# grunwaldlab/krisp

Hardware: AMD Instinct MI355X
Metric: k-mers/s sorted+intersected at k=28 (higher is better)
Workload: dtype u64

## Files before the change

### include/krisp_hip.h

```cpp
#ifndef KRISP_HIP_H
#define KRISP_HIP_H

#include <stddef.h>
#include <stdint.h>

#ifdef __cplusplus
extern "C" {
#endif

typedef struct kr_ctx kr_ctx;

typedef struct { uint64_t prefix, in_mask, out_mask; } kr_cand;

typedef struct { uint64_t key; uint32_t genome; uint32_t count; } kr_record;

enum {
    KR_OK = 0,
    KR_ERR_HIP = -1,
    KR_ERR_PARAM = -2,
    KR_ERR_CAPACITY = -3,
    KR_ERR_STATE = -4,
    KR_ERR_KEY = -5,
    KR_ERR_HOST = -6
};
// ... 122 lines not shown
int64_t kr_design_fetch(kr_ctx*, kr_design_record* out, size_t cap);
typedef struct {
    int32_t loop_ds[64];
} kr_hairpin_params;
int kr_design_hairpins(kr_ctx*, const kr_hairpin_params* params);
int64_t kr_design_fetch_hairpins(kr_ctx*, int32_t* out, size_t cap);

typedef struct {
    int32_t guide_size, pam5_len, pam3_len;
    uint8_t pam5[8], pam3[8];
    int32_t gc_lo, gc_hi, min_mismatches;
} kr_guide_params;
int kr_guides_table(kr_ctx*, const kr_guide_params* params);
typedef struct {
    uint32_t found, strand, start, min_mismatches, sum_mismatches, gc, candidates, pad;
} kr_guide_record;
int64_t kr_guides_run(kr_ctx*, const uint8_t* rows, const uint64_t* row_off, const uint32_t* bounds, uint64_t nregions, int K,
                      int L, int D);
int64_t kr_guides_fetch(kr_ctx*, kr_guide_record* out, size_t cap);
int64_t kr_guides_run_top(kr_ctx*, const uint8_t* rows, const uint64_t* row_off, const uint32_t* bounds, uint64_t nregions, int K,
                          int L, int D, int top);
int64_t kr_guides_fetch_top(kr_ctx*, kr_guide_record* out, size_t cap);

int64_t kr_guide_hits_table(kr_ctx*, const uint8_t* texts, uint64_t nguides, int mismatches, const char* pam5, const char* pam3,
                            int need_pam);
typedef struct { uint32_t guide; uint8_t strand, mismatches, pam, pad; uint64_t pos; uint64_t columns; } kr_guide_hit;
int64_t kr_guide_hits_scan(kr_ctx*, int id);
int64_t kr_guide_hits_fetch(kr_ctx*, kr_guide_hit* out, size_t cap);
int64_t kr_guide_hits_windows(kr_ctx*, uint8_t* rows, size_t cap_bytes);
int64_t kr_guide_hits_tally(kr_ctx*, uint32_t* out, size_t cap);

int64_t kr_guide_bulges_table(kr_ctx*, const uint8_t* texts, uint64_t nguides, int mismatches, int bulges, const char* pam5,
                              const char* pam3, int need_pam);
typedef struct { uint32_t guide; uint8_t strand, mismatches, pam; int8_t bulge; uint64_t pos; uint64_t columns;
                 uint32_t bulge_column, length; } kr_guide_bulge_hit;
int64_t kr_guide_bulges_scan(kr_ctx*, int id);
int64_t kr_guide_bulges_fetch(kr_ctx*, kr_guide_bulge_hit* out, size_t cap);
int64_t kr_guide_bulges_windows(kr_ctx*, uint8_t* rows, size_t cap_bytes);

int64_t kr_assay_table(kr_ctx*, const uint32_t* links, uint64_t n);
typedef struct { uint64_t pos; uint32_t length, pair; uint8_t strand, left_mm, right_mm, left_end_mm, right_end_mm, hit_strand,
                 hit_mismatches, hit_pam; uint64_t hit_pos; uint64_t columns; uint32_t guide, hit; } kr_assay_hit;
int64_t kr_assay_join(kr_ctx*, int id);
int64_t kr_assay_fetch(kr_ctx*, kr_assay_hit* out, size_t cap);

int64_t kr_fasta_to_bases(const uint8_t* text, size_t n, int universal_newlines, int one_shot, uint8_t* out,
                          size_t cap, int64_t* stats);

int64_t kr_ingest_file(const char* path, uint8_t** bases, int64_t* stats);
int64_t kr_read_file(const char* path, uint8_t** text, int64_t* stats);
int64_t kr_genome_upload_bgzf(kr_ctx*, int id, const uint8_t* file, size_t n, int one_shot, int64_t* stats);
int64_t kr_genome_upload_gzip(kr_ctx*, int id, const uint8_t* file, size_t n, size_t chunk, int one_shot, int64_t* stats);
int kr_reserve(kr_ctx*, const int* ids, int n, size_t n_bases, int with_text);
int kr_mem_info(kr_ctx*, int64_t* out4);
int64_t kr_genome_upload_text(kr_ctx*, int id, const uint8_t* text, size_t n, int universal_newlines, int one_shot,
                              int64_t* stats);
int64_t kr_genome_fetch_bases(kr_ctx*, int id, uint8_t* out, size_t cap);
void    kr_host_free(void* p);

int64_t kr_scan_special(const uint8_t* bases, size_t n, int k, int omit_soft, uint64_t* starts, size_t cap,
                        int* bad_char);

int64_t kr_render_records(const kr_record* recs, size_t n, int L, int D, int R, const uint32_t* label_of,
                          size_t n_genomes, const char* const* label_text, size_t n_labels, const uint8_t* label_in,
                          int dot, char** csv, size_t* csv_len, char** align, size_t* align_len);
int64_t kr_render_windows(const uint8_t* rows, size_t n, int L, int D, int R, const uint32_t* cand, const uint32_t* genome,
                          const uint32_t* label_of, size_t n_genomes, const char* const* label_text, size_t n_labels,
                          const uint8_t* label_in, int dot, int rna, char** csv, size_t* csv_len, char** align,
                          size_t* align_len);
void    kr_text_free(void* p);

enum { KR_OPT_SLICE_BASES = 1,
       KR_OPT_GENERIC_INTERSECT = 2,
       KR_OPT_ISECT_FORMAT = 3,
       KR_OPT_ABLATE = 4,
       KR_OPT_WIDE_SLOTS = 5,
       KR_OPT_PLACE_TRIES = 7,
       KR_OPT_ISECT_KERNEL = 8,
       KR_OPT_LANES = 9,
       KR_OPT_LAZY_ORDER = 10,
       KR_OPT_COARSE_REST = 11,
       KR_OPT_COARSE_POOL = 12,
       KR_OPT_JOIN2 = 13,
       KR_OPT_WIDE_ORDERED = 6 };
int     kr_set_option(kr_ctx*, int option, int64_t value);

int     kr_sync(kr_ctx*);
int     kr_timer_begin(kr_ctx*);
double  kr_timer_end_ms(kr_ctx*);
int     kr_stage_enable(kr_ctx*, int on);
int     kr_stage_select(kr_ctx*, unsigned stage_mask);
int     kr_stage_reset(kr_ctx*);
double  kr_stage_ms(kr_ctx*, int stage);
int64_t kr_stage_launches(kr_ctx*, int stage);

int64_t kr_debug_fetch(kr_ctx*, int genome_id, int what, void* out, size_t cap_bytes);
int64_t kr_debug_inversions(kr_ctx*, int genome_id);
double  kr_debug_localsort(kr_ctx*, int genome_id, int reps, int mode);
double  kr_debug_intersect(kr_ctx*, const int* genome_ids, int n, const uint8_t* is_ingroup, int reps, int mode);
double  kr_debug_copy_gbps(kr_ctx*, size_t bytes, int reps);
const char* kr_debug_copy_which(kr_ctx*);
int     kr_build_experiments(void);
int     kr_debug_lazy(kr_ctx*, int64_t* out8);
int     kr_debug_isect(kr_ctx*, int64_t* out8);
int     kr_debug_scan(kr_ctx*, int64_t* out8);
int     kr_debug_place(kr_ctx*, double* out8);
int     kr_debug_coarse_pool(kr_ctx*, double* out8);
int     kr_debug_comm(kr_ctx*, int64_t* out8);
int     kr_debug_comm_probe(kr_ctx*, size_t bytes, int reps, double* out3);
int64_t kr_debug_cands_selfexchange(kr_ctx*, int apply_filter);
int     kr_debug_comm_hang(kr_ctx*);
int64_t kr_debug_budget_left(kr_ctx*);
int     kr_debug_budget_set(kr_ctx*, int64_t left);
int     kr_debug_info(kr_ctx*, int64_t* out8);

#ifdef __cplusplus
}
#endif
#endif
```

### krisp_amd/_native.py

```python
import ctypes
import os

import numpy as np

HERE = os.path.dirname(os.path.abspath(__file__))
LIB_PATH = os.environ.get("KRISP_HIP_LIB") or os.path.join(HERE, "libkrisp_hip.so")

CAND = np.dtype([("prefix", "<u8"), ("in_mask", "<u8"), ("out_mask", "<u8")])
RECORD = np.dtype([("key", "<u8"), ("genome", "<u4"), ("count", "<u4")])
WIDE_HIT = np.dtype([("cand", "<u4"), ("genome", "<u4"), ("pos", "<u4"), ("strand", "<u4")])
LOC_HIT = np.dtype([("group", "<u4"), ("strand", "<u4"), ("pos", "<u8")])
NEAR_HIT = np.dtype([("target", "<u4"), ("strand", "u1"), ("mismatches", "u1"), ("flank_mismatches", "u1"), ("pad", "u1"),
                     ("pos", "<u8")])
PRODUCT_SITE = np.dtype([("pos", "<u8"), ("entry", "<u4"), ("mismatches", "u1"), ("end_mismatches", "u1"),
                         ("pad", "<u2")])
PRODUCT_HIT = np.dtype([("pos", "<u8"), ("length", "<u4"), ("pair", "<u4"), ("strand", "u1"), ("left_mm", "u1"),
                        ("right_mm", "u1"), ("left_end_mm", "u1"), ("right_end_mm", "u1"), ("pad", "u1", (3,))])
DESIGN_RECORD = np.dtype([("found", "<u4"), ("product_size", "<u4"), ("pair_penalty", "<u4"), ("left_start", "<u2"),
                          ("left_len", "<u2"), ("right_start", "<u2"), ("right_len", "<u2"), ("left_tm", "<i4"), ("right_tm", "<i4"),
                          ("left_gc", "<u2"), ("right_gc", "<u2"), ("left_penalty", "<u4"), ("right_penalty", "<u4"),
                          ("left_self_any", "<i4"), ("left_self_end", "<i4"), ("right_self_any", "<i4"),
                          ("right_self_end", "<i4"), ("pair_any", "<i4"), ("pair_end", "<i4")])
DESIGN_RECORD_HP = np.dtype(DESIGN_RECORD.descr + [("left_hairpin", "<i4"), ("right_hairpin", "<i4")])
GUIDE_RECORD = np.dtype([("found", "<u4"), ("strand", "<u4"), ("start", "<u4"), ("min_mismatches", "<u4"),
                         ("sum_mismatches", "<u4"), ("gc", "<u4"), ("candidates", "<u4"), ("pad", "<u4")])
GUIDE_HIT_RAW = np.dtype([("guide", "<u4"), ("strand", "u1"), ("mismatches", "u1"), ("pam", "u1"), ("pad", "u1"), ("pos", "<u8"),
                          ("columns", "<u8")])
ASSAY_HIT_RAW = np.dtype([("pos", "<u8"), ("length", "<u4"), ("pair", "<u4"), ("strand", "u1"), ("left_mm", "u1"), ("right_mm", "u1"),
                          ("left_end_mm", "u1"), ("right_end_mm", "u1"), ("hit_strand", "u1"), ("hit_mismatches", "u1"),
                          ("hit_pam", "u1"), ("hit_pos", "<u8"), ("columns", "<u8"), ("guide", "<u4"), ("hit", "<u4")])
GUIDE_BULGE_HIT_RAW = np.dtype([("guide", "<u4"), ("strand", "u1"), ("mismatches", "u1"), ("pam", "u1"), ("bulge", "i1"),
                                ("pos", "<u8"), ("columns", "<u8"), ("bulge_column", "<u4"), ("length", "<u4")])
WIDE_DICT_LEFT, WIDE_DICT_RIGHT, WIDE_GROUPS, WIDE_HITS, WIDE_COUNTS, WIDE_SLOT_BITS, WIDE_NGROUPS, WIDE_BATCH_USED, WIDE_LOCATED, WIDE_KEYS_LISTED = 0, 1, 2, 3, 4, 5, 6, 7, 8, 9
WIDE_MAX_K = 1024
WIDE_MAX_FLANK = 256
COMM_ID_BYTES = 128

SOFT_MAP, SOFT_OMIT = 0, 1
OPT_SLICE_BASES, OPT_GENERIC_INTERSECT, OPT_ISECT_FORMAT, OPT_ABLATE, OPT_WIDE_SLOTS, OPT_WIDE_ORDERED, OPT_PLACE_TRIES = 1, 2, 3, 4, 5, 6, 7
OPT_ISECT_KERNEL = 8
OPT_LANES = 9
OPT_LAZY_ORDER = 10
OPT_COARSE_REST = 11
OPT_COARSE_POOL = 12
OPT_JOIN2 = 13
ERR_KEY, ERR_HOST = -5, -6
STRANDS_BOTH, STRANDS_FORWARD, STRANDS_CANONICAL = 0, 1, 2
STAGES = ["pack", "hist8", "reduce8", "scatter1", "hist2", "scan2", "scatter2", "chunks", "localsort",
          "fallback", "intersect", "compact", "collect", "merge", "locate"]
STAGE_KERNELS = {"pack": "k_pack", "hist8": "k_hist8 (wide path: k_hist8w, slices: k_hist8k)", "reduce8": "k_reduce8a+k_reduce8b",
                 "scatter1": "k_scatter1p (wide path: k_scatter1w, slices: k_scatter1kp)",
                 "hist2": "k_hist16 (or k_hist2)", "scan2": "k_hist16_off (or k_scan2)", "scatter2": "k_scatter2",
                 "chunks": "k_chunk_table", "localsort": "k_localsort2",
                 "fallback": "k_seg_merge", "intersect": "k_intersect3 (+ k_intersect for oversized items)",
                 "compact": "k_scan+k_publish_reset+k_gather_items",
                 "collect": "k_collect_count+k_tile_sums+k_scan+k_tile_apply+k_publish+k_collect_emit",
                 "merge": "k_cands_flag+k_scan+k_cands_compact", "locate": "k_wide_locate"}

_c = ctypes
_P = _c.c_void_p
SYMBOLS = [
    ("kr_create", _P, [_c.c_int, _c.c_size_t]),
    ("kr_destroy", None, [_P]),
    ("kr_last_error", _c.c_char_p, [_P]),
    ("kr_set_params", _c.c_int, [_P, _c.c_int, _c.c_int, _c.c_int, _c.c_int, _c.c_size_t]),
    ("kr_set_strands", _c.c_int, [_P, _c.c_int]),
    ("kr_genome_upload", _c.c_int, [_P, _c.c_int, _P, _c.c_size_t]),
    ("kr_genome_sort", _c.c_int, [_P, _c.c_int]),
    ("kr_genome_partition", _c.c_int, [_P, _c.c_int]),
    ("kr_genome_add", _c.c_int64, [_P, _c.c_int, _P, _c.c_size_t]),
    ("kr_genome_count", _c.c_int64, [_P, _c.c_int]),
    ("kr_genome_load_sorted", _c.c_int64, [_P, _c.c_int, _P, _c.c_size_t]),
    ("kr_genome_fetch_keys", _c.c_int64, [_P, _c.c_int, _P, _c.c_size_t]),
    ("kr_genome_keys_in_order", _c.c_int64, [_P, _c.c_int, _P, _c.c_size_t]),
    ("kr_set_allow", _c.c_int, [_P, _c.c_uint]),
    ("kr_set_field_order", _c.c_int, [_P, _P, _P]),
    ("kr_set_field_pieces", _c.c_int, [_P, _c.c_int, _P, _P]),
    ("kr_genome_free", _c.c_int, [_P, _c.c_int]),
    ("kr_intersect", _c.c_int64, [_P, _P, _c.c_int, _P, _c.c_int]),
    ("kr_cands_count", _c.c_int64, [_P]),
    ("kr_cands_fetch", _c.c_int64, [_P, _P, _c.c_size_t]),
    ("kr_cands_load", _c.c_int64, [_P, _P, _c.c_size_t]),
    ("kr_cands_merge", _c.c_int64, [_P, _P, _c.c_size_t, _c.c_int, _c.c_int]),
    ("kr_cands_probe", _c.c_int64, [_P, _P, _c.c_int, _P, _c.c_int]),
    ("kr_comm_unique_id", _c.c_int, [_P]),
    ("kr_comm_init", _c.c_int, [_P, _c.c_int, _c.c_int, _P]),
    ("kr_comm_init_dir", _c.c_int, [_P, _c.c_int, _c.c_int, _c.c_char_p]),
    ("kr_comm_destroy", _c.c_int, [_P]),
    ("kr_comm_rank", _c.c_int, [_P]),
    ("kr_comm_world", _c.c_int, [_P]),
    ("kr_comm_rccl_ranks", _c.c_int, [_P]),
    ("kr_comm_barrier", _c.c_int, [_P]),
    ("kr_comm_allreduce", _c.c_int, [_P, _P, _c.c_int, _c.c_int]),
    ("kr_comm_allgather", _c.c_int, [_P, _P, _c.c_size_t, _P]),
    ("kr_cands_reduce", _c.c_int64, [_P, _c.c_int]),
    ("kr_cands_bcast", _c.c_int64, [_P]),
    ("kr_records_gather", _c.c_int64, [_P]),
    ("kr_collect", _c.c_int64, [_P, _P, _c.c_int]),
    ("kr_fetch", _c.c_int64, [_P, _P, _c.c_size_t]),
    ("kr_set_params_wide", _c.c_int, [_P, _c.c_int, _c.c_int, _c.c_int, _c.c_int, _c.c_size_t]),
    ("kr_wide_run", _c.c_int64, [_P, _P, _c.c_int, _P, _c.c_int]),
    ("kr_wide_fetch", _c.c_int64, [_P, _c.c_int, _P, _c.c_size_t]),
    ("kr_wide_fetch_windows", _c.c_int64, [_P, _P, _c.c_size_t]),
    ("kr_set_params_locate", _c.c_int, [_P, _c.c_int, _c.c_int, _c.c_int, _c.c_int, _c.c_size_t]),
    ("kr_locate_table", _c.c_int64, [_P, _P, _c.c_uint64]),
    ("kr_locate_scan", _c.c_int64, [_P, _c.c_int]),
    ("kr_locate_fetch", _c.c_int64, [_P, _P, _c.c_size_t]),
    ("kr_locate_windows", _c.c_int64, [_P, _P, _c.c_size_t]),
    ("kr_locate_seps", _c.c_int64, [_P, _c.c_int, _P, _c.c_size_t]),
    ("kr_near_table", _c.c_int64, [_P, _P, _c.c_uint64, _c.c_int]),
    ("kr_near_scan", _c.c_int64, [_P, _c.c_int]),
    ("kr_near_fetch", _c.c_int64, [_P, _P, _c.c_size_t]),
    ("kr_near_windows", _c.c_int64, [_P, _P, _c.c_size_t]),
    ("kr_products_table", _c.c_int64, [_P, _P, _c.c_uint64, _P, _c.c_uint64, _P, _c.c_uint64, _c.c_int, _c.c_uint32]),
    ("kr_products_scan", _c.c_int64, [_P, _c.c_int]),
    ("kr_products_fetch", _c.c_int64, [_P, _P, _c.c_size_t]),
    ("kr_products_sites", _c.c_int64, [_P, _P, _c.c_size_t]),
    ("kr_primers_table", _c.c_int64, [_P, _P, _P, _c.c_uint64, _c.c_uint64, _P, _c.c_uint64, _c.c_int, _c.c_uint32]),
    ("kr_primers_scan", _c.c_int64, [_P, _c.c_int]),
    ("kr_primers_fetch", _c.c_int64, [_P, _P, _c.c_size_t]),
    ("kr_primers_sites", _c.c_int64, [_P, _P, _c.c_size_t]),
    ("kr_design_table", _c.c_int, [_P, _P]),
    ("kr_design_run", _c.c_int64, [_P, _P, _c.c_uint64, _c.c_int, _c.c_int, _c.c_int]),
    ("kr_design_fetch", _c.c_int64, [_P, _P, _c.c_size_t]),
    ("kr_design_hairpins", _c.c_int, [_P, _P]),
    ("kr_design_fetch_hairpins", _c.c_int64, [_P, _P, _c.c_size_t]),
    ("kr_guides_table", _c.c_int, [_P, _P]),
    ("kr_guides_run", _c.c_int64, [_P, _P, _P, _P, _c.c_uint64, _c.c_int, _c.c_int, _c.c_int]),
    ("kr_guides_fetch", _c.c_int64, [_P, _P, _c.c_size_t]),
    ("kr_guides_run_top", _c.c_int64, [_P, _P, _P, _P, _c.c_uint64, _c.c_int, _c.c_int, _c.c_int, _c.c_int]),
    ("kr_guides_fetch_top", _c.c_int64, [_P, _P, _c.c_size_t]),
    ("kr_guide_hits_table", _c.c_int64, [_P, _P, _c.c_uint64, _c.c_int, _c.c_char_p, _c.c_char_p, _c.c_int]),
    ("kr_guide_hits_scan", _c.c_int64, [_P, _c.c_int]),
    ("kr_guide_hits_fetch", _c.c_int64, [_P, _P, _c.c_size_t]),
    ("kr_guide_hits_windows", _c.c_int64, [_P, _P, _c.c_size_t]),
    ("kr_guide_hits_tally", _c.c_int64, [_P, _P, _c.c_size_t]),
    ("kr_guide_bulges_table", _c.c_int64, [_P, _P, _c.c_uint64, _c.c_int, _c.c_int, _c.c_char_p, _c.c_char_p, _c.c_int]),
    ("kr_guide_bulges_scan", _c.c_int64, [_P, _c.c_int]),
    ("kr_guide_bulges_fetch", _c.c_int64, [_P, _P, _c.c_size_t]),
    ("kr_guide_bulges_windows", _c.c_int64, [_P, _P, _c.c_size_t]),
    ("kr_assay_table", _c.c_int64, [_P, _P, _c.c_uint64]),
    ("kr_assay_join", _c.c_int64, [_P, _c.c_int]),
    ("kr_assay_fetch", _c.c_int64, [_P, _P, _c.c_size_t]),
    ("kr_render_windows", _c.c_int64, [_P, _c.c_size_t, _c.c_int, _c.c_int, _c.c_int, _P, _P, _P, _c.c_size_t, _P, _c.c_size_t, _P,
                                       _c.c_int, _c.c_int, _P, _P, _P, _P]),
    ("kr_fasta_to_bases", _c.c_int64, [_P, _c.c_size_t, _c.c_int, _c.c_int, _P, _c.c_size_t, _P]),
    ("kr_ingest_file", _c.c_int64, [_c.c_char_p, _P, _P]),
    ("kr_read_file", _c.c_int64, [_c.c_char_p, _P, _P]),
    ("kr_genome_upload_text", _c.c_int64, [_P, _c.c_int, _P, _c.c_size_t, _c.c_int, _c.c_int, _P]),
    ("kr_genome_upload_bgzf", _c.c_int64, [_P, _c.c_int, _P, _c.c_size_t, _c.c_int, _P]),
    ("kr_genome_upload_gzip", _c.c_int64, [_P, _c.c_int, _P, _c.c_size_t, _c.c_size_t, _c.c_int, _P]),
    ("kr_reserve", _c.c_int, [_P, _P, _c.c_int, _c.c_size_t, _c.c_int]),
    ("kr_genome_fetch_bases", _c.c_int64, [_P, _c.c_int, _P, _c.c_size_t]),
    ("kr_host_free", None, [_P]),
    ("kr_scan_special", _c.c_int64, [_P, _c.c_size_t, _c.c_int, _c.c_int, _P, _c.c_size_t, _P]),
    ("kr_set_option", _c.c_int, [_P, _c.c_int, _c.c_int64]),
    ("kr_sync", _c.c_int, [_P]),
    ("kr_timer_begin", _c.c_int, [_P]),
    ("kr_timer_end_ms", _c.c_double, [_P]),
    ("kr_stage_enable", _c.c_int, [_P, _c.c_int]),
    ("kr_stage_select", _c.c_int, [_P, _c.c_uint]),
    ("kr_stage_reset", _c.c_int, [_P]),
    ("kr_stage_ms", _c.c_double, [_P, _c.c_int]),
    ("kr_stage_launches", _c.c_int64, [_P, _c.c_int]),
    ("kr_debug_fetch", _c.c_int64, [_P, _c.c_int, _c.c_int, _P, _c.c_size_t]),
    ("kr_debug_inversions", _c.c_int64, [_P, _c.c_int]),
    ("kr_debug_localsort", _c.c_double, [_P, _c.c_int, _c.c_int, _c.c_int]),
    ("kr_debug_intersect", _c.c_double, [_P, _P, _c.c_int, _P, _c.c_int, _c.c_int]),
    ("kr_debug_copy_gbps", _c.c_double, [_P, _c.c_size_t, _c.c_int]),
    ("kr_debug_copy_which", _c.c_char_p, [_P]),
    ("kr_mem_info", _c.c_int, [_P, _P]),
    ("kr_debug_comm", _c.c_int, [_P, _P]),
    ("kr_debug_place", _c.c_int, [_P, _P]),
    ("kr_debug_coarse_pool", _c.c_int, [_P, _P]),
    ("kr_debug_comm_probe", _c.c_int, [_P, _c.c_size_t, _c.c_int, _P]),
    ("kr_debug_cands_selfexchange", _c.c_int64, [_P, _c.c_int]),
    ("kr_debug_info", _c.c_int, [_P, _P]),
    ("kr_render_records", _c.c_int64, [_P, _c.c_size_t, _c.c_int, _c.c_int, _c.c_int, _P, _c.c_size_t, _P, _c.c_size_t, _P,
                                       _c.c_int, _P, _P, _P, _P]),
    ("kr_text_free", None, [_P]),
    ("kr_debug_isect", _c.c_int, [_P, _P]),
    ("kr_debug_lazy", _c.c_int, [_P, _P]),
    ("kr_debug_scan", _c.c_int, [_P, _P]),
    ("kr_set_mixed_alphabets", _c.c_int, [_P, _c.c_int]),
    ("kr_build_experiments", _c.c_int, []),
    ("kr_comm_set_timeout", _c.c_int, [_P, _c.c_int]),
    ("kr_debug_comm_hang", _c.c_int, [_P]),
    ("kr_debug_budget_left", _c.c_int64, [_P]),
    ("kr_debug_budget_set", _c.c_int, [_P, _c.c_int64]),
]


class GuideParams(ctypes.Structure):
    _fields_ = [("guide_size", _c.c_int32), ("pam5_len", _c.c_int32), ("pam3_len", _c.c_int32), ("pam5", _c.c_uint8 * 8),
                ("pam3", _c.c_uint8 * 8), ("gc_lo", _c.c_int32), ("gc_hi", _c.c_int32), ("min_mismatches", _c.c_int32)]


class KrispHipError(RuntimeError):
    code = None


ERR_CAPACITY = -3


_lib = None


def load():
    global _lib
    if _lib is not None:
        return _lib
    if not os.path.exists(LIB_PATH):
        raise KrispHipError(
            f"{LIB_PATH} is missing: build it with `python -m krisp_amd.build` "
            "(hipcc --offload-arch=gfx950); there is no CPU fallback")
    lib = ctypes.CDLL(LIB_PATH)
    for name, res, args in SYMBOLS:
        fn = getattr(lib, name)
        fn.restype = res
        fn.argtypes = args
    _lib = lib
    return lib


def _ptr(a):
    return a.ctypes.data_as(ctypes.c_void_p)


def _motif_bytes(m):
    return m if isinstance(m, bytes) else str(m).encode("ascii", "replace")


def fasta_to_bases(data, universal_newlines, one_shot=True):
    lib = load()
    src = np.frombuffer(data, dtype=np.uint8)
    out = np.empty(len(src) + 1, dtype=np.uint8)
    stats = np.zeros(4, dtype=np.int64)
    n = lib.kr_fasta_to_bases(_ptr(src) if len(src) else None, len(src), 1 if universal_newlines else 0,
                              1 if one_shot else 0, _ptr(out), len(out), _ptr(stats))
    if n < 0:
        raise KrispHipError(f"kr_fasta_to_bases: [{n}]")
    return out[:n], int(stats[0]), int(stats[1]), stats[2] == 1, bool(stats[3])


class _HostBlock:

    def __init__(self, lib, ptr):
        self.lib, self.ptr = lib, ptr

    def __del__(self):
        try:
            if self.ptr:
                self.lib.kr_host_free(self.ptr)
                self.ptr = None
        except Exception:
            pass

# ... 555 lines not shown

    def guides_top(self, rows, row_off, bounds, L, D, top):
        rows, off, bnd, n = self._guide_regions(rows, row_off, bounds, "guides_top")
        self._check(self.lib.kr_guides_run_top(self.ctx, _ptr(rows) if rows.size else None, _ptr(off), _ptr(bnd) if n else None, n,
                                               rows.shape[1], L, D, top), "kr_guides_run_top")
        out = np.empty((max(n, 1), top), dtype=GUIDE_RECORD)
        self._check(self.lib.kr_guides_fetch_top(self.ctx, _ptr(out), n * top), "kr_guides_fetch_top")
        return out[:n]

    def sync(self):
        self._check(self.lib.kr_sync(self.ctx), "kr_sync")

    def timer_begin(self):
        self._check(self.lib.kr_timer_begin(self.ctx), "kr_timer_begin")

    def timer_end_ms(self):
        ms = self.lib.kr_timer_end_ms(self.ctx)
        if ms < 0:
            raise KrispHipError("kr_timer_end_ms failed")
        return ms

    def stage_enable(self, on=True):
        self.lib.kr_stage_enable(self.ctx, 1 if on else 0)

    def stage_select(self, names):
        mask = 0
        for n in names:
            mask |= 1 << STAGES.index(n)
        self.lib.kr_stage_select(self.ctx, mask)

    def stage_reset(self):
        self.lib.kr_stage_reset(self.ctx)

    def stage_times(self):
        return {name: (self.lib.kr_stage_ms(self.ctx, i), self.lib.kr_stage_launches(self.ctx, i))
                for i, name in enumerate(STAGES)}

    def debug_info(self):
        o = np.zeros(8, dtype=np.int64)
        self.lib.kr_debug_info(self.ctx, _ptr(o))
        return dict(b=int(o[0]), nbuckets=int(o[1]), T=int(o[2]), CAP=int(o[3]), nwg=int(o[4]),
                    overflow_segments=int(o[5]), fallback_launches=int(o[6]), nslices=int(o[7]))

    def debug_isect(self):
        o = np.zeros(8, dtype=np.int64)
        self.lib.kr_debug_isect(self.ctx, _ptr(o))
        return dict(chunk_kernel_items=int(o[0]), slices_redone=int(o[1]), threads=int(o[2]), buckets_per_item_log2=int(o[3]),
                    heads32=int(o[4]), sort_lanes=int(o[5]), join2_launches=int(o[6]), join2_handed_on=int(o[7]))

    def debug_lazy(self):
        o = np.zeros(8, dtype=np.int64)
        self.lib.kr_debug_lazy(self.ctx, _ptr(o))
        return dict(skipped=int(o[0]), ordered_later=int(o[1]), touch_collects=int(o[2]), on=int(o[3]),
                    anchor_in_bucket_order=int(o[4]), fuse_anchor=int(o[5]), coarse=int(o[6]), coarse_promoted=int(o[7]))

    def debug_scan(self):
        o = np.zeros(8, dtype=np.int64)
        self.lib.kr_debug_scan(self.ctx, _ptr(o))
        return dict(tiles=int(o[0]), grid=int(o[1]), cap=int(o[2]), blocks=int(o[3]))

    def copy_gbps(self, nbytes=1 << 30, reps=10):
        v = self.lib.kr_debug_copy_gbps(self.ctx, nbytes, reps)
        if v < 0:
            raise KrispHipError("kr_debug_copy_gbps failed")
        return v

    def mem_info(self):
        o = np.zeros(4, dtype=np.int64)
        self._check(self.lib.kr_mem_info(self.ctx, _ptr(o)), "kr_mem_info")
        return dict(avail=int(o[0]), total=int(o[1]), used=int(o[2]), budget=int(o[3]))

    def debug_comm(self):
        o = np.zeros(8, dtype=np.int64)
        self._check(self.lib.kr_debug_comm(self.ctx, _ptr(o)), "kr_debug_comm")
        return dict(syncs=int(o[0]), p2p=int(o[1]), collectives=int(o[2]), exchange_us=int(o[3]), reduces=int(o[4]),
                    message_entries=int(o[5]))

    def debug_place(self):
        o = np.zeros(8, dtype=np.float64)
        self._check(self.lib.kr_debug_place(self.ctx, _ptr(o)), "kr_debug_place")
        return dict(candidates=int(o[0]), taken=int(o[1]), fastest_ms=[round(float(x), 4) for x in o[2:6]],
                    median_ms=round(float(o[6]), 4), slowest_ms=round(float(o[7]), 4))

    def debug_coarse_pool(self):
        o = np.zeros(8, dtype=np.float64)
        self._check(self.lib.kr_debug_coarse_pool(self.ctx, _ptr(o)), "kr_debug_coarse_pool")
        return dict(total=int(o[0]), free=int(o[1]), held=int(o[2]), partitions=int(o[3]), searches=int(o[4]),
                    held_ms=[round(float(o[5]), 4), round(float(o[6]), 4)], on=int(o[7]))

    def comm_set_timeout(self, seconds):
        self._check(self.lib.kr_comm_set_timeout(self.ctx, int(seconds)), "kr_comm_set_timeout")

    def debug_comm_hang(self):
        return self._check(self.lib.kr_debug_comm_hang(self.ctx), "kr_debug_comm_hang")

    def cands_selfexchange(self, apply_filter=False):
        return self._check(self.lib.kr_debug_cands_selfexchange(self.ctx, 1 if apply_filter else 0), "kr_debug_cands_selfexchange")

    def comm_probe(self, nbytes=64 << 10, reps=50):
        o = np.zeros(3, dtype=np.float64)
        self._check(self.lib.kr_debug_comm_probe(self.ctx, nbytes, reps, _ptr(o)), "kr_debug_comm_probe")
        return dict(allreduce_sync_us=round(float(o[0]), 2), sendrecv_self_sync_us=round(float(o[1]), 2),
                    bcast_sync_us=round(float(o[2]), 2), message_bytes=int(nbytes))

    def copy_which(self):
        return (self.lib.kr_debug_copy_which(self.ctx) or b"").decode()

    def inversions(self, gid):
        return self._check(self.lib.kr_debug_inversions(self.ctx, gid), "kr_debug_inversions")

    def debug_fetch(self, gid, what, n_max):
        dt = {0: np.uint64, 1: np.uint32, 2: np.uint32, 3: np.uint32, 4: np.uint64, 5: np.uint64}[what]
        out = np.empty(max(n_max, 1), dtype=dt)
        n = self._check(self.lib.kr_debug_fetch(self.ctx, gid, what, _ptr(out), out.nbytes), "kr_debug_fetch")
        return out[:n]
```

### krisp_amd/csrc/h_core.inc

```
static thread_local std::string g_last_error;

struct DevBuf {
    void* p = nullptr;
    size_t bytes = 0;
};

struct Slice {
    DevBuf keys, off, chunkstart, chunkdesc, ovf;
    u64 nmax = 0;
    u32 nchunks = 0;
    int64_t count = -1;
    int res = -1;
};

struct Genome {
    int id = -1;
    size_t n_bases = 0;
    u64 nwords = 0;
    u64 nmax = 0;
    DevBuf bases, wkeys;
    DevBuf wlcnt;
    bool wlist = false;
    u32 wlcap = 0;
    std::vector<Slice> sl;
    bool uploaded = false, sorted = false, finalized = false;
    bool ordered = false;
    bool coarse = false;
    DevBuf ckeys;
    double ckeys_ms = 0;
    hipStream_t ckeys_busy = nullptr;
    hipEvent_t ckeys_ev = nullptr;
    bool ckeys_wait = false;
    int64_t partitions = 0;
    DevBuf hits;
    u32 hitcap = 0;
    bool hits_valid = false;
    bool was_anchor = false;
    int64_t count = -1;
    hipEvent_t up_done = nullptr;
};

struct Lane {
    hipStream_t stream = nullptr;
    hipEvent_t done = nullptr;
    bool pending = false;
    DevBuf codes, bad, partial8, base1, tmpkeys, tp, tiledesc, tilehist, wkeys;
    DevBuf partial16, cursor, h16exc;
    DevBuf pass0, base64;
    DevBuf slt, offa, cura;
    void bufs(std::vector<DevBuf*>& v) {
        v.insert(v.end(), {&codes, &bad, &partial8, &base1, &tmpkeys, &tp, &tiledesc, &tilehist, &wkeys, &pass0, &base64,
                           &partial16, &cursor, &h16exc, &slt, &offa, &cura});
    }
};
#define MAX_LANES 8

struct kr_comm;

struct kr_ctx {
    int device = 0;
    kr_comm* comm = nullptr;
    hipStream_t stream = nullptr;
    hipStream_t copy_stream = nullptr;
    Lane lanes[MAX_LANES];
    int nlanes = 0, next_lane = 0;
    int lanes_ready = 0;
    int64_t sorts_done = 0;
    int place_n = 0, place_taken = 0;
    double place_ms[6] = {0, 0, 0, 0, 0, 0};
    size_t place_bytes = 0;
    u64 ex_cap = 0;
    char copy_which[160] = {0};
    u64 lane_maxcount = 0;
    int last_lane = 0;
    int sb = 0, nslices = 1;
    size_t budget = 0, used = 0;
    bool have_params = false;
    Geom g{};
    size_t max_bases = 0;
    std::map<int, Genome> genomes;
    int ls_grid = 768;
    int place_tries = 8;
    bool place_tries_set = false;
    bool shared_gpu = false;
    DevBuf candP;
    DevBuf candA, candB, chunkcnt, chunkpos, flags, blockcnt, blockpos, other, records, nrec, fbdesc, fbsegs;
    DevBuf coltab, collo, colcnt, colpos, coltsum, coltpos, colfirst, colfm;
    int64_t ncand = -1;
    int64_t nrecords = 0;
    std::string err;
    hipEvent_t t0 = nullptr, t1 = nullptr;
    bool stage_on = false;
    unsigned stage_mask = ~0u;
    struct Pair { hipEvent_t a, b; int stage; };
    std::vector<Pair> pending;
    std::vector<hipEvent_t> pool;
    double stage_ms[KR_ST_COUNT] = {0};
    int64_t stage_n[KR_ST_COUNT] = {0};
    int64_t fallback_launches = 0, overflow_segments = 0;
    int dbg = 0;
    int isect_kernel = 0;
    int ncu = 256;
    DevBuf bgz_in, bgz_tab, bgz_stat;
    DevBuf tx_scan;
    DevBuf tx_text, tx_tile, tx_tilepos, tx_lines, tx_ls, tx_ll, tx_op, tx_outpos, tx_state, tx_tsum, tx_tpos;
    u32* mbox = nullptr;
    std::vector<uint64_t> coltab_host;
    std::vector<int> mb_free;
    int mb_next = 0;
    int i3_occ[3][4][9] = {{{0}}};
    DevBuf isovf;
    int join2 = 1;
    u32 j2_grid = 0;
    int j2_occ[9] = {0};
    int64_t j2_launches = 0, j2_full = 0;
    bool j2_full_counted = false;
    int64_t isect_ovf_items = 0, isect_refall = 0;
    int i3_last_T = 0, i3_last_mlog = 0, i3_last_tags = 0, i3_last_ua = 0;
    int64_t isect_ua = 0;
    int fuse_anchor = 1;
    u32 i3_ovf_cap = I3_OVF_CAP;
    int isect_fmt = 0;
    int opt_slice_bases = -1;
    hipEvent_t slice_ready[2] = {nullptr, nullptr};
    bool custom_layout = false;
    bool mixed_alphabets = false;
    int lazy_order = 1;
    bool order_wanted = false;
    int64_t lazy_skipped = 0, lazy_ordered = 0, lazy_touch = 0;
    DevBuf touchdesc, touchovf;
    int coarse_rest = 1;
    int64_t coarse_done = 0, coarse_promoted = 0;
    int coarse_pool = 1;
    struct PoolBuf { DevBuf buf; double ms; hipEvent_t ev; bool wait; };
    std::vector<PoolBuf> cpool_free;
    int cpool_total = 0;
    int64_t cpool_partitions = 0;
    int64_t cpool_searches = 0;
    size_t place_min_bytes = (size_t)256 << 20;
    DevBuf co_state, co_tab;
    u32 co_tcap = CO_TCAP;
    u32 co_hitcap = 0;
    int co_occ = 0;
    u32 co_grid = 0;
    u32 scan_cap = 0;
    int64_t scan_dbg[3] = {0, 0, 0};
    int slice_route = 1;
    typedef std::vector<DevBuf*> Bufs;
    struct Wide {
        bool on = false;
        int L = 0, D = 0, R = 0, k = 0, omit = 0, W = 0, strands = 0;
        struct DictBufs {
            DevBuf keys, idx, slots;
            DevBuf mzT, mzB;
            int ib = 1, sb = 0, mzlen = 0;
            u32 n = 0, mznb = 0;
            bool canon = false;
            u32 nfull = 0;
            void bufs(Bufs& v) { v.insert(v.end(), {&keys, &idx, &slots, &mzT, &mzB}); }
            Dict view() const {
                Dict d{};
                d.keys = (const u64*)keys.p;
                d.idx = (const u32*)idx.p;
                d.slots = sb && slots.p ? (const uint4*)slots.p : nullptr;
                d.ib = ib;
                d.sb = sb;
                d.mzT = mzlen && mzT.p ? (const u64*)mzT.p : nullptr;
                d.mzB = (const u32*)mzB.p;
                d.mznb = mznb;
                d.mzlen = mzlen;
                d.canon = canon ? 1 : 0;
                return d;
            }
        };
        DictBufs fd[2][2 * FR_MAXP - 1], fin;
        static int fd_pieces(int len) { return (len + 31) / 32; }
        static int fd_plen(int len, int j) { const int np = fd_pieces(len); return len / np + (j < len % np ? 1 : 0); }
        static int fd_poff(int len, int j) { int o = 0; for (int q = 0; q < j; q++) o += fd_plen(len, q); return o; }
        static int fd_last(int len) { return fd_pieces(len) > 1 ? 2 * (fd_pieces(len) - 1) : 0; }
        FlankRank fr[2];
        DevBuf flbuf;
        FlankRank flhost[8][2];
        int flslot = 0;
        std::vector<int> run_ids;
        DevBuf rows, rowtab;
        DevBuf masks, keep, cnt, hitoff, cursor, hits, cibuf, tsum, tpos;
        DevBuf loc, loccur;
        u64 located = 0;
        bool use_slots = true;
        bool ordered = false;
        bool use_share = true;
        int lanes = 0;
        bool packed_spectrum = true;
        DevBuf wcount;
        bool share = false;
        bool genome_cache = false;
        bool key_list = false;
        bool key_list_failed = false;
        double key_list_frac = 0;
        u64 keys_listed = 0;
        int batch = 0;
        std::vector<u64> nkeys;
        u32 nfin = 0;
        u64 ngroups = 0;
        int64_t nhits = -1;
        void locate_bufs(Bufs& v) { v.insert(v.end(), {&masks, &keep, &cnt, &hitoff, &cursor, &hits, &cibuf, &loc}); }
        void bufs(Bufs& v) {
            fin.bufs(v);
            locate_bufs(v);
            v.insert(v.end(), {&loccur, &tsum, &tpos, &wcount, &flbuf, &rows, &rowtab});
            for (auto& flank : fd)
                for (DictBufs& d : flank) d.bufs(v);
        }
    } wide;
    struct SeedTable {
// ... 173 lines not shown

#define MB_WORDS 65536
#define MB_SLICE0 64
#define PUB_CAP 4096
static int mbox_slot(kr_ctx* c) {
    if (!c->mb_free.empty()) { const int s = c->mb_free.back(); c->mb_free.pop_back(); return s; }
    if (MB_SLICE0 + 2 * (c->mb_next + 1) > MB_WORDS) return -1;
    return c->mb_next++;
}

static void coarse_pool_handover(kr_ctx* c, Genome& G) {
    if (!G.ckeys.p || !G.ckeys_busy) return;
    if (!G.ckeys_ev && hipEventCreateWithFlags(&G.ckeys_ev, hipEventDisableTiming) != hipSuccess) G.ckeys_ev = nullptr;
    if (G.ckeys_ev && hipEventRecord(G.ckeys_ev, G.ckeys_busy) == hipSuccess) G.ckeys_wait = true;
    else (void)hipStreamSynchronize(G.ckeys_busy);
    G.ckeys_busy = nullptr;
    (void)c;
}
static void coarse_pool_return(kr_ctx* c, Genome& G) {
    if (!G.ckeys.p) return;
    coarse_pool_handover(c, G);
    kr_ctx::PoolBuf pb{G.ckeys, G.ckeys_ms, G.ckeys_ev, G.ckeys_wait};
    auto at = c->cpool_free.begin();
    while (at != c->cpool_free.end() && at->ms <= pb.ms) ++at;
    c->cpool_free.insert(at, pb);
    G.ckeys = DevBuf();
    G.ckeys_ms = 0;
    G.ckeys_ev = nullptr;
    G.ckeys_wait = false;
}
static void coarse_pool_purge(kr_ctx* c, size_t bytes) {
    for (size_t i = c->cpool_free.size(); i-- > 0;) {
        kr_ctx::PoolBuf& pb = c->cpool_free[i];
        if (pb.buf.bytes >= bytes) continue;
        if (pb.ev) { if (pb.wait) (void)hipEventSynchronize(pb.ev); (void)hipEventDestroy(pb.ev); }
        release(c, pb.buf);
        c->cpool_free.erase(c->cpool_free.begin() + (long)i);
        c->cpool_total--;
    }
}
static bool coarse_pool_take(kr_ctx* c, Genome& G, size_t bytes) {
    for (auto at = c->cpool_free.begin(); at != c->cpool_free.end(); ++at)
        if (at->buf.bytes >= bytes) {
            G.ckeys = at->buf;
            G.ckeys_ms = at->ms;
            G.ckeys_ev = at->ev;
            G.ckeys_wait = at->wait;
            G.ckeys_busy = nullptr;
            c->cpool_free.erase(at);
            return true;
        }
    return false;
}
static void coarse_pool_release(kr_ctx* c) {
    if (c->cpool_free.empty()) return;
    (void)hipDeviceSynchronize();
    for (auto& pb : c->cpool_free) {
        release(c, pb.buf);
        if (pb.ev) (void)hipEventDestroy(pb.ev);
    }
    c->cpool_total -= (int)c->cpool_free.size();
    c->cpool_free.clear();
}

static void release_slice(kr_ctx* c, Slice& S) {
    release(c, S.keys);
    release(c, S.off);
    release(c, S.chunkstart);
    release(c, S.chunkdesc);
    release(c, S.ovf);
    if (S.res >= 0) c->mb_free.push_back(S.res);
}
static void genome_drop_sorted(kr_ctx* c, Genome& G) {
    for (Slice& S : G.sl) release_slice(c, S);
    G.sl.clear();
    G.sorted = G.finalized = G.ordered = false;
}
static void reset_slices(kr_ctx* c, Genome& G) {
    if ((int)G.sl.size() == c->nslices) return;
    for (Slice& S : G.sl) release_slice(c, S);
    G.sl.assign(c->nslices, Slice());
}
static void genome_unsorted(Genome& G) {
    G.sorted = G.finalized = G.ordered = G.coarse = G.hits_valid = false;
    G.count = -1;
}

static void release_genome(kr_ctx* c, Genome& G) {
    coarse_pool_return(c, G);
    if (G.up_done) { (void)hipEventDestroy(G.up_done); G.up_done = nullptr; }
    release(c, G.bases);
    release(c, G.wkeys);
    release(c, G.wlcnt);
    release(c, G.hits);
    for (Slice& S : G.sl) release_slice(c, S);
    G.sl.clear();
}

struct StageScope {
    kr_ctx* c;
    int stage;
    hipEvent_t a = nullptr, b = nullptr;
    hipStream_t stream;
    StageScope(kr_ctx* c_, int st, hipStream_t s_ = nullptr) : c(c_), stage(st), stream(s_ ? s_ : c_->stream) {
        c->stage_n[st]++;
        if (!c->stage_on || !((c->stage_mask >> st) & 1u)) return;
        auto get = [&]() {
            hipEvent_t e;
            if (!c->pool.empty()) { e = c->pool.back(); c->pool.pop_back(); }
            else (void)hipEventCreate(&e);
            return e;
        };
        a = get();
        b = get();
        (void)hipEventRecord(a, stream);
    }
    ~StageScope() {
        if (!a) return;
        (void)hipEventRecord(b, stream);
        c->pending.push_back({a, b, stage});
    }
};

static void resolve_stages(kr_ctx* c) {
    for (auto& p : c->pending) {
        float ms = 0;
        (void)hipEventSynchronize(p.b);
        if (hipEventElapsedTime(&ms, p.a, p.b) == hipSuccess) c->stage_ms[p.stage] += ms;
        c->pool.push_back(p.a);
        c->pool.push_back(p.b);
    }
    c->pending.clear();
}

#define LANES_AUTO 3
#define LANES_AFTER 16
static inline int lanes_used(const kr_ctx* c) {
    if (c->wide.on) return c->wide.lanes > 0 ? c->wide.lanes : (c->nlanes > 1 ? 2 : 1);
    if (c->g.wmode) return 1;
    if (c->nslices > 1) return c->nlanes == 1 || (c->nlanes == 0 && c->sorts_done < 2) ? 1 : 2;
    return c->nlanes > 0 ? c->nlanes : (c->sorts_done >= LANES_AFTER ? LANES_AUTO : 1);
}

static int join_lanes(kr_ctx* c) {
    for (int i = 1; i < MAX_LANES; i++) {
        Lane& ln = c->lanes[i];
        if (!ln.pending) continue;
        HIPCHK(c, hipEventRecord(ln.done, ln.stream));
        HIPCHK(c, hipStreamWaitEvent(c->stream, ln.done, 0));
        ln.pending = false;
    }
    return KR_OK;
}

static int lane_open(kr_ctx* c, Lane& ln) {
    if (ln.stream) return KR_OK;
    HIPCHK(c, hipStreamCreate(&ln.stream));
    HIPCHK(c, hipEventCreateWithFlags(&ln.done, hipEventDisableTiming));
    return KR_OK;
}
static void release_lanes(kr_ctx* c, int first) {
    std::vector<DevBuf*> lb;
    for (int i = first; i < MAX_LANES; i++) c->lanes[i].bufs(lb);
    for (DevBuf* b : lb) release(c, *b);
}
static int ensure_h16exc(kr_ctx* c, Lane& ln, hipStream_t st) {
    if (ln.h16exc.p) return KR_OK;
    int rc;
    if ((rc = ensure(c, ln.h16exc, (1 + 3 * (size_t)H16_EXC_CAP) * 4))) return rc;
    HIPCHK(c, hipMemsetAsync(ln.h16exc.p, 0, 16, st));
    return KR_OK;
}

static void launch_excl_scan(hipStream_t st, const u32* in, u32 n, u32* tsum, u32* tpos, u32* out) {
    const u32 ntiles = (n + 2047) / 2048;
    hipLaunchKernelGGL(k_tile_sums, dim3(ntiles), dim3(256), 0, st, in, n, tsum);
    hipLaunchKernelGGL(k_scan, dim3(1), dim3(1024), 0, st, (const u32*)tsum, tpos, ntiles);
    hipLaunchKernelGGL(k_tile_apply, dim3(ntiles), dim3(256), 0, st, in, n, (const u32*)tpos, ntiles, out);
}

extern "C" {

const char* kr_last_error(kr_ctx* c) { return c ? c->err.c_str() : g_last_error.c_str(); }

kr_ctx* kr_create(int device, size_t hbm_budget_bytes) {
    int ndev = 0;
    if (hipGetDeviceCount(&ndev) != hipSuccess || ndev <= 0) {
        g_last_error = "no HIP device visible";
        return nullptr;
    }
    if (device < 0 || device >= ndev) {
        g_last_error = "device index out of range";
        return nullptr;
    }
    if (hipSetDevice(device) != hipSuccess) {
        g_last_error = "hipSetDevice failed";
        return nullptr;
    }
    kr_ctx* c = new kr_ctx();
    c->device = device;
    c->budget = hbm_budget_bytes;
    {
        const char* e = getenv("KR_DBG");
        c->dbg = e ? (atoi(e) & 32) : 0;
        const char* e2 = getenv("KR_ISECT_FMT");
        c->isect_fmt = e2 ? (atoi(e2) == 1 ? 1 : (atoi(e2) == 2 ? 2 : 0)) : 0;
        const char* e3 = getenv("KR_SLICE_BASES");
        c->opt_slice_bases = e3 ? std::max(0, std::min(4, atoi(e3))) : -1;
        const char* e16 = getenv("KR_FUSE_ANCHOR");
        c->fuse_anchor = e16 ? atoi(e16) != 0 : 1;
        const char* e15 = getenv("KR_LAZY_ORDER");
        c->lazy_order = e15 ? atoi(e15) != 0 : 1;
        const char* e17 = getenv("KR_COARSE_REST");
        c->coarse_rest = e17 ? atoi(e17) != 0 : 1;
        const char* e21 = getenv("KR_COARSE_POOL");
        c->coarse_pool = e21 ? atoi(e21) != 0 : 1;
        const char* e22 = getenv("KR_PLACE_MIN_BYTES");
        if (e22) c->place_min_bytes = (size_t)std::max(0ll, atoll(e22));
        const char* e18 = getenv("KR_COARSE_TCAP");
        if (e18) c->co_tcap = (u32)std::max(1, std::min((int)CO_TCAP, atoi(e18)));
        const char* e19 = getenv("KR_COARSE_HITCAP");
        if (e19) c->co_hitcap = (u32)std::max(1, atoi(e19));
        const char* e20 = getenv("KR_COARSE_GRID");
        if (e20) c->co_grid = (u32)std::max(0, std::min(65536, atoi(e20)));
        const char* e24 = getenv("KR_JOIN2");
        c->join2 = e24 ? atoi(e24) != 0 : 1;
        const char* e25 = getenv("KR_JOIN2_GRID");
        if (e25) c->j2_grid = (u32)std::max(0, std::min(65536, atoi(e25)));
        const char* e23 = getenv("KR_SCAN_GRID");
        if (e23) c->scan_cap = (u32)std::max(0, std::min(65536, atoi(e23)));
        const char* e13 = getenv("KR_SLICE_ROUTE");
        c->slice_route = e13 ? atoi(e13) != 0 : 1;
        const char* e8 = getenv("KR_PLACE_TRIES");
        c->place_tries = e8 ? std::max(1, std::min(16, atoi(e8))) : 8;
        c->place_tries_set = e8 != nullptr;
        const char* e4 = getenv("KR_WIDE_SLOTS");
        c->wide.use_slots = e4 ? atoi(e4) != 0 : true;
        const char* e7 = getenv("KR_WIDE_SHARE");
        c->wide.use_share = e7 ? atoi(e7) != 0 : true;
        const char* e11 = getenv("KR_WIDE_SPECTRUM");
        c->wide.packed_spectrum = e11 ? atoi(e11) != 0 : true;
        const char* e5 = getenv("KR_WIDE_ORDERED");
        c->wide.ordered = e5 ? atoi(e5) != 0 : false;
        int ncu = 256, per = 3;
        (void)hipDeviceGetAttribute(&ncu, hipDeviceAttributeMultiprocessorCount, device);
        if (hipOccupancyMaxActiveBlocksPerMultiprocessor(&per, k_localsort2, LS_THREADS, 0) != hipSuccess || per < 1)
            per = 2;
        c->ls_grid = ncu * per;
        c->ncu = ncu;
        const char* e9 = getenv("KR_ISECT_KERNEL");
        c->isect_kernel = e9 ? (atoi(e9) == 1 ? 1 : (atoi(e9) == 2 ? 2 : 0)) : 0;
        const char* e10 = getenv("KR_ISECT_OVF_CAP");
        if (e10) c->i3_ovf_cap = (u32)std::max(0, std::min((int)I3_OVF_CAP, atoi(e10)));
    }
    {
        const char* e = getenv("KR_LANES");
        int nl = e ? atoi(e) : 0;
        c->nlanes = nl < 0 ? 0 : (nl > MAX_LANES ? MAX_LANES : nl);
    }
    bool ok = hipHostMalloc((void**)&c->mbox, MB_WORDS * 4 + PUB_CAP * sizeof(PubEnt), hipHostMallocMapped) == hipSuccess &&
              hipEventCreate(&c->t0) == hipSuccess && hipEventCreate(&c->t1) == hipSuccess &&
              hipStreamCreateWithFlags(&c->copy_stream, hipStreamNonBlocking) == hipSuccess;
    ok = ok && lane_open(c, c->lanes[0]) == KR_OK;
    if (!ok) {
        g_last_error = "stream / event creation failed";
        delete c;
        return nullptr;
    }
    c->stream = c->lanes[0].stream;
    return c;
}

int kr_comm_destroy(kr_ctx* c);

void kr_destroy(kr_ctx* c) {
    if (!c) return;
    (void)kr_comm_destroy(c);
    (void)hipSetDevice(c->device);
    (void)hipDeviceSynchronize();
    resolve_stages(c);
    release_lanes(c, 0);
    for (auto& kv : c->genomes) release_genome(c, kv.second);
    coarse_pool_release(c);
    DevBuf* all[] = {&c->candA, &c->candB, &c->chunkcnt,
                     &c->chunkpos, &c->flags, &c->blockcnt, &c->blockpos, &c->other, &c->records, &c->nrec, &c->fbdesc, &c->fbsegs,
                     &c->coltab, &c->collo, &c->colcnt, &c->colpos, &c->coltsum, &c->coltpos, &c->colfirst, &c->colfm, &c->isovf,
                     &c->bgz_in, &c->bgz_tab, &c->bgz_stat, &c->tx_scan, &c->tx_text, &c->tx_tile, &c->tx_tilepos, &c->tx_lines, &c->tx_ls, &c->tx_ll, &c->tx_op, &c->tx_outpos, &c->tx_state,
                     &c->tx_tsum, &c->tx_tpos, &c->candP, &c->touchdesc, &c->touchovf, &c->co_state, &c->co_tab};
    for (DevBuf* b : all) release(c, *b);
    {
        kr_ctx::Bufs sb;
        c->wide.bufs(sb);
        c->loc.bufs(sb); c->near.bufs(sb); c->ghit.bufs(sb); c->gbulge.bufs(sb); c->prod.bufs(sb); c->prim.bufs(sb); c->assay.bufs(sb);
        for (DevBuf* b : sb) release(c, *b);
        auto& ds = c->design;
        DevBuf* db[] = {&ds.par, &ds.tmpl, &ds.rec, &ds.hprec};
        for (DevBuf* b : db) release(c, *b);
        auto& gu = c->guides;
        DevBuf* gb[] = {&gu.rows, &gu.off, &gu.bnd, &gu.rec};
        for (DevBuf* b : gb) release(c, *b);
    }
    if (c->mbox) (void)hipHostFree(c->mbox);
    for (auto e : c->pool) (void)hipEventDestroy(e);
    if (c->copy_stream) (void)hipStreamDestroy(c->copy_stream);
    for (hipEvent_t e : c->slice_ready) if (e) (void)hipEventDestroy(e);
    (void)hipEventDestroy(c->t0);
    (void)hipEventDestroy(c->t1);
    for (int i = 0; i < MAX_LANES; i++) {
        if (c->lanes[i].done) (void)hipEventDestroy(c->lanes[i].done);
        if (c->lanes[i].stream) (void)hipStreamDestroy(c->lanes[i].stream);
    }
    delete c;
}

static u64 topbits(int nbits) { return nbits <= 0 ? 0ull : (nbits >= 64 ? ~0ull : (~0ull << (64 - nbits))); }

static Geom slice_geom(const kr_ctx* c, u32 slice) {
    Geom g = c->g;
    g.slice = slice;
    return g;
}

#define KR_RETRY_DENSE (-1000)
static Geom make_geom(int L, int D, int R, int omit, int sb, int b) {
    Geom g{};
    const int k = L + D + R;
    g.k = k; g.L = L; g.D = D; g.R = R;
    g.sR = 2 * D;
    g.sD = 2 * R;
    g.topmask = topbits(2 * k);
    g.mL = topbits(2 * L);
    g.mR = topbits(2 * (L + R)) & ~g.mL;
    g.mD = topbits(2 * k) & ~topbits(2 * (L + R));
    g.omit = omit;
    g.allow = 15;
    g.sbits = 2 * sb;
    g.slice = 0;
    g.LRrel = L - sb + R;
    g.pmask = topbits(2 * g.LRrel);
    g.b = b;
    g.rb = 64 - b;
    return g;
}

static int plan_sort(kr_ctx* c, size_t max_bases, int Lmin, int& sb, int& b) {
    const u64 nmax = 2 * (u64)max_bases;
    sb = 0;
    while (sb < 4 && (nmax >> (2 * sb)) > (BUCKET_AVG << 18)) sb++;
    if (sb > 0)
        while (sb < 4 && sb < Lmin && (nmax >> (2 * sb)) > (BUCKET_AVG << 16)) sb++;
    const bool forced = c->opt_slice_bases >= 0;
    if (forced) sb = c->opt_slice_bases;
    if (sb > Lmin) {
        if (forced) sb = Lmin;
        else return fail(c, KR_ERR_PARAM, "a genome of %zu bases needs %d slice bases but conserved-left is %d", max_bases, sb, Lmin);
    }
    if ((nmax >> (2 * sb)) > (BUCKET_AVG << 18) * 4)
        return fail(c, KR_ERR_PARAM, "genome of %zu bases is too large for %d slice bases", max_bases, sb);
    if (sb == 0 && nmax >= KR_MAX_SLICE_KEYS)
        return fail(c, KR_ERR_CAPACITY, "a genome of %zu bases gives up to %llu keys in one sort unit (the limit is %llu, "
                    "the 4 GiB a buffer descriptor spans): use key-space slices (KR_OPT_SLICE_BASES >= 1)", max_bases,
                    (unsigned long long)nmax, (unsigned long long)KR_MAX_SLICE_KEYS);
    const u64 per_slice = nmax >> (2 * sb);
    b = 8;
    while (b < 18 && (per_slice >> b) > BUCKET_AVG) b++;
    return KR_OK;
}

int kr_set_params(kr_ctx* c, int L, int D, int R, int softmask_mode, size_t max_bases) {
    if (!c) return KR_ERR_PARAM;
    const int k = L + D + R;
    if (L < 0 || D < 0 || R < 0 || k < 1 || k > 32)
        return fail(c, KR_ERR_PARAM, "need 1 <= L+D+R <= 32 on the packed path (got %d/%d/%d)", L, D, R);
    if (D > 16) return fail(c, KR_ERR_PARAM, "diagnostic length %d > 16 unsupported by the mask format", D);
    if (softmask_mode != KR_SOFT_MAP && softmask_mode != KR_SOFT_OMIT)
        return fail(c, KR_ERR_PARAM, "unknown softmask mode %d", softmask_mode);
    if (!c->genomes.empty()) return fail(c, KR_ERR_STATE, "kr_set_params after genomes were uploaded");
    coarse_pool_release(c);
    if (max_bases >= KR_MAX_BASES) return fail(c, KR_ERR_PARAM, "genomes of >= 2^33 bases are not supported");
    int sb, b, rc;
    if ((rc = plan_sort(c, max_bases, L, sb, b))) return rc;
    c->sb = sb;
    c->nslices = 1 << (2 * sb);
    c->g = make_geom(L, D, R, softmask_mode == KR_SOFT_OMIT, sb, b);
    c->max_bases = max_bases;
    c->have_params = true;
    c->wide.on = false;
    c->custom_layout = false;
    return KR_OK;
}

static int ensure_lanes(kr_ctx* c, u64 maxcount);

int kr_set_option(kr_ctx* c, int option, int64_t value) {
    if (!c) return KR_ERR_PARAM;
    switch (option) {
    case KR_OPT_SLICE_BASES:
        if (value < -1 || value > 4) return fail(c, KR_ERR_PARAM, "KR_OPT_SLICE_BASES: -1 .. 4");
        if (!c->genomes.empty()) return fail(c, KR_ERR_STATE, "KR_OPT_SLICE_BASES after genomes were uploaded");
        c->opt_slice_bases = (int)value;
        return KR_OK;
    case KR_OPT_GENERIC_INTERSECT:
        c->dbg = (c->dbg & ~32) | (value ? 32 : 0);
        return KR_OK;
    case KR_OPT_ISECT_FORMAT:
        if (value < 0 || value > 2) return fail(c, KR_ERR_PARAM, "KR_OPT_ISECT_FORMAT: 0, 1 or 2");
        c->isect_fmt = (int)value;
        return KR_OK;
    case KR_OPT_ISECT_KERNEL:
        if (value < 0 || value > 2) return fail(c, KR_ERR_PARAM, "KR_OPT_ISECT_KERNEL: 0, 1 or 2");
        c->isect_kernel = (int)value;
        return KR_OK;
    case KR_OPT_WIDE_SLOTS:
        if (value != 0 && value != 1) return fail(c, KR_ERR_PARAM, "KR_OPT_WIDE_SLOTS: 0 or 1");
        c->wide.use_slots = value != 0;
        return KR_OK;
    case KR_OPT_LANES:
        if (value < 0 || value > MAX_LANES) return fail(c, KR_ERR_PARAM, "KR_OPT_LANES: 0 (automatic), 1 .. %d", MAX_LANES);
        HIPCHK(c, hipSetDevice(c->device));
        { int rcj = join_lanes(c); if (rcj) return rcj; }
        HIPCHK(c, hipDeviceSynchronize());
        c->nlanes = (int)value;
        c->next_lane = 0;
        return (c->have_params && c->lane_maxcount) ? ensure_lanes(c, c->lane_maxcount) : KR_OK;
    case KR_OPT_PLACE_TRIES:
        if (value < 1 || value > 16) return fail(c, KR_ERR_PARAM, "KR_OPT_PLACE_TRIES: 1 .. 16");
        c->place_tries = (int)value;
        c->place_tries_set = true;
        return KR_OK;
    case KR_OPT_WIDE_ORDERED:
        if (value != 0 && value != 1) return fail(c, KR_ERR_PARAM, "KR_OPT_WIDE_ORDERED: 0 or 1");
        c->wide.ordered = value != 0;
        return KR_OK;
    case KR_OPT_LAZY_ORDER:
        if (value != 0 && value != 1) return fail(c, KR_ERR_PARAM, "KR_OPT_LAZY_ORDER: 0 or 1");
        c->lazy_order = (int)value;
        return KR_OK;
    case KR_OPT_COARSE_REST:
        if (value != 0 && value != 1) return fail(c, KR_ERR_PARAM, "KR_OPT_COARSE_REST: 0 or 1");
        c->coarse_rest = (int)value;
        return KR_OK;
    case KR_OPT_COARSE_POOL:
        if (value != 0 && value != 1) return fail(c, KR_ERR_PARAM, "KR_OPT_COARSE_POOL: 0 or 1");
        c->coarse_pool = (int)value;
        return KR_OK;
    case KR_OPT_JOIN2:
        if (value != 0 && value != 1) return fail(c, KR_ERR_PARAM, "KR_OPT_JOIN2: 0 or 1");
        c->join2 = (int)value;
        return KR_OK;
    case KR_OPT_ABLATE:
#ifdef KR_ABLATE
        c->dbg = (c->dbg & 32) | ((int)value & ~32);
        return KR_OK;
#else
        return fail(c, KR_ERR_PARAM, "KR_OPT_ABLATE needs a -DKR_ABLATE build");
#endif
    default:
        return fail(c, KR_ERR_PARAM, "unknown option %d", option);
    }
}

int kr_set_strands(kr_ctx* c, int mode) {
    if (!c || !c->have_params) return fail(c, KR_ERR_STATE, "kr_set_params first");
    if (mode < KR_STRANDS_BOTH || mode > KR_STRANDS_CANONICAL) return fail(c, KR_ERR_PARAM, "unknown strand mode %d", mode);
    if (c->wide.on && mode == KR_STRANDS_CANONICAL) return fail(c, KR_ERR_PARAM, "the wide path emits both strands or the forward one");
    if (!c->genomes.empty()) return fail(c, KR_ERR_STATE, "kr_set_strands after genomes were uploaded");
    c->g.strands = mode;
    c->wide.strands = mode;
    return KR_OK;
}

int kr_set_allow(kr_ctx* c, unsigned base_mask) {
    if (!c || !c->have_params) return fail(c, KR_ERR_STATE, "kr_set_params first");
    if (base_mask > 15) return fail(c, KR_ERR_PARAM, "kr_set_allow: a mask of the four bases A C G T (bits 0..3)");
    if (!c->genomes.empty()) return fail(c, KR_ERR_STATE, "kr_set_allow after genomes were uploaded");
    c->g.allow = base_mask;
    return KR_OK;
}

int kr_set_field_order(kr_ctx* c, const int* widths, const int* order) {
    if (!c || !c->have_params || c->wide.on) return fail(c, KR_ERR_STATE, "kr_set_params first");
    if (!widths || !order) return KR_ERR_PARAM;
    if (!c->genomes.empty()) return fail(c, KR_ERR_STATE, "kr_set_field_order after genomes were uploaded");
    const int k = c->g.k;
    if (c->g.D != 0 || c->g.R != 0 || c->g.L != k)
        return fail(c, KR_ERR_STATE, "kr_set_field_order: after kr_set_params(k, 0, 0, ...)");
    int seen = 0, sum = 0;
    for (int i = 0; i < 3; i++) {
        if (widths[i] < 0 || order[i] < 0 || order[i] > 2) return fail(c, KR_ERR_PARAM, "kr_set_field_order: widths >= 0, order a permutation of 0 1 2");
        seen |= 1 << order[i];
        sum += widths[i];
    }
    if (seen != 7 || sum != k) return fail(c, KR_ERR_PARAM, "kr_set_field_order: order must be a permutation of 0 1 2 and the widths add up to k = %d", k);
    int src0[3], dst[3];
    src0[0] = 0; src0[1] = widths[0]; src0[2] = widths[0] + widths[1];
    for (int i = 0, at = 0; i < 3; i++) { dst[order[i]] = at; at += widths[order[i]]; }
    u64 mS = 0, mLf = 0, mRt = 0;
    int sLf = 0, sRt = 0, rot = -1;
    for (int r : {0, src0[1], src0[2]}) {
        if (r >= k) continue;
        mS = mLf = mRt = 0;
        sLf = sRt = 0;
        bool ok = true;
        for (int f = 0; f < 3 && ok; f++) {
            if (!widths[f]) continue;
            const int src = (src0[f] - r + k) % k;
            if (src + widths[f] > k) { ok = false; break; }
            const u64 m = topbits(2 * (dst[f] + widths[f])) & ~topbits(2 * dst[f]);
            const int mv = dst[f] - src;
            if (mv == 0) mS |= m;
            else if (mv < 0) {
                if (sLf && sLf != -2 * mv) ok = false;
                sLf = -2 * mv; mLf |= m;
            } else {
                if (sRt && sRt != 2 * mv) ok = false;
                sRt = 2 * mv; mRt |= m;
            }
        }
        if (ok) { rot = 2 * r; break; }
    }
    if (rot < 0) return fail(c, KR_ERR_PARAM, "kr_set_field_order: this order needs two different shifts of one direction");
    c->g.rot = rot;
    c->g.mL = mS;
    c->g.sR = sLf; c->g.mR = mLf;
    c->g.sD = sRt; c->g.mD = mRt;
    const bool moved = (mS & topbits(2)) == 0 || mLf || mRt || rot;
    if (moved) { c->g.L = 0; c->g.LRrel = 0; c->g.pmask = 0; }
    c->custom_layout = moved;
// ... 150 lines not shown
        if (bufs[i]->bytes < bytes) todo.push_back(bufs[i]);
    if (todo.empty()) return KR_OK;
    int rc;
    for (DevBuf* b : todo)
        if ((rc = ensure(c, *b, bytes))) return rc;
    const int tries = place_tries_for(c, bytes);
    if (tries <= 1) return KR_OK;
    PlaceStats ps;
    place_search(c, todo, bytes, tries, ps);
    c->place_n = ps.n;
    c->place_taken = ps.taken;
    for (int i = 0; i < 6; i++) c->place_ms[i] = ps.ms[i];
    c->place_bytes = ps.bytes;
    return KR_OK;
}

static void coarse_pool_grow(kr_ctx* c, int want) {
    const size_t bytes = ((size_t)c->lane_maxcount + 2) * 8;
    if (want <= 0 || !c->coarse_pool || !c->lane_maxcount) return;
    coarse_pool_purge(c, bytes);
    want -= (int)c->cpool_free.size();
    if (want <= 0) return;
    const int tries = place_tries_for(c, bytes);
    if (tries <= 1) return;
    std::vector<DevBuf> fresh((size_t)want);
    std::vector<DevBuf*> todo;
    for (DevBuf& b : fresh) {
        if (ensure(c, b, bytes)) break;
        todo.push_back(&b);
    }
    c->err.clear();
    if (todo.empty()) return;
    PlaceStats ps;
    std::vector<double> ms;
    place_search(c, todo, bytes, tries, ps, &ms);
    c->err.clear();
    c->cpool_searches++;
    for (size_t i = 0; i < todo.size(); i++) {
        if (!todo[i]->p) continue;
        c->cpool_free.push_back({*todo[i], ms[i] > 0 ? ms[i] : 1e30, nullptr, false});
        c->cpool_total++;
    }
    std::stable_sort(c->cpool_free.begin(), c->cpool_free.end(),
                     [](const kr_ctx::PoolBuf& a, const kr_ctx::PoolBuf& b2) { return a.ms < b2.ms; });
}

static int ensure_lanes(kr_ctx* c, u64 maxcount) {
    const u32 nb = 1u << c->g.b;
    const u64 mw = (c->max_bases + 31) / 32 + PAD_WORDS + 2;
    const u64 ntmax = maxcount / P2_TILE + 260;
    int rc;
    c->lane_maxcount = std::max(c->lane_maxcount, maxcount);
    maxcount = c->lane_maxcount;
    c->lanes_ready = lanes_used(c);
    for (int i = 0; i < lanes_used(c); i++) {
        Lane& ln = c->lanes[i];
        if ((rc = lane_open(c, ln))) return rc;
        if ((rc = ensure(c, ln.codes, mw * 8))) return rc;
        if ((rc = ensure(c, ln.bad, mw * 4))) return rc;
        if ((rc = ensure(c, ln.partial8, (size_t)NWG * 256 * 4))) return rc;
        if ((rc = ensure(c, ln.base1, (260 + 256) * 4))) return rc;
        if ((rc = ensure(c, ln.tp, 260 * 4))) return rc;
        if ((rc = ensure(c, ln.base64, 260 * 8))) return rc;
        if ((rc = ensure(c, ln.tiledesc, ntmax * 8))) return rc;
        if ((rc = ensure(c, ln.tilehist, ntmax * (nb >> 8) * 4))) return rc;
        if (USE_HIST16 && nb > 256) {
            if ((rc = ensure(c, ln.partial16, (size_t)H16_RANGES * nb * 2 + 64))) return rc;
            if ((rc = ensure_h16exc(c, ln, ln.stream))) return rc;
            if ((rc = ensure(c, ln.cursor, ((size_t)nb + 4) * 4))) return rc;
        }
    }
    DevBuf* tk[MAX_LANES];
    for (int i = 0; i < lanes_used(c); i++) tk[i] = &c->lanes[i].tmpkeys;
    return ensure_placed(c, tk, lanes_used(c), (maxcount + 2) * 8);
}

static void launch_pack(kr_ctx* c, Genome& G, Lane& ln, hipStream_t st) {
    const u64 nwp = G.nwords + PAD_WORDS;
    u32 grid = (u32)std::min<u64>((nwp + 255) / 256, 4096);
    hipLaunchKernelGGL(k_pack, dim3(grid), dim3(256), 0, st, (const uint8_t*)G.bases.p, (u64)G.n_bases,
                       (u64*)ln.codes.p, (u32*)ln.bad.p, nwp, c->g.omit, c->g.allow);
}

static void launch_scatter1(const Geom& g, hipStream_t st, const u64* codes, const u32* bad, u64 nwords,
                            const u32* base1, const u64* base64, const u32* rowoff, u64* dst, u64 dst_keys) {
    const bool big = base64 != nullptr;
    static const bool fast_on = [] { const char* e = getenv("KR_P1_FAST"); return e ? atoi(e) != 0 : true; }();
    const bool fast = fast_on && g.wmode == 0 && g.strands == 0 && g.rot == 0 && g.npc == 0 && (u32)((g.mR | g.mD) >> 32) == 0u;
    if (g.wmode && g.wmode != 1 && g.wcmode == 4) {
        hipLaunchKernelGGL(k_scatter1l, dim3(NWG), dim3(P1_T), 0, st, base1, base64, rowoff, dst, g);
    } else if (g.wmode) {
        const auto kw = g.wmode == 1 ? k_scatter1w<1> : g.wcmode == 2 ? k_scatter1w<3> : k_scatter1w<2>;
        hipLaunchKernelGGL(kw, dim3(NWG), dim3(P1_T), 0, st, codes, bad, nwords, base1, base64, rowoff, dst, g);
    } else {
        const auto kp = fast ? (big ? k_scatter1p<0, 1, 1> : k_scatter1p<0, 0, 1>)
                             : g.strands ? (big ? k_scatter1p<2, 1> : k_scatter1p<2, 0>) : (big ? k_scatter1p<0, 1> : k_scatter1p<0, 0>);
        hipLaunchKernelGGL(kp, dim3(NWG), dim3(P1_T), 0, st, codes, bad, nwords, base1, base64, rowoff, dst, dst_keys, g);
    }
}

static void launch_scatter2(hipStream_t st, const u64* src, u64* dst, const uint2* tiledesc, u32 ntmax,
                            const u32* tilehist, u32* cursor, int b, int shl = 0, u32 region_n = 0) {
    hipLaunchKernelGGL(k_scatter2<2 * P2_T>, dim3(ntmax), dim3(2 * P2_T), 0, st, src, dst, tiledesc, tilehist, cursor, b, shl, region_n);
}

static void launch_hist8(kr_ctx* c, Genome& G, Lane& ln, hipStream_t st, const Geom& g) {
    const auto kh = g.wmode == 1 ? k_hist8w<1> : g.wmode ? (g.wcmode == 2 ? k_hist8w<3> : k_hist8w<2>) : g.strands ? k_hist8<2> : k_hist8<0>;
    hipLaunchKernelGGL(kh, dim3(NWG), dim3(P1_T), 0, st, (const u64*)ln.codes.p, (const u32*)ln.bad.p, G.nwords,
                       (u32*)ln.partial8.p, g);
}

static constexpr u32 P2_KEYS = 2 * P2_TILE;
static u32 p2_tiles(u64 nmax) { return (u32)(nmax / P2_KEYS) + 257; }

static Lane& peek_lane(kr_ctx* c) {
    if (c->next_lane >= lanes_used(c)) c->next_lane = 0;
    return c->lanes[c->next_lane];
}

static Geom pass0_geom(const kr_ctx* c, bool counting = false) {
    Geom g0 = c->g;
    g0.sbits = 0;
    g0.slice = 0;
    if (counting && g0.wmode == 2 && g0.wcache) g0.wcmode = g0.wlcnt ? 3 : 1;
    return g0;
}

static int count_slices(kr_ctx* c, Genome& G) {
    int rc;
    if ((rc = ensure_lanes(c, 16))) return rc;
    Lane& ln = peek_lane(c);
    hipStream_t st = ln.stream;
    ln.pending = true;
    if (G.up_done && st != c->stream) HIPCHK(c, hipStreamWaitEvent(st, G.up_done, 0));
    launch_pack(c, G, ln, st);
    reset_slices(c, G);
    std::vector<u32> tot(256);
    u64 maxcount = 0;
    G.nmax = 0;
    genome_unsorted(G);
    coarse_pool_return(c, G);
    const Geom g0 = pass0_geom(c, true);
    {
        StageScope sc(c, KR_ST_HIST8, st);
        launch_hist8(c, G, ln, st, g0);
    }
    hipLaunchKernelGGL(k_reduce8a, dim3(256), dim3(256), 0, st, (u32*)ln.partial8.p, (u32*)ln.base1.p + 260);
    HIPCHK(c, hipMemcpyAsync(tot.data(), (u32*)ln.base1.p + 260, 256 * 4, hipMemcpyDeviceToHost, st));
    std::vector<u32> seglen;
    if (g0.wcmode == 3) {
        seglen.resize(NWG);
        HIPCHK(c, hipMemcpyAsync(seglen.data(), g0.wlcnt, NWG * 4, hipMemcpyDeviceToHost, st));
    }
    HIPCHK(c, hipStreamSynchronize(st));
    if (g0.wcmode == 3) {
        u64 listed = 0;
        for (u32 v : seglen) {
            if (v > g0.wlcap) return KR_RETRY_DENSE;
            listed += v;
        }
        c->wide.keys_listed += listed;
    }
    const int per = 256 >> c->g.sbits;
    for (int s = 0; s < c->nslices; s++) {
        u64 cnt = 0;
        for (int d = s * per; d < (s + 1) * per; d++) cnt += tot[d];
        if (cnt >= KR_MAX_SLICE_KEYS)
            return fail(c, KR_ERR_CAPACITY, "slice %d of genome %d holds %llu keys (the limit is %llu, the 4 GiB a buffer "
                        "descriptor spans): raise KR_SLICE_BASES", s, G.id, (unsigned long long)cnt,
                        (unsigned long long)KR_MAX_SLICE_KEYS);
        if ((rc = alloc_slice(c, G.sl[s], cnt))) return rc;
        G.nmax += cnt;
        maxcount = std::max(maxcount, cnt);
    }
    if (c->nslices > 1 && (rc = ensure(c, ln.pass0, (G.nmax + 2) * 8))) return rc;
    HIPCHK(c, hipGetLastError());
    return ensure_lanes(c, maxcount);
}

static bool host_is_pinned(const void* p, int device);

static int upload_finish(kr_ctx* c, Genome& G, int id, size_t n);

int kr_genome_upload(kr_ctx* c, int id, const uint8_t* bases, size_t n) {
    if (!c || !c->have_params) return fail(c, KR_ERR_STATE, "kr_set_params first");
    if (n > c->max_bases) return fail(c, KR_ERR_PARAM, "genome of %zu bases exceeds max_bases %zu", n, c->max_bases);
    HIPCHK(c, hipSetDevice(c->device));
    const auto seen = c->genomes.find(id);
    const bool known = seen != c->genomes.end() && (seen->second.uploaded || seen->second.n_bases);
    if (known) HIPCHK(c, hipDeviceSynchronize());
// ... 16 lines not shown
static int upload_finish(kr_ctx* c, Genome& G, int id, size_t n) {
    int rc;
    if (c->wide.on || c->loc.on) {
        G.uploaded = true;
        return KR_OK;
    }
    if (c->nslices == 1) {
        reset_slices(c, G);
        const u64 bound = 2 * (u64)n;
        if (bound >= KR_MAX_SLICE_KEYS)
            return fail(c, KR_ERR_CAPACITY, "genome %d: %llu keys in one sort unit (the limit is %llu)", id,
                        (unsigned long long)bound, (unsigned long long)KR_MAX_SLICE_KEYS);
        if ((rc = alloc_slice(c, G.sl[0], bound))) return rc;
        G.nmax = bound;
        if ((rc = ensure_lanes(c, bound))) return rc;
    } else if ((rc = count_slices(c, G))) {
        return rc;
    }
    G.uploaded = true;
    return KR_OK;
}

#define SLICE_HELPER 2
#define SLICE_HELPERS 2
static inline int slice_lanes(const kr_ctx* c) { return c->nlanes == 1 ? 1 : 1 + SLICE_HELPERS; }

static int ensure_slice_lanes(kr_ctx* c, int helper) {
    const u32 nb = 1u << c->g.b;
    const u64 maxcount = c->lane_maxcount;
    const u64 ntmax = maxcount / P2_TILE + 260;
    int rc;
    Lane& ln = c->lanes[helper];
    if ((rc = lane_open(c, ln))) return rc;
    if ((rc = ensure(c, ln.base1, (260 + 256) * 4))) return rc;
    if ((rc = ensure(c, ln.tp, 260 * 4))) return rc;
    if ((rc = ensure(c, ln.slt, 1024 * 4))) return rc;
    if ((rc = ensure(c, ln.tiledesc, ntmax * 8))) return rc;
    if ((rc = ensure(c, ln.tilehist, ntmax * (nb >> 8) * 4))) return rc;
    return ensure(c, ln.tmpkeys, (maxcount + 2) * 8);
}

int kr_reserve(kr_ctx* c, const int* ids, int n, size_t n_bases, int with_text) {
    if (!c || !c->have_params) return fail(c, KR_ERR_STATE, "kr_set_params first");
    if (n < 0 || (n && !ids)) return fail(c, KR_ERR_PARAM, "kr_reserve: bad argument");
    if (n_bases > c->max_bases) return fail(c, KR_ERR_PARAM, "kr_reserve: %zu bases exceed max_bases %zu", n_bases, c->max_bases);
    HIPCHK(c, hipSetDevice(c->device));
    int rc;
    const u64 bound = 2 * (u64)n_bases;
    const u64 per_slice = c->nslices > 1 ? bound / (u64)c->nslices + bound / (u64)c->nslices / 50 + 4096 : bound;
    if (with_text && (rc = ensure(c, c->tx_text, n_bases + 64))) return rc;
    for (int i = 0; i < n; i++) {
        Genome& G = c->genomes[ids[i]];
        G.id = ids[i];
        if ((rc = ensure(c, G.bases, n_bases + 64))) return rc;
        if (c->wide.on || c->g.wmode) continue;
        reset_slices(c, G);
        if (per_slice >= KR_MAX_SLICE_KEYS) continue;
        for (Slice& S : G.sl)
            if ((rc = ensure(c, S.keys, (per_slice + 2) * 8))) return rc;
    }
    if (c->wide.on || c->g.wmode || !n || per_slice >= KR_MAX_SLICE_KEYS) return KR_OK;
    if ((rc = ensure_lanes(c, per_slice))) return rc;
    if (c->nslices > 1)
        for (int l = 0; l < std::min(n, lanes_used(c)); l++)
            if ((rc = ensure(c, c->lanes[l].pass0, (bound + 2) * 8))) return rc;
    return KR_OK;
}

static int genome_sort(kr_ctx* c, int id, bool reuse_count, bool coarse = false);
int kr_genome_sort(kr_ctx* c, int id) { return genome_sort(c, id, false); }

static bool coarse_eligible(const kr_ctx* c) {
    return c->coarse_rest && c->have_params && !c->wide.on && c->g.wmode == 0 && c->g.strands == 0 && !c->custom_layout &&
           c->nslices == 1 && c->g.b > 8;
}
int kr_genome_partition(kr_ctx* c, int id) {
    if (!c) return KR_ERR_PARAM;
    return genome_sort(c, id, false, coarse_eligible(c));
}

struct SortPlan {
    bool reuse_count;
    bool coarse;
    bool lazy;
    bool sliced, route2, fine16;
    bool cached_keys;
    int cached_mode;
    int nba;
    u32 h16_ranges;
    int nsl, helper;
};

static SortPlan sort_plan(const kr_ctx* c, const Genome& G, const Lane& ln, bool reuse_count, bool coarse) {
    SortPlan p{};
    p.reuse_count = reuse_count;
    p.coarse = coarse;
    p.cached_keys = reuse_count && c->g.wmode == 2 && c->g.wcache;
    p.cached_mode = c->g.wlcnt ? 4 : 2;
    p.sliced = c->nslices > 1;
    static const bool lazy_wide = [] { const char* e = getenv("KR_LAZY_WIDE"); return e ? atoi(e) != 0 : true; }();
    p.lazy = c->lazy_order && (lazy_wide || (!c->wide.on && c->g.wmode == 0)) && !c->custom_layout && c->g.strands == 0 &&
             !c->order_wanted && !(G.was_anchor && !c->i3_last_ua);
    p.nba = 8 + c->g.sbits;
    p.route2 = p.sliced && USE_HIST16 && c->slice_route && c->g.wmode == 0 && c->g.strands == 0 && 2 * c->g.L >= p.nba && p.nba <= 16;
    p.h16_ranges = H16_RANGES;
    if (p.route2)
        while (p.h16_ranges < NWG && G.nmax / ((u64)p.h16_ranges * 256) > 30000) p.h16_ranges *= 2;
    p.fine16 = USE_HIST16 && c->g.b > 8 && !p.sliced && c->g.wmode == 0 && c->g.strands == 0 && 2 * c->g.L >= c->g.b;
    p.nsl = p.route2 ? slice_lanes(c) : 1;
    p.helper = SLICE_HELPER + SLICE_HELPERS * (int)(&ln - c->lanes);
    return p;
}

static int take_lane(kr_ctx* c, Genome& G, Lane*& taken) {
    if (lanes_used(c) > c->lanes_ready) {
        int rcl = ensure_lanes(c, c->lane_maxcount);
        if (rcl && c->nlanes == 0) {
            release_lanes(c, 1);
            c->nlanes = 1;
            c->lanes_ready = 1;
            c->next_lane = 0;
            c->err.clear();
            rcl = KR_OK;
        }
        if (rcl) return rcl;
    }
    Lane& ln = peek_lane(c);
    c->last_lane = c->next_lane;
    c->next_lane = (c->next_lane + 1) % lanes_used(c);
    ln.pending = true;
    hipStream_t st = ln.stream;
    if (G.up_done && st != c->stream) HIPCHK(c, hipStreamWaitEvent(st, G.up_done, 0));
    taken = &ln;
    return KR_OK;
}

static void coarse_pool_step(kr_ctx* c, Genome& G, bool coarse) {
    const size_t cbytes = ((size_t)c->lane_maxcount + 2) * 8;
    if (G.ckeys.p && (!coarse || !c->coarse_pool || G.ckeys.bytes < cbytes)) coarse_pool_return(c, G);
    if (coarse) {
        G.partitions++;
        if (c->coarse_pool && !G.ckeys.p) (void)coarse_pool_take(c, G, cbytes);
    }
}

static void pass_pack(kr_ctx* c, Genome& G, Lane& ln) {
    StageScope sc(c, KR_ST_PACK, ln.stream);
    launch_pack(c, G, ln, ln.stream);
}

static int pass0(kr_ctx* c, Genome& G, const SortPlan& p, Lane& ln) {
    hipStream_t st = ln.stream;
    int rc;
    for (int h = 0; h < SLICE_HELPERS; h++) {
        Lane& hp = c->lanes[p.helper + h];
        if (hp.stream && hp.pending) {
            HIPCHK(c, hipEventRecord(hp.done, hp.stream));
            HIPCHK(c, hipStreamWaitEvent(st, hp.done, 0));
        }
    }
    if (p.route2) {
        if ((rc = ensure(c, ln.partial16, ((size_t)p.h16_ranges << p.nba) * 2 + 64))) return rc;
        if ((rc = ensure_h16exc(c, ln, st))) return rc;
        if ((rc = ensure(c, ln.slt, 1024 * 4))) return rc;
        if ((rc = ensure(c, ln.offa, (((size_t)1 << p.nba) + 4) * 4))) return rc;
        if ((rc = ensure(c, ln.cura, (((size_t)1 << p.nba) + 4) * 4))) return rc;
    }
    if (!p.reuse_count) pass_pack(c, G, ln);
    if ((rc = ensure(c, ln.pass0, (G.nmax + 2) * 8))) return rc;
    if (!p.reuse_count) {
        StageScope sc(c, KR_ST_HIST8, st);
        launch_hist8(c, G, ln, st, pass0_geom(c, true));
    }
    {
        StageScope sc(c, KR_ST_REDUCE8, st);
        if (!p.reuse_count)
            hipLaunchKernelGGL(k_reduce8a, dim3(256), dim3(256), 0, st, (u32*)ln.partial8.p, (u32*)ln.base1.p + 260);
        hipLaunchKernelGGL(k_bases64, dim3(1), dim3(64), 0, st, (const u32*)ln.base1.p + 260, (u64*)ln.base64.p);
    }
    Geom g0 = pass0_geom(c);
    g0.wcmode = (g0.wmode == 2 && g0.wcache) ? p.cached_mode : 0;
    g0.slice = (u32)c->g.sbits;
    {
        StageScope sc(c, KR_ST_SCATTER1, st);
        launch_scatter1(g0, st, (const u64*)ln.codes.p, (const u32*)ln.bad.p, G.nwords, (const u32*)nullptr,
                        (const u64*)ln.base64.p, (const u32*)ln.partial8.p, (u64*)ln.pass0.p, G.nmax);
    }
    if (!p.route2) return KR_OK;
    {
        StageScope sc(c, KR_ST_HIST2, st);
        hipLaunchKernelGGL(k_hist16, dim3(p.h16_ranges, 1), dim3(H16_T), 0, st, (const u64*)ln.codes.p, (const u32*)ln.bad.p,
                           G.nwords, (const u32*)ln.partial8.p, (const u32*)ln.base1.p + 260,
                           (unsigned short*)ln.partial16.p, (u32*)ln.h16exc.p, c->g.k, p.nba);
    }
    StageScope sc(c, KR_ST_SCAN2, st);
    hipLaunchKernelGGL(k_bases_rel, dim3(1), dim3(256), 0, st, (const u32*)ln.base1.p + 260, 256u >> c->g.sbits,
                       (u32*)ln.slt.p);
    hipLaunchKernelGGL(k_hist16_off, dim3(256), dim3(1024), 0, st, (const unsigned short*)ln.partial16.p, p.h16_ranges,
                       p.nba, (const u32*)ln.h16exc.p, (const u32*)ln.slt.p, (u32*)ln.offa.p, (u32*)ln.cura.p);
    return KR_OK;
}

static int slice_lanes_start(kr_ctx* c, const SortPlan& p, Lane& ln) {
    int rcs;
    hipStream_t st = ln.stream;
    hipEvent_t& ready = c->slice_ready[(int)(&ln - c->lanes)];
    if (!ready) HIPCHK(c, hipEventCreateWithFlags(&ready, hipEventDisableTiming));
    HIPCHK(c, hipEventRecord(ready, st));
    for (int h = p.helper; h < p.helper + SLICE_HELPERS; h++) {
        if ((rcs = ensure_slice_lanes(c, h))) return rcs;
        HIPCHK(c, hipStreamWaitEvent(c->lanes[h].stream, ready, 0));
        c->lanes[h].pending = true;
    }
    return KR_OK;
}

static int pass1_target(kr_ctx* c, Genome& G, const SortPlan& p, Lane& ls, Slice& S, u64*& pass1_dst) {
    hipStream_t ss = ls.stream;
    pass1_dst = (c->g.b > 8 && !p.coarse) ? (u64*)ls.tmpkeys.p : (u64*)S.keys.p;
    if (!p.coarse || !G.ckeys.p) return KR_OK;
    pass1_dst = (u64*)G.ckeys.p;
    if (G.ckeys_busy && G.ckeys_busy != ss) coarse_pool_handover(c, G);
    if (G.ckeys_wait) {
        HIPCHK(c, hipStreamWaitEvent(ss, G.ckeys_ev, 0));
        G.ckeys_wait = false;
    }
    G.ckeys_busy = ss;
    c->cpool_partitions++;
    return KR_OK;
}

static void pass1_route2(kr_ctx* c, const SortPlan& p, Lane& ln, Lane& ls, Slice& S, int s, const u64* src, u64* pass1_dst) {
    hipStream_t ss = ls.stream;
    const int b = c->g.b;
    const u32 ntA = (u32)((S.nmax + P2_KEYS - 1) / P2_KEYS);
    if (ntA) {
        StageScope sc(c, KR_ST_SCATTER1, ss);
        launch_scatter2(ss, src, pass1_dst, (const uint2*)nullptr, ntA, (const u32*)nullptr, (u32*)ln.cura.p, p.nba, c->g.sbits,
                        (u32)S.nmax);
    }
    StageScope sc(c, KR_ST_REDUCE8, ss);
    const u32 ntmax = b > 8 ? p2_tiles(S.nmax) : 0u;
    hipLaunchKernelGGL(k_reduce8b, dim3(std::max(1u, (ntmax + 255) / 256)), dim3(256), 0, ss, (const u32*)nullptr,
                       (u32*)ls.base1.p, (u32*)ls.tp.p, b > 8 ? P2_KEYS : 0u, ntmax, (uint2*)ls.tiledesc.p,
                       (const u32*)ln.offa.p + (size_t)s * 256, (u32)S.nmax);
}

static void pass1_counted(kr_ctx* c, Genome& G, const SortPlan& p, Lane& ln, Lane& ls, Slice& S, int s, const u64* src,
                          u64* pass1_dst) {
    hipStream_t ss = ls.stream;
    Geom g = slice_geom(c, (u32)s);
    if (p.cached_keys) g.wcmode = p.cached_mode;
    if (p.sliced) {
        StageScope sc(c, KR_ST_HIST8, ss);
        hipLaunchKernelGGL(k_hist8k, dim3(NWG), dim3(P1_T), 0, ss, src, (u64)S.nmax, g.sbits, (u32*)ln.partial8.p);
    } else if (!p.reuse_count) {
        StageScope sc(c, KR_ST_HIST8, ss);
        launch_hist8(c, G, ln, ss, g);
    }
    {
        StageScope sc(c, KR_ST_REDUCE8, ss);
        if (p.sliced || !p.reuse_count)
            hipLaunchKernelGGL(k_reduce8a, dim3(256), dim3(256), 0, ss, (u32*)ln.partial8.p, (u32*)ls.base1.p + 260);
        const u32 ntmax = (g.b > 8 && !p.coarse) ? p2_tiles(S.nmax) : 0u;
        hipLaunchKernelGGL(k_reduce8b, dim3(std::max(1u, (ntmax + 255) / 256)), dim3(256), 0, ss,
                           (const u32*)ls.base1.p + 260, (u32*)ls.base1.p, (u32*)ls.tp.p, ntmax ? P2_KEYS : 0u, ntmax,
                           (uint2*)ls.tiledesc.p, (const u32*)nullptr, 0u);
    }
    StageScope sc(c, KR_ST_SCATTER1, ss);
    if (p.sliced)
        hipLaunchKernelGGL(k_scatter1kp, dim3(NWG), dim3(P1_T), 0, ss, src, (u64)S.nmax, g.sbits,
                           (const u32*)ls.base1.p, (const u32*)ln.partial8.p, pass1_dst, (u32)S.nmax);
    else
        launch_scatter1(g, ss, (const u64*)ln.codes.p, (const u32*)ln.bad.p, G.nwords, (const u32*)ls.base1.p,
                        (const u64*)nullptr, (const u32*)ln.partial8.p, pass1_dst, S.nmax);
}

static void coarse_exit(kr_ctx* c, Lane& ls, Slice& S) {
    StageScope sc(c, KR_ST_REDUCE8, ls.stream);
    hipLaunchKernelGGL(k_coarse_keep, dim3(1), dim3(320), 0, ls.stream, (const u32*)ls.base1.p, (u32*)S.off.p, 1u << c->g.b,
                       (u32*)S.ovf.p);
}

static int pass2(kr_ctx* c, Genome& G, const SortPlan& p, Lane& ln, Lane& ls, Slice& S) {
    hipStream_t ss = ls.stream;
    const int b = c->g.b;
    const u32 nb = 1u << b;
    if (b <= 8) {
        HIPCHK(c, hipMemcpyAsync(S.off.p, ls.base1.p, 257 * 4, hipMemcpyDeviceToDevice, ss));
        return KR_OK;
    }
    const u32 ntmax = p2_tiles(S.nmax);
    if (p.fine16) {
        {
            StageScope sc(c, KR_ST_HIST2, ss);
            const u32 parts = nb > H16_BINS ? nb / H16_BINS : 1;
            hipLaunchKernelGGL(k_hist16, dim3(H16_RANGES, parts), dim3(H16_T), 0, ss, (const u64*)ln.codes.p,
                               (const u32*)ln.bad.p, G.nwords, (const u32*)ln.partial8.p, (const u32*)ls.base1.p + 260,
                               (unsigned short*)ln.partial16.p, (u32*)ln.h16exc.p, c->g.k, b);
        }
        {
            StageScope sc(c, KR_ST_SCAN2, ss);
            hipLaunchKernelGGL(k_hist16_off, dim3(256), dim3(1024), 0, ss, (const unsigned short*)ln.partial16.p,
                               (u32)H16_RANGES, b, (const u32*)ln.h16exc.p, (const u32*)ls.base1.p, (u32*)S.off.p,
                               (u32*)ls.cursor.p);
        }
        StageScope sc(c, KR_ST_SCATTER2, ss);
        launch_scatter2(ss, (const u64*)ls.tmpkeys.p, (u64*)S.keys.p, (const uint2*)ls.tiledesc.p, ntmax, (const u32*)nullptr,
                        (u32*)ls.cursor.p, b);
        return KR_OK;
    }
    {
        StageScope sc(c, KR_ST_HIST2, ss);
        hipLaunchKernelGGL(k_hist2<2 * P2_T>, dim3(ntmax), dim3(2 * P2_T), 0, ss, (const u64*)ls.tmpkeys.p,
                           (const uint2*)ls.tiledesc.p, (u32*)ls.tilehist.p, b);
    }
    {
        StageScope sc(c, KR_ST_SCAN2, ss);
        hipLaunchKernelGGL(k_scan2, dim3(256), dim3(1024), 0, ss, (u32*)ls.tilehist.p, (const u32*)ls.base1.p,
                           (const u32*)ls.tp.p, (u32*)S.off.p, b);
    }
    StageScope sc(c, KR_ST_SCATTER2, ss);
    launch_scatter2(ss, (const u64*)ls.tmpkeys.p, (u64*)S.keys.p, (const uint2*)ls.tiledesc.p, ntmax, (const u32*)ls.tilehist.p,
                    (u32*)nullptr, b);
    return KR_OK;
}

static void launch_localsort(kr_ctx* c, Slice& S, const DevBuf& desc, u32 ntiles, hipStream_t st) {
    hipLaunchKernelGGL(k_localsort2, dim3(std::min<u32>(ntiles, (u32)c->ls_grid)), dim3(LS_THREADS), 0, st, (u64*)S.keys.p,
                       (const u32*)S.off.p, (const uint4*)desc.p, ntiles, c->g.b, (u32*)S.ovf.p, (uint4*)((char*)S.ovf.p + 16));
}

static void chunks_and_order(kr_ctx* c, const SortPlan& p, Lane& ln, Lane& ls, Slice& S) {
    hipStream_t ss = ls.stream;
    {
        StageScope sc(c, KR_ST_CHUNKS, ss);
        hipLaunchKernelGGL(k_chunk_table, dim3((S.nchunks + 255) / 256), dim3(256), 0, ss, (const u32*)S.off.p, 1u << c->g.b,
                           S.nchunks, (uint4*)S.chunkdesc.p, (u32*)S.ovf.p, (p.fine16 || p.route2) ? (u32*)ln.h16exc.p : (u32*)nullptr);
    }
    if (p.lazy) {
        c->lazy_skipped++;
        return;
    }
    StageScope sc(c, KR_ST_LOCALSORT, ss);
    launch_localsort(c, S, S.chunkdesc, S.nchunks, ss);
}

static int genome_sort(kr_ctx* c, int id, bool reuse_count, bool coarse) {
    if (!c) return KR_ERR_PARAM;
    auto it = c->genomes.find(id);
    if (it == c->genomes.end() || !it->second.uploaded) return fail(c, KR_ERR_STATE, "genome %d not uploaded", id);
    if (it->second.sl.empty()) return fail(c, KR_ERR_STATE, "genome %d has no slice plan (wide windows: use kr_wide_run)", id);
    HIPCHK(c, hipSetDevice(c->device));
    Genome& G = it->second;
    c->sorts_done++;
    int rc;
    Lane* lane;
    if ((rc = take_lane(c, G, lane))) return rc;
    Lane& ln = *lane;
    genome_unsorted(G);
    coarse_pool_step(c, G, coarse);
    const SortPlan p = sort_plan(c, G, ln, reuse_count, coarse);
    if (p.sliced) {
        if ((rc = pass0(c, G, p, ln))) return rc;
    } else if (!reuse_count) {
        pass_pack(c, G, ln);
    }
    if (p.nsl > 1 && (rc = slice_lanes_start(c, p, ln))) return rc;
    u64 region = 0;
    for (int s = 0; s < c->nslices; s++) {
        Slice& S = G.sl[s];
        Lane& ls = (p.nsl > 1 && s % p.nsl) ? c->lanes[p.helper + s % p.nsl - 1] : ln;
        const u64* src = (const u64*)ln.pass0.p + region;
        region += S.nmax;
        S.count = -1;
        u64* pass1_dst;
        if ((rc = pass1_target(c, G, p, ls, S, pass1_dst))) return rc;
        if (p.route2) pass1_route2(c, p, ln, ls, S, s, src, pass1_dst);
        else pass1_counted(c, G, p, ln, ls, S, s, src, pass1_dst);
        if (coarse) {
            coarse_exit(c, ls, S);
            continue;
        }
        if ((rc = pass2(c, G, p, ln, ls, S))) return rc;
        chunks_and_order(c, p, ln, ls, S);
    }
    G.ordered = !p.lazy && !coarse;
    G.sorted = !coarse;
    G.coarse = coarse;
    return KR_OK;
}

static int ensure_fine(kr_ctx* c, Genome& G) {
    if (!G.coarse) return KR_OK;
    c->coarse_promoted++;
    return genome_sort(c, G.id, false);
}
static int ensure_fine_id(kr_ctx* c, int id) {
    auto it = c->genomes.find(id);
    return (it == c->genomes.end()) ? KR_OK : ensure_fine(c, it->second);
}

static void publish_slices(kr_ctx* c, Slice* const* sl, size_t n, hipStream_t st) {
    PubEnt* tab = (PubEnt*)(c->mbox + MB_WORDS);
    const u32 nb = 1u << c->g.b;
    for (size_t i = 0; i < n; i++) {
        tab[i].ovf = (const u32*)sl[i]->ovf.p;
        tab[i].tot = (const u32*)sl[i]->off.p + nb;
        tab[i].res = (u32)sl[i]->res;
        tab[i].pad = 0;
    }
    if (n) hipLaunchKernelGGL(k_publish_slices, dim3((u32)(n + 63) / 64), dim3(64), 0, st, (const PubEnt*)tab, (u32)n, c->mbox + MB_SLICE0);
}

static int order_genome(kr_ctx* c, Genome& G, hipStream_t st) {
    if (!G.sorted || G.ordered) return KR_OK;
    for (Slice& S : G.sl) {
        HIPCHK(c, hipMemsetAsync(S.ovf.p, 0, 16, st));
        StageScope sc(c, KR_ST_LOCALSORT, st);
        launch_localsort(c, S, S.chunkdesc, S.nchunks, st);
        c->lazy_ordered++;
    }
    G.ordered = true;
    G.finalized = false;
    return KR_OK;
}

static int ensure_ordered(kr_ctx* c, const std::vector<Genome*>& gs) {
    bool any = false;
    for (Genome* G : gs) any = any || (G->sorted && !G->ordered);
    if (!any) return KR_OK;
    int rc = join_lanes(c);
    if (rc) return rc;
    for (Genome* G : gs)
        if ((rc = order_genome(c, *G, c->stream))) return rc;
    return KR_OK;
}

static int repair_slice(kr_ctx* c, Slice& S, u32 novf, u32 total, hipStream_t st) {
    StageScope sc(c, KR_ST_FALLBACK);
    const u32 nb = 1u << c->g.b;
    std::vector<uint4> segs;
    uint4* dsegs = (uint4*)((char*)S.ovf.p + 16);
    if (novf > OVF_MAX) {
        segs.push_back(make_uint4(0, total, 0, nb));
    } else {
        segs.resize(novf);
        HIPCHK(c, hipMemcpy(segs.data(), dsegs, (size_t)novf * 16, hipMemcpyDeviceToHost));
        for (auto& sg : segs) sg.w = sg.z + 1;
    }
    c->overflow_segments += (int64_t)segs.size();
    std::vector<uint4> tiles;
    u32 maxlen = 0;
    for (auto& sg : segs) {
        maxlen = std::max(maxlen, sg.y - sg.x);
        for (u32 t = sg.x; t < sg.y; t += LS_CAP) tiles.push_back(make_uint4(t, std::min(t + LS_CAP, sg.y), sg.z, sg.w));
    }
    int rc;
    if ((rc = ensure(c, c->fbdesc, tiles.size() * 16 + 16))) return rc;
    if ((rc = ensure(c, c->fbsegs, (segs.size() + 1) * 16))) return rc;
    HIPCHK(c, hipMemcpy(c->fbdesc.p, tiles.data(), tiles.size() * 16, hipMemcpyHostToDevice));
    HIPCHK(c, hipMemsetAsync(S.ovf.p, 0, 16, st));
    launch_localsort(c, S, c->fbdesc, (u32)tiles.size(), st);
    c->fallback_launches++;
    Lane& ln = c->lanes[0];
    if ((rc = ensure(c, ln.tmpkeys, ((size_t)total + 2) * 8))) return rc;
    for (u64 run = LS_CAP; run < maxlen; run *= 2) {
        std::vector<uint4> act;
        u32 ntiles = 0;
        for (auto& sg : segs) {
            u32 len = sg.y - sg.x;
            if (len <= run) continue;
// ... 223 lines not shown
```

### krisp_amd/csrc/h_intersect.inc

```
static int64_t intersect_once(kr_ctx* c, const int* ids, int n, const uint8_t* is_in, int apply_filter, bool* redo);

static int64_t cands_merge_device(kr_ctx* c, size_t m, int have_other, int apply_filter);

static inline int fmode(const kr_ctx* c, int apply_filter) { return apply_filter ? (c->mixed_alphabets ? 2 : 1) : 0; }

int kr_set_mixed_alphabets(kr_ctx* c, int on) {
    if (!c) return KR_ERR_PARAM;
    c->mixed_alphabets = on != 0;
    return KR_OK;
}

#define KR_MAX_CANDS 0xFFFFFF00ull
static int cands_fit(kr_ctx* c, uint64_t n, const char* who) {
    if (n < KR_MAX_CANDS) return KR_OK;
    return fail(c, KR_ERR_CAPACITY, "%s: a candidate list of %llu entries exceeds the %llu a list may hold (an intersection that "
                "nothing prunes: give both ingroup and outgroup genomes to one call, or fewer genomes per call)", who,
                (unsigned long long)n, (unsigned long long)KR_MAX_CANDS);
}

static int cands_compact_room(kr_ctx* c, u32 n) {
    const size_t nblk = ((size_t)n + 255) / 256;
    int rc;
    if ((rc = ensure(c, c->flags, (size_t)n * 4))) return rc;
    if ((rc = ensure(c, c->blockcnt, (nblk + 2) * 4))) return rc;
    if ((rc = ensure(c, c->blockpos, (nblk + 2) * 4))) return rc;
    return ensure(c, c->candA, ((size_t)n + 2) * sizeof(kr_cand));
}
static const u32* cands_compact_enqueue(kr_ctx* c, u32 n, hipStream_t st, bool publish) {
    const u32 nblk = (n + 255) / 256;
    const u32* total = (const u32*)c->blockpos.p + nblk;
    hipLaunchKernelGGL(k_scan, dim3(1), dim3(1024), 0, st, (const u32*)c->blockcnt.p, (u32*)c->blockpos.p, nblk);
    hipLaunchKernelGGL(k_cands_compact, dim3(nblk), dim3(256), 0, st, (const kr_cand*)c->candB.p, n,
                       (const u32*)c->flags.p, (const u32*)c->blockpos.p, (kr_cand*)c->candA.p);
    if (publish)
        hipLaunchKernelGGL(k_publish, dim3(1), dim3(64), 0, st, total, (const u32*)nullptr, (const u32*)nullptr, c->mbox + 16);
    return total;
}
static int64_t cands_compact_adopt(kr_ctx* c, u32 total) {
    std::swap(c->candA, c->candB);
    c->ncand = total;
    return total;
}

static int64_t intersect_batch(kr_ctx* c, const int* ids, int n, const uint8_t* is_in, int apply_filter) {
    bool redo = false;
    int64_t r = intersect_once(c, ids, n, is_in, apply_filter, &redo);
    if (r >= 0 && redo) r = intersect_once(c, ids, n, is_in, apply_filter, &redo);
    return r;
}

#define KR_COARSE_PASS (-1001)
static int64_t intersect_coarse(kr_ctx* c, const int* ids, int n, const uint8_t* is_in, int apply_filter) {
    std::vector<Genome*> cg;
    std::vector<int> pid, cpos;
    std::vector<uint8_t> pin;
    bool has_in = false, has_out = false;
    for (int i = 0; i < n; i++) {
        auto it = c->genomes.find(ids[i]);
        if (it == c->genomes.end()) return KR_COARSE_PASS;
        if (it->second.coarse) { cg.push_back(&it->second); cpos.push_back(i); }
        else {
            pid.push_back(ids[i]);
            pin.push_back(is_in[i]);
            (is_in[i] ? has_in : has_out) = true;
        }
    }
    if (cg.empty()) return KR_COARSE_PASS;
    const bool ok = apply_filter && fmode(c, apply_filter) == 1 && c->g.D == 1 && n <= CO_MAXG && has_in && has_out &&
                    c->nslices == 1 && !c->wide.on && !c->custom_layout;
    if (!ok) return KR_COARSE_PASS;
    HIPCHK(c, hipSetDevice(c->device));
    const int64_t nC64 = intersect_batch(c, pid.data(), (int)pid.size(), pin.data(), 1);
    if (nC64 <= 0) {
        if (nC64 == 0) c->coarse_done += (int64_t)cg.size();
        return nC64;
    }
    int rc;
    if ((rc = cands_fit(c, (uint64_t)nC64, "kr_intersect"))) return rc;
    const u32 nC = (u32)nC64, nblk = (nC + 255) / 256;
    const Geom g = slice_geom(c, 0);
    hipStream_t st = c->stream;
    const u32 hitcap = c->co_hitcap ? c->co_hitcap : (u32)std::min<u64>(2ull * nC + 65536, 0x7FFFFFF0ull);
    if ((rc = ensure(c, c->co_state, (size_t)nC * 4))) return rc;
    if ((rc = ensure(c, c->co_tab, (size_t)(2 * 260 + 256 * CO_ROW) * 4))) return rc;
    if ((rc = cands_compact_room(c, nC))) return rc;
    for (Genome* G : cg) {
        if (G->hitcap < hitcap || !G->hits.p) {
            if ((rc = ensure(c, G->hits, (size_t)hitcap * 8 + 16))) return rc;
        }
        G->hitcap = hitcap;
        G->hits_valid = false;
    }
    if (c->co_occ == 0) {
        int per = 0;
        const hipError_t e = hipOccupancyMaxActiveBlocksPerMultiprocessor(&per, k_coarse_probe, CO_T, 0);
        c->co_occ = (e == hipSuccess && per >= 1) ? per : 1;
    }
    const u32 grid = c->co_grid ? c->co_grid : (u32)(c->co_occ * c->ncu);
    if ((rc = join_lanes(c))) return rc;
    HIPCHK(c, hipMemsetAsync(c->co_state.p, 0, (size_t)nC * 4, st));
    u32 *cb = (u32*)c->co_tab.p, *ust = cb + 260, *rows = cb + 520;
    u32 need = 0;
    CoarsePub pub{};
    pub.n = (int)cg.size();
    CoarseArgs ca{};
    ca.n = (u32)cg.size();
    for (size_t j = 0; j < cg.size(); j++) {
        Genome& G = *cg[j];
        ca.keys[j] = (const u64*)(G.ckeys.p ? G.ckeys.p : G.sl[0].keys.p);
        ca.off[j] = (const u32*)G.sl[0].off.p;
        ca.hits[j] = (u32*)G.hits.p;
        ca.hitcap[j] = hitcap;
        ca.bit[j] = 8u + (u32)j;
        ca.side[j] = is_in[cpos[j]] ? 0u : 4u;
        need |= 1u << (8 + j);
        pub.cnt[j] = (const u32*)G.hits.p;
    }
    {
        StageScope sc(c, KR_ST_INTERSECT, st);
        hipLaunchKernelGGL(k_coarse_tables, dim3(1), dim3(256), 0, st, (const kr_cand*)c->candB.p, nC, ca, c->co_tcap, cb, ust, rows);
        hipLaunchKernelGGL(k_coarse_probe, dim3(grid), dim3(CO_T), 0, st, ca, (const u32*)cb, (const u32*)ust, (const u32*)rows,
                           (const kr_cand*)c->candB.p, (u32*)c->co_state.p, c->co_tcap, g.pmask, g.LRrel);
    }
    for (Genome* G : cg)
        if (G->ckeys.p) G->ckeys_busy = st;
    {
        StageScope sc(c, KR_ST_MERGE, st);
        hipLaunchKernelGGL(k_coarse_flag, dim3(nblk), dim3(256), 0, st, (kr_cand*)c->candB.p, nC, (const u32*)c->co_state.p, need,
                           fmode(c, 1), (u32*)c->flags.p, (u32*)c->blockcnt.p);
        cands_compact_enqueue(c, nC, st, true);
        hipLaunchKernelGGL(k_coarse_publish, dim3(1), dim3(64), 0, st, pub, c->mbox + 32);
    }
    HIPCHK(c, hipStreamSynchronize(st));
    HIPCHK(c, hipGetLastError());
    for (Genome* G : cg) G->ckeys_busy = nullptr;
    for (size_t j = 0; j < cg.size(); j++)
        if (((volatile u32*)c->mbox)[32 + j] > hitcap) {
            c->ncand = -1;
            return KR_COARSE_PASS;
        }
    const u32 total = ((volatile u32*)c->mbox)[16];
    cands_compact_adopt(c, total);
    for (Genome* G : cg) G->hits_valid = true;
    c->coarse_done += (int64_t)cg.size();
    {
        int want = 0;
        for (Genome* G : cg) want += !G->ckeys.p && G->partitions >= 2;
        if (want > 0) coarse_pool_grow(c, want);
    }
    return total;
}

int64_t kr_intersect(kr_ctx* c, const int* ids, int n, const uint8_t* is_in, int apply_filter) {
    if (!c || n < 1) return fail(c, KR_ERR_PARAM, "kr_intersect: need at least one genome");
    if (c->custom_layout) return fail(c, KR_ERR_STATE, "kr_intersect: this context sorts by a custom field order (kr_set_field_order)");
    {
        bool any_coarse = false;
        for (auto& kv : c->genomes) kv.second.hits_valid = false;
        for (int i = 0; i < n; i++) {
            auto it = c->genomes.find(ids[i]);
            any_coarse = any_coarse || (it != c->genomes.end() && it->second.coarse);
        }
        if (any_coarse) {
            const int64_t r = intersect_coarse(c, ids, n, is_in, apply_filter);
            if (r != KR_COARSE_PASS) return r;
            int rcf;
            for (int i = 0; i < n; i++)
                if ((rcf = ensure_fine_id(c, ids[i]))) return rcf;
        }
    }
    if (n <= MAXG) return intersect_batch(c, ids, n, is_in, apply_filter);
    HIPCHK(c, hipSetDevice(c->device));
    int64_t cur = -1, nprev = 0;
    int rc;
    for (int o = 0; o < n; o += MAXG) {
        const int m = std::min(MAXG, n - o);
        if ((cur = intersect_batch(c, ids + o, m, is_in + o, 0)) < 0) return cur;
        if (o > 0) {
            if ((rc = ensure(c, c->other, ((size_t)nprev + 2) * sizeof(kr_cand)))) return rc;
            if (nprev) HIPCHK(c, hipMemcpyAsync(c->other.p, c->candP.p, (size_t)nprev * sizeof(kr_cand), hipMemcpyDeviceToDevice, c->stream));
            if ((cur = cands_merge_device(c, (size_t)nprev, 1, 0)) < 0) return cur;
        }
        if (o + MAXG < n) {
            if ((rc = ensure(c, c->candP, ((size_t)cur + 2) * sizeof(kr_cand)))) return rc;
            if (cur) HIPCHK(c, hipMemcpyAsync(c->candP.p, c->candB.p, (size_t)cur * sizeof(kr_cand), hipMemcpyDeviceToDevice, c->stream));
            nprev = cur;
        }
    }
    if (apply_filter) cur = cands_merge_device(c, 0, 0, 1);
    return cur;
}

struct ItemPlan {
    int mlog;
    u32 T;
    bool tagk;
    int p0, sht;
};
static ItemPlan item_plan(const kr_ctx* c, const Slice& AS, const Geom& g) {
    const u32 nbk = 1u << c->g.b;
    const double avg = (double)std::max<int64_t>(AS.count >= 0 ? AS.count : (int64_t)AS.nmax, 1) / nbk;
    auto need = [](double mean) { return mean + 6.0 * std::sqrt(mean) + 8.0; };
    ItemPlan p;
    p.mlog = 0;
    while ((2u << p.mlog) <= nbk && need(avg * (2u << p.mlog)) <= (double)I3_SLOTS) p.mlog++;
    p.T = (u32)std::min(512.0, std::max(256.0, 64.0 * std::ceil(need(avg * (1u << p.mlog)) / 256.0)));
    p.p0 = 64 - 2 * g.LRrel;
    p.sht = g.rb + p.mlog - (int)I3T_NB_LOG;
    p.tagk = c->isect_kernel != 2 && p.p0 >= 0 && p.p0 < 32 && p.sht >= 32 && p.sht <= p.p0 + 32;
    return p;
}

typedef void (*Isect3Kernel)(Isect3Args, Geom);
static Isect3Kernel isect3_kernel(bool ua, bool tagk, bool st32, int fmt) {
    static const Isect3Kernel heads32[2][4] = {
        {k_intersect3t<0>, k_intersect3t<1>, k_intersect3t<2>, k_intersect3t<3>},
        {k_intersect3t<0, true>, k_intersect3t<1, true>, k_intersect3t<2, true>, k_intersect3t<3, true>}};
    static const Isect3Kernel heads64[3] = {k_intersect3<0>, k_intersect3<1>, k_intersect3<2>};
// ... 555 lines not shown
```

### krisp_amd/csrc/h_misc.inc

```
double kr_debug_localsort(kr_ctx* c, int id, int reps, int mode) {
    if (!c || mode != 0) return -1.0;
    auto it = c->genomes.find(id);
    if (it != c->genomes.end() && ensure_fine(c, it->second)) return -1.0;
    if (it == c->genomes.end() || !it->second.sorted || it->second.sl.empty()) return -1.0;
    if (ensure_ordered(c, {&it->second}) || finalize(c, {&it->second})) return -1.0;
    Slice& S = it->second.sl[0];
    hipStream_t st = c->stream;
    const u32 grid = std::min<u32>(S.nchunks, (u32)c->ls_grid);
    auto launch = [&]() {
        hipLaunchKernelGGL(k_localsort2, dim3(grid), dim3(LS_THREADS), 0, st, (u64*)S.keys.p, (const u32*)S.off.p,
                           (const uint4*)S.chunkdesc.p, S.nchunks, c->g.b, (u32*)S.ovf.p,
                           (uint4*)((char*)S.ovf.p + 16));
    };
    hipEvent_t a, b;
    (void)hipEventCreate(&a);
    (void)hipEventCreate(&b);
    launch();
    (void)hipEventRecord(a, st);
    for (int r = 0; r < reps; r++) launch();
    (void)hipEventRecord(b, st);
    (void)hipEventSynchronize(b);
    float ms = 0;
    (void)hipEventElapsedTime(&ms, a, b);
    (void)hipEventDestroy(a);
// ... 164 lines not shown
    case 1: src = ln.bad.p; esz = 4; n = G.nwords + 2; break;
    case 2: src = ln.base1.p; esz = 4; n = 257; break;
    case 3: src = S0.off.p; esz = 4; n = nb + 1; break;
    case 4: src = c->g.b > 8 ? ln.tmpkeys.p : S0.keys.p; esz = 8; n = total; break;
    case 5: src = S0.keys.p; esz = 8; n = total; break;
    default: return fail(c, KR_ERR_PARAM, "kr_debug_fetch: unknown selector %d", what);
    }
    if (n * esz > cap_bytes) return fail(c, KR_ERR_CAPACITY, "debug buffer too small");
    if (n) HIPCHK(c, hipMemcpy(out, src, n * esz, hipMemcpyDeviceToHost));
    return (int64_t)n;
}

int64_t kr_debug_inversions(kr_ctx* c, int id) {
    if (!c) return KR_ERR_PARAM;
    auto it = c->genomes.find(id);
    if (it != c->genomes.end()) { int rcf = ensure_fine(c, it->second); if (rcf) return rcf; }
    if (it == c->genomes.end() || !it->second.sorted) return fail(c, KR_ERR_STATE, "genome %d not sorted", id);
    HIPCHK(c, hipSetDevice(c->device));
    int rc = ensure_ordered(c, {&it->second});
    if (rc) return rc;
    if ((rc = finalize(c, {&it->second}))) return rc;
    if ((rc = ensure(c, c->nrec, 16))) return rc;
    HIPCHK(c, hipMemset(c->nrec.p, 0, 16));
    for (Slice& S : it->second.sl)
        if (S.count > 1)
            hipLaunchKernelGGL(k_count_inversions, dim3(4096), dim3(256), 0, c->stream, (const u64*)S.keys.p,
                               (u64)S.count, (u64*)c->nrec.p);
    u64 bad = 0;
    HIPCHK(c, hipMemcpy(&bad, c->nrec.p, 8, hipMemcpyDeviceToHost));
    HIPCHK(c, hipGetLastError());
    return (int64_t)bad;
}

int kr_mem_info(kr_ctx* c, int64_t* out4) {
    if (!c || !out4) return KR_ERR_PARAM;
    HIPCHK(c, hipSetDevice(c->device));
    size_t fr = 0, tot = 0;
    HIPCHK(c, hipMemGetInfo(&fr, &tot));
    int64_t avail = (int64_t)fr;
    if (c->budget) avail = std::min<int64_t>(avail, (int64_t)c->budget - (int64_t)c->used);
    out4[0] = std::max<int64_t>(avail, 0);
    out4[1] = (int64_t)tot;
    out4[2] = (int64_t)c->used;
    out4[3] = (int64_t)c->budget;
    return KR_OK;
}
int64_t kr_debug_budget_left(kr_ctx* c) { return !c ? KR_ERR_PARAM : (c->budget ? (int64_t)c->budget - (int64_t)c->used : -1); }
int kr_debug_budget_set(kr_ctx* c, int64_t left) {
    if (!c || left < 0) return KR_ERR_PARAM;
    c->budget = c->used + (size_t)left;
    return KR_OK;
}

int kr_debug_place(kr_ctx* c, double* out8) {
    if (!c || !out8) return KR_ERR_PARAM;
    out8[0] = c->place_n;
    out8[1] = c->place_taken;
    for (int i = 0; i < 6; i++) out8[2 + i] = c->place_ms[i];
    return KR_OK;
}

int kr_debug_coarse_pool(kr_ctx* c, double* out8) {
    if (!c || !out8) return KR_ERR_PARAM;
    int held = 0;
    double lo = 0, hi = 0;
    for (auto& kv : c->genomes) {
        const Genome& G = kv.second;
        if (!G.ckeys.p) continue;
        lo = held ? std::min(lo, G.ckeys_ms) : G.ckeys_ms;
        hi = held ? std::max(hi, G.ckeys_ms) : G.ckeys_ms;
        held++;
    }
    out8[0] = c->cpool_total;
    out8[1] = (double)c->cpool_free.size();
    out8[2] = held;
    out8[3] = (double)c->cpool_partitions;
    out8[4] = (double)c->cpool_searches;
    out8[5] = lo;
    out8[6] = hi;
    out8[7] = c->coarse_pool;
    return KR_OK;
}

int kr_debug_isect(kr_ctx* c, int64_t* o) {
    if (!c || !o) return KR_ERR_PARAM;
    o[0] = c->isect_ovf_items;
    o[1] = c->isect_refall;
    o[2] = c->i3_last_T;
    o[3] = c->i3_last_mlog;
    o[4] = c->i3_last_tags;
    o[5] = lanes_used(c);
    o[6] = c->j2_launches;
    o[7] = c->j2_full;
    return KR_OK;
}

int kr_debug_scan(kr_ctx* c, int64_t* o) {
    if (!c || !o) return KR_ERR_PARAM;
    o[0] = c->scan_dbg[0];
    o[1] = c->scan_dbg[1];
    o[2] = c->scan_cap;
    o[3] = c->scan_dbg[2];
    o[4] = o[5] = o[6] = o[7] = 0;
    return KR_OK;
}

int kr_build_experiments(void) {
    int bits = 0;
#ifdef KR_EXPERIMENTS
    bits |= 1;
#endif
#ifdef KR_ABLATE
    bits |= 2;
#endif
#if defined(I3_ABL) && I3_ABL
    bits |= 4;
#endif
#if defined(P2_ABL) && P2_ABL
    bits |= 8;
#endif
#ifdef LS2_NORANK
    bits |= 16;
#endif
#ifdef KR_EXP_NOLOOKUP
    bits |= 32;
#endif
#ifdef KR_EXP_MZONLY
    bits |= 64;
#endif
    return bits;
}

int kr_debug_lazy(kr_ctx* c, int64_t* o) {
    if (!c || !o) return KR_ERR_PARAM;
    o[0] = c->lazy_skipped;
    o[1] = c->lazy_ordered;
    o[2] = c->lazy_touch;
    o[3] = c->lazy_order;
    o[4] = c->isect_ua;
    o[5] = c->fuse_anchor;
    o[6] = c->coarse_done;
    o[7] = c->coarse_promoted;
    return KR_OK;
}

int kr_debug_info(kr_ctx* c, int64_t* o) {
    if (!c || !o) return KR_ERR_PARAM;
    o[0] = c->g.b;
    o[1] = 1ll << c->g.b;
    o[2] = LS_T;
    o[3] = LS_CAP;
    o[4] = NWG;
    o[5] = c->overflow_segments;
    o[6] = c->fallback_launches;
    o[7] = (int64_t)c->nslices;
    return KR_OK;
}
```

### krisp_amd/csrc/k_coarse.inc

```

#include "co_units.inc"

#define CO_T 1024
#define CO_SLOT_LOG 13
#define CO_SLOTS (1u << CO_SLOT_LOG)
#define CO_BM_LOG 17
#define CO_QCAP 2048
#define CO_TCAP 6144
#define CO_EMPTY 0xFFFFFFFFu
#define CO_UNROLL 4
#define CO_ITER (2u * CO_T * CO_UNROLL)
#define CO_HB 1024
#define CO_MAXG 24
#define CO_ROW (2 * CO_MAXG)

struct CoarseArgs {
    const u64* keys[CO_MAXG];
    const u32* off[CO_MAXG];
    u32* hits[CO_MAXG];
    u32 hitcap[CO_MAXG];
    u32 bit[CO_MAXG];
    u32 side[CO_MAXG];
    u32 n;
};

__device__ __forceinline__ u32 co_hash(u64 pre) {
    const u32 y = (u32)pre * 0x9E3779B1u;
    return ((u32)(pre >> 32) ^ y) * 0x85EBCA6Bu;
}

__global__ __launch_bounds__(256) void k_coarse_tables(const kr_cand* __restrict__ cands, u32 n, CoarseArgs A, u32 tcap,
                                                       u32* __restrict__ cb, u32* __restrict__ ust, u32* rows) {
    __shared__ u32 waves[17];
    __shared__ u32 s_cb[257];
    for (u32 t = threadIdx.x; t <= 256; t += 256) {
        u32 l = 0, r = n;
        if (t == 256) l = n;
        else {
            const u64 bound = (u64)t << 56;
            while (l < r) {
                const u32 mid = l + ((r - l) >> 1);
                if (cands[mid].prefix < bound) l = mid + 1; else r = mid;
            }
        }
        s_cb[t] = l;
        cb[t] = l;
    }
    __syncthreads();
    const u32 t = threadIdx.x;
    if (t < 4 * A.n) A.hits[t >> 2][t & 3u] = 0;
    u32* row = rows + t * CO_ROW;
    for (u32 j = 0; j < A.n; j++) {
        row[2 * j] = A.off[j][t];
        row[2 * j + 1] = A.off[j][t + 1];
    }
    const u32 units = co_byte_units(s_cb[t + 1] - s_cb[t], tcap, row, A.n);
    u32 total;
    const u32 ex = block_excl_scan(units, waves, total);
    ust[t] = ex;
    if (t == 0) ust[256] = total;
}

__device__ __forceinline__ void co_lookup(u64 key, u64 pmask, int LR, const u32* slots, u32 c0, const kr_cand* __restrict__ cands,
                                          u32* __restrict__ state, u32 orbits, u32 side_shift, u64* s_hit, u32* s_nhit,
                                          u32* __restrict__ hits, u64* __restrict__ hitkeys, u32 hitcap) {
    const u64 pre = key & pmask;
    const u32 h = co_hash(pre);
    const u32 tag = h & 0x7FFFFu;
    u32 s = h >> (32 - CO_SLOT_LOG);
    for (u32 w = slots[s]; w != CO_EMPTY; w = slots[s]) {
        if ((w & 0x7FFFFu) == tag) {
            const u32 ci = c0 + (w >> 19);
            if (cands[ci].prefix == pre) {
                const u32 at0 = atomicAdd(s_nhit, 1u);
                if (at0 < CO_HB) s_hit[at0] = key;
                else {
                    const u32 pos = atomicAdd(hits, 1u);
                    if (pos < hitcap) hitkeys[pos] = key;
                }
                const u32 bb = (u32)(key >> (62 - 2 * LR)) & 3u;
                atomicOr(&state[ci], orbits | (1u << (side_shift + bb)));
                return;
            }
        }
        s = (s + 1) & (CO_SLOTS - 1);
    }
}

__device__ __forceinline__ void co_load(u32x4 (&v)[CO_UNROLL], const u64* __restrict__ keys, u32 p0, u32 a0, u32 k1) {
#pragma unroll
    for (int q = 0; q < CO_UNROLL; q++) {
        const u32 p = p0 + 2 * (q * CO_T + threadIdx.x);
        const u32 pc = p < k1 ? p : a0;
        v[q] = __builtin_nontemporal_load(reinterpret_cast<const u32x4*>(keys + pc));
    }
}

#define CO_RFL(x) ((u32)__builtin_amdgcn_readfirstlane((int)(x)))

__global__ __launch_bounds__(CO_T, 8) void k_coarse_probe(CoarseArgs A, const u32* __restrict__ cb, const u32* __restrict__ ust,
                                                       const u32* __restrict__ rows, const kr_cand* __restrict__ cands,
                                                       u32* __restrict__ state, u32 tcap, u64 pmask, int LR) {
    __shared__ u32 slots[CO_SLOTS];
    __shared__ u32 bitmap[1u << (CO_BM_LOG - 5)];
    __shared__ u32 s_ust[257];
    __shared__ u32 s_bnd[CO_ROW];
    __shared__ u64 s_q[CO_QCAP];
    __shared__ u64 s_hit[CO_HB];
    __shared__ u32 s_nhit, s_hbase, s_qn;
    if (threadIdx.x == 0) { s_nhit = 0; s_qn = 0; }
    for (u32 t = threadIdx.x; t <= 256; t += CO_T) s_ust[t] = ust[t];
    __syncthreads();
    const u32 G = A.n;
    const u32 U = s_ust[256];
    const u32 u0 = (u32)(((u64)blockIdx.x * U) / gridDim.x), u1 = (u32)(((u64)(blockIdx.x + 1) * U) / gridDim.x);
    if (u0 >= u1) return;
    const u32 lane = threadIdx.x & 63u;
    u32 u = u0, t = 0, ust_t = 0, ust_t1 = 0, k0 = 0, k1 = 0, p0 = 0, c0 = 0;
    u32 cur_t = ~0u, cur_r = ~0u;
    const u64* __restrict__ kp = nullptr;
    u32* __restrict__ hits = nullptr;
    u64* __restrict__ hitkeys = nullptr;
    u32 hitcap = 0, orbits = 0, side_shift = 0;
    bool cold = true;

    auto adopt = [&](const CoUnit& un) {
        const u32 g = un.genome, r = un.round;
        k0 = un.k0;
        k1 = un.k1;
        p0 = k0 & ~1u;
        kp = A.keys[g];
        hits = A.hits[g];
        hitkeys = (u64*)(hits + 4);
        hitcap = A.hitcap[g];
        orbits = 1u << A.bit[g];
        side_shift = A.side[g];
        if (t != cur_t || r != cur_r) {
            cur_t = t;
            cur_r = r;
            for (u32 i = threadIdx.x; i < CO_SLOTS; i += CO_T) slots[i] = CO_EMPTY;
            for (u32 i = threadIdx.x; i < (1u << (CO_BM_LOG - 5)); i += CO_T) bitmap[i] = 0;
            __syncthreads();
            const u32 cb0 = cb[t], cb1 = cb[t + 1];
            c0 = cb0 + r * tcap;
            const u32 c1 = cb1 - c0 > tcap ? c0 + tcap : cb1;
            for (u32 i = c0 + threadIdx.x; i < c1; i += CO_T) {
                const u32 h = co_hash(cands[i].prefix);
                const u32 word = ((i - c0) << 19) | (h & 0x7FFFFu);
                u32 s = h >> (32 - CO_SLOT_LOG);
                while (atomicCAS(&slots[s], CO_EMPTY, word) != CO_EMPTY) s = (s + 1) & (CO_SLOTS - 1);
                atomicOr(&bitmap[h >> (37 - CO_BM_LOG)], 1u << ((h >> (32 - CO_BM_LOG)) & 31u));
            }
            __syncthreads();
        }
    };
    auto uniform = [](CoUnit un) {
        un.round = CO_RFL(un.round); un.genome = CO_RFL(un.genome); un.chunk = CO_RFL(un.chunk);
        un.k0 = CO_RFL(un.k0); un.k1 = CO_RFL(un.k1);
        return un;
    };
    auto new_byte = [&]() {
        t = CO_RFL(co_unit_byte(s_ust, u));
        ust_t = CO_RFL(s_ust[t]);
        ust_t1 = CO_RFL(s_ust[t + 1]);
        if (threadIdx.x < 2 * G) s_bnd[threadIdx.x] = rows[t * CO_ROW + threadIdx.x];
        __syncthreads();
        adopt(uniform(co_unit_decode(u - ust_t, s_bnd, G)));
    };

    auto step = [&](u32x4 (&V)[CO_UNROLL], u32x4 (&NV)[CO_UNROLL]) -> bool {
        const bool last = k1 - p0 <= CO_ITER;
        bool ahead = false;
        CoUnit un = {};
        const u64* __restrict__ nkp = kp;
        u32 np0 = p0 + CO_ITER, na0 = k0 & ~1u, nk1 = k1;
        if (last) {
            np0 = na0;
            nk1 = 0;
            if (u + 1 < u1 && u + 1 < ust_t1) {
                un = uniform(co_unit_decode(u + 1 - ust_t, s_bnd, G));
                nkp = A.keys[un.genome];
                np0 = na0 = un.k0 & ~1u;
                nk1 = un.k1;
                ahead = true;
            }
        }
        if (cold) co_load(V, kp, p0, p0, k1);
        cold = false;
        co_load(NV, nkp, np0, na0, nk1);
        __builtin_amdgcn_sched_barrier(0);
        const int hi = (int)(k1 - p0) - 2 * (int)threadIdx.x;
        const bool front = p0 < k0 && threadIdx.x == 0;
#pragma unroll
        for (int q = 0; q < CO_UNROLL; q++) {
#pragma unroll
            for (int e = 0; e < 2; e++) {
                const u64 key = e ? ((u64)V[q].w << 32 | V[q].z) : ((u64)V[q].y << 32 | V[q].x);
                const u32 h = co_hash(key & pmask);
                const u32 bw = bitmap[h >> (37 - CO_BM_LOG)];
                const u32 inr = (u32)(2 * q * (int)CO_T + e < hi) & (u32)!(q == 0 && e == 0 && front);
                const bool mine = ((bw >> ((h >> (32 - CO_BM_LOG)) & 31u)) & inr) != 0;
                const u64 bal = __builtin_amdgcn_ballot_w64(mine);
                if (bal) {
                    u32 qb = 0;
                    if (lane == 0) qb = atomicAdd(&s_qn, (u32)__popcll(bal));
                    qb = CO_RFL(qb);
                    const u32 qa = qb + __builtin_amdgcn_mbcnt_hi((u32)(bal >> 32), __builtin_amdgcn_mbcnt_lo((u32)bal, 0u));
                    if (mine && qa < CO_QCAP) s_q[qa] = key;
                }
            }
        }
        if (!last) { p0 += CO_ITER; return false; }
        __syncthreads();
        if (s_qn <= CO_QCAP) {
            const u32 qn = s_qn;
            for (u32 i = threadIdx.x; i < qn; i += CO_T)
                co_lookup(s_q[i], pmask, LR, slots, c0, cands, state, orbits, side_shift, s_hit, &s_nhit, hits, hitkeys, hitcap);
        } else {
            const u32 a0 = k0 & ~1u;
            for (u32 p = a0 + 2 * threadIdx.x; p < k1; p += 2 * CO_T) {
                const u32x4 w = *reinterpret_cast<const u32x4*>(kp + p);
#pragma unroll
                for (int e = 0; e < 2; e++) {
                    const u64 key = e ? ((u64)w.w << 32 | w.z) : ((u64)w.y << 32 | w.x);
                    const u32 h = co_hash(key & pmask);
                    if (p + e >= k0 && p + e < k1 && ((bitmap[h >> (37 - CO_BM_LOG)] >> ((h >> (32 - CO_BM_LOG)) & 31u)) & 1u))
                        co_lookup(key, pmask, LR, slots, c0, cands, state, orbits, side_shift, s_hit, &s_nhit, hits, hitkeys, hitcap);
                }
            }
        }
        __syncthreads();
        const u32 m = min(s_nhit, (u32)CO_HB);
        __syncthreads();
        if (threadIdx.x == 0) {
            s_qn = 0;
            s_nhit = 0;
            if (m) s_hbase = atomicAdd(hits, m);
        }
        if (m) {
            __syncthreads();
            const u32 hb = s_hbase;
            for (u32 i = threadIdx.x; i < m; i += CO_T)
                if (hb + i < hitcap) hitkeys[hb + i] = s_hit[i];
        }
        __syncthreads();
        if (++u >= u1) return true;
        if (ahead) adopt(un);
        else {
            new_byte();
            cold = true;
        }
        return false;
    };

    u32x4 va[CO_UNROLL], vb[CO_UNROLL];
    new_byte();
    for (;;) {
        if (step(va, vb)) break;
        if (step(vb, va)) break;
    }
}

__global__ void k_coarse_flag(kr_cand* __restrict__ cur, u32 n, const u32* __restrict__ state, u32 need, int mode,
                              u32* __restrict__ flags, u32* __restrict__ blockcnt) {
    __shared__ u32 waves[17];
    const u32 i = blockIdx.x * blockDim.x + threadIdx.x;
    bool keep = false;
    if (i < n) {
        const u32 st = state[i];
        keep = (st & need) == need;
        if (keep) {
            kr_cand c = cur[i];
            c.in_mask |= st & 15u;
            c.out_mask |= (st >> 4) & 15u;
            keep = passes_filter(c.in_mask, c.out_mask, 1, mode);
            if (keep) cur[i] = c;
        }
        flags[i] = keep ? 1u : 0u;
    }
    u32 tot;
    block_compact(keep, waves, tot);
    if (threadIdx.x == 0) blockcnt[blockIdx.x] = tot;
}

struct CoarsePub { const u32* cnt[CO_MAXG]; int n; };
__global__ void k_coarse_publish(CoarsePub p, u32* __restrict__ host) {
    if (blockIdx.x == 0 && (int)threadIdx.x < p.n) host[threadIdx.x] = *p.cnt[threadIdx.x];
}

__global__ __launch_bounds__(256) void k_coarse_rows(const u32* __restrict__ hits, u32 hitcap, const kr_cand* __restrict__ cands,
                                                     u32 nc, u32 n, u32 gi, u64 pmask, u64* __restrict__ arena,
                                                     u32* __restrict__ mcnt) {
    const u32 nh = min(hits[0], hitcap);
    const u64* __restrict__ hk = (const u64*)(hits + 4);
    for (u32 i = blockIdx.x * blockDim.x + threadIdx.x; i < nh; i += gridDim.x * blockDim.x) {
        const u64 key = hk[i], pre = key & pmask;
        u32 l = 0, r = nc;
        while (l < r) {
            const u32 mid = l + ((r - l) >> 1);
            if (cands[mid].prefix < pre) l = mid + 1; else r = mid;
        }
        if (l < nc && cands[l].prefix == pre) {
            const u32 row = l * n + gi;
            const u32 at = atomicAdd(&mcnt[row], 1u);
            if (at < COL_CAPM) arena[(u64)row * COL_CAPM + at] = key;
        }
    }
}

__global__ __launch_bounds__(256) void k_coarse_rowsort(u32 npairs, u32 n, const u32* __restrict__ ibo, u64* __restrict__ arena,
                                                        u32* __restrict__ mcnt, u32* __restrict__ overflow) {
    const u32 idx = blockIdx.x * blockDim.x + threadIdx.x;
    if (idx >= npairs || ibo[idx % n] != 2u) return;
    const u32 m = mcnt[idx];
    if (m > COL_CAPM) {
        atomicAdd(overflow, 1u);
        mcnt[idx] = 0;
        return;
    }
    u64* __restrict__ K = arena + (u64)idx * COL_CAPM;
    for (u32 i = 1; i < m; i++) {
        const u64 key = K[i];
        u32 j = i;
        for (; j > 0 && K[j - 1] > key; j--) K[j] = K[j - 1];
        K[j] = key;
    }
}

__global__ void k_coarse_keep(const u32* __restrict__ base1, u32* __restrict__ off, u32 nb, u32* __restrict__ ovf) {
    const u32 t = threadIdx.x;
    if (t <= 256) off[t] = base1[t];
    else if (t == 257) off[nb] = base1[256];
    else if (t == 258) ovf[0] = 0;
}
```

### krisp_amd/csrc/k_sort.inc

```
__device__ __forceinline__ u32 bytes_equal(u32 v, u32 k4) {
    const u32 z = v ^ k4;
    return ~(((z & 0x7F7F7F7Fu) + 0x7F7F7F7Fu) | z) & 0x80808080u;
}
__device__ __forceinline__ void pack4(u32 w, int omit, u32 allow, u32& code8, u32& bad4) {
    const u32 up = w & 0xDFDFDFDFu;
    u32 x = (up >> 1) & 0x03030303u;
    x ^= (x >> 1) & 0x01010101u;
    u32 ok = bytes_equal(up, 0x41414141u) | bytes_equal(up, 0x43434343u) | bytes_equal(up, 0x47474747u) |
             bytes_equal(up, 0x54545454u);
    if (omit) ok &= ~((w & 0x20202020u) << 2);
    if (allow != 15u) {
#pragma unroll
        for (u32 c = 0; c < 4; c++)
            if (!((allow >> c) & 1u)) ok &= ~bytes_equal(x, c * 0x01010101u);
    }
    x &= (ok >> 7) | (ok >> 6);
    code8 = ((x << 6) | (x >> 4) | (x >> 14) | (x >> 24)) & 0xFFu;
    const u32 nb = ~ok & 0x80808080u;
    bad4 = ((nb >> 4) | (nb >> 13) | (nb >> 22) | (nb >> 31)) & 0xFu;
}

__global__ void k_pack(const uint8_t* __restrict__ bases, u64 n, u64* __restrict__ codes,
                       u32* __restrict__ bad, u64 nwords_padded, int omit, u32 allow) {
    u64 w = (u64)blockIdx.x * blockDim.x + threadIdx.x;
// ... 9 lines not shown
            u32 hi = 0, lo = 0;
#pragma unroll
            for (int q = 0; q < 8; q++) {
                u32 c8, b4;
                pack4(wd[q], omit, allow, c8, b4);
                if (q < 4) hi |= c8 << (24 - 8 * q); else lo |= c8 << (56 - 8 * q);
                bd |= b4 << (28 - 4 * q);
            }
            c = ((u64)hi << 32) | lo;
        } else {
            for (int q = 0; q < 32; q++) {
                u32 code = 0;
                bool ok = false;
                if (base + q < n) {
                    u32 ch = bases[base + q];
                    u32 up = ch & 0xDF;
                    code = (up >> 1) & 3;
                    code ^= code >> 1;
                    ok = (up == 'A') | (up == 'C') | (up == 'G') | (up == 'T');
                    if (omit) ok = ok & (ch == up);
                    ok = ok & ((allow >> code) & 1u);
                }
                c = (c << 2) | (ok ? code : 0);
                bd = (bd << 1) | (ok ? 0u : 1u);
            }
        }
        codes[w] = c;
        bad[w] = bd;
    }
}


template <int OFF>
__device__ __forceinline__ u32 bits128(const u32 (&w)[5]) {
    constexpr int q = OFF >> 5, r = OFF & 31;
    return r ? __funnelshift_l(w[q + 1], w[q], r) : w[q];
}
__device__ __forceinline__ u32 word_invalid(u32 b0, u32 b1, int k) {
    u64 R = ((u64)b0 << 32) | b1;
    for (int span = 1; span < k;) {
        const int st = span < k - span ? span : k - span;
        R |= R << st;
        span += st;
    }
    return (u32)(R >> 32);
}
__device__ __forceinline__ u32 revcomp16(u32 x) {
    const u32 y = __brev(~x);
    return ((y & 0xAAAAAAAAu) >> 1) | ((y & 0x55555555u) << 1);
}
__device__ __forceinline__ void word_revstring(u64 c0, u64 c1, int k, u32 (&sf)[5], u32 (&rv)[5]) {
    sf[0] = (u32)(c0 >> 32); sf[1] = (u32)c0; sf[2] = (u32)(c1 >> 32); sf[3] = (u32)c1; sf[4] = 0;
    const u64 r0 = ((u64)revcomp16((u32)c1) << 32) | revcomp16((u32)(c1 >> 32));
    const u64 r1 = ((u64)revcomp16((u32)c0) << 32) | revcomp16((u32)(c0 >> 32));
    const int sl = 66 - 2 * k;
    u64 q0, q1;
    if (sl >= 64) { q0 = r1; q1 = 0; }
    else { q0 = (r0 << sl) | (r1 >> (64 - sl)); q1 = r1 << sl; }
    rv[0] = (u32)(q0 >> 32); rv[1] = (u32)q0; rv[2] = (u32)(q1 >> 32); rv[3] = (u32)q1; rv[4] = 0;
}

__device__ __forceinline__ bool top16_in_slice(u32 t16, const Geom& g, u32& d1) {
    if (g.sbits && (t16 >> (16 - g.sbits)) != g.slice) return false;
    d1 = (t16 >> (8 - g.sbits)) & 0xFFu;
    return true;
}

template <int J>
__device__ __forceinline__ void hist8_window(const u32 (&sf)[5], const u32 (&rv)[5], u32 invalid, const Geom& g,
                                             u32* lhist) {
    if ((invalid >> (31 - J)) & 1u) return;
    const u32 tf = bits128<2 * J>(sf) >> 16;
    const u32 tr = bits128<62 - 2 * J>(rv) >> 16;
    u32 d1;
    if (top16_in_slice(tf, g, d1)) atomicAdd(&lhist[d1], 1u);
    if (top16_in_slice(tr, g, d1)) atomicAdd(&lhist[d1], 1u);
}
template <int... J>
__device__ __forceinline__ void hist8_word(std::integer_sequence<int, J...>, const u32 (&sf)[5], const u32 (&sr)[5],
                                           u32 invalid, const Geom& g, u32* lhist) {
    (hist8_window<J>(sf, sr, invalid, g, lhist), ...);
}

template <int WIDE>
__global__ __launch_bounds__(P1_T) void k_hist8(const u64* __restrict__ codes, const u32* __restrict__ bad,
                                               u64 nwords, u32* __restrict__ partial8, Geom g) {
    __shared__ u32 lhist[256];
    if (threadIdx.x < 256) lhist[threadIdx.x] = 0;
    __syncthreads();
    u64 wpw = (nwords + NWG - 1) / NWG;
    u64 w0 = (u64)blockIdx.x * wpw;
    u64 w1 = w0 + wpw < nwords ? w0 + wpw : nwords;
    const bool cheap = g.L >= 8;
    for (u64 w = w0 + threadIdx.x; w < w1; w += P1_T) {
        u32 b0 = bad[w], b1 = bad[w + 1];
        if (b0 == 0xFFFFFFFFu) continue;
        u64 c0 = codes[w], c1 = codes[w + 1];
        if (WIDE == 2) {
#pragma unroll 4
            for (int j = 0; j < 32; j++) {
                u64 k1;
                if (window_key_single(c0, c1, b0, b1, j, g, k1) && slice_key(k1, g))
                    atomicAdd(&lhist[(u32)(k1 >> 56)], 1u);
            }
            continue;
        }
        if (cheap) {
            u32 sf[5], rv[5];
            word_revstring(c0, c1, g.k, sf, rv);
            hist8_word(std::make_integer_sequence<int, 32>{}, sf, rv, word_invalid(b0, b1, g.k), g, lhist);
        } else {
#pragma unroll 4
            for (int j = 0; j < 32; j++) {
                u64 kf, kr;
                if (!window_keys(c0, c1, b0, b1, j, g, kf, kr)) continue;
                if (slice_key(kf, g)) atomicAdd(&lhist[(u32)(kf >> 56)], 1u);
                if (slice_key(kr, g)) atomicAdd(&lhist[(u32)(kr >> 56)], 1u);
            }
        }
    }
    __syncthreads();
    if (threadIdx.x < 256) partial8[P8(blockIdx.x, threadIdx.x)] = lhist[threadIdx.x];
}

#ifndef H8W_PPT
#define H8W_PPT 4
#endif
#define H8W_HALO 512
template <int WM>
__global__ __launch_bounds__(P1_T) void k_hist8w(const u64* __restrict__ codes, const u32* __restrict__ bad,
                                                u64 nwords, u32* __restrict__ partial8, Geom g) {
    __shared__ u32 lhist[256];
    __shared__ u32 lcount;
    if (threadIdx.x < 256) lhist[threadIdx.x] = 0;
    if (threadIdx.x == 0) lcount = 0;
    __syncthreads();
    const u64 wpw = (nwords + NWG - 1) / NWG;
    const u64 w0 = (u64)blockIdx.x * wpw;
    const u64 w1 = w0 + wpw < nwords ? w0 + wpw : nwords;
    if (WM == 2 && g.wshare && g.wfl[0].np == 1 && g.wfl[0].d[0].canon && g.wk - g.wfl[0].len <= H8W_HALO) {
        __shared__ u32 sF[H8W_PPT * P1_T], sR[H8W_PPT * P1_T];
        const FlankRank& F = g.wfl[0];
        const int len = F.len, halo = g.wk - len;
        const u32 tid = threadIdx.x;
        const u32 TP = H8W_PPT * P1_T, TW = TP - (u32)halo;
        for (u64 base = w0 * 32; base < w1 * 32; base += TW) {
            u32 idf[H8W_PPT], idr[H8W_PPT];
#pragma unroll
            for (int q = 0; q < H8W_PPT; q++) {
                const u64 p = base + tid + q * P1_T;
                idf[q] = idr[q] = ~0u;
                if ((p >> 5) < nwords && range_valid(bad, p, len) && !canon_ids(codes, p + g.woff[0], len, F.d[0], idf[q], idr[q]))
                    idf[q] = idr[q] = ~0u;
            }
#pragma unroll
            for (int q = 0; q < H8W_PPT; q++) {
                sF[tid + q * P1_T] = idf[q];
                sR[tid + q * P1_T] = idr[q];
            }
            __syncthreads();
#pragma unroll
            for (int q = 0; q < H8W_PPT; q++) {
                const u32 t = tid + q * P1_T;
                const u64 pos = base + t;
                if (t < TW && pos < w1 * 32) {
                    const u32 a = sF[t], b = sR[t + halo];
                    u64 kf = ~0ull, kr = 0;
                    const bool ok = a != ~0u && b != ~0u && range_valid(bad, pos, g.wk);
                    if (ok) {
                        kf = ((u64)min(a, b) << g.wshL) | ((u64)max(a, b) << g.wshR);
                        kr = (a > b ? 1ull : 0ull) | (a == b ? 2ull : 0ull);
                    }
                    if (g.wcmode == 1) {
                        ulonglong2 v;
                        v.x = kf;
                        v.y = kr;
                        *reinterpret_cast<ulonglong2*>(g.wcache + 2 * pos) = v;
                    } else if (g.wcmode == 3 && ok) {
                        const u32 at = atomicAdd(&lcount, 1u);
                        if (at < g.wlcap) {
// ... 758 lines not shown
```

### krisp_amd/csrc/k_sort2.inc

```
template <int NW>
__device__ __forceinline__ u32 block_excl_scan1(u32 v, u32* lds_waves , u32& total) {
    const int lane = threadIdx.x & 63, wave = threadIdx.x >> 6;
    const u32 x = wave_incl_scan(v);
    if (lane == 63) lds_waves[wave] = x;
    __syncthreads();
    u32 before = 0, tot = 0;
#pragma unroll
    for (int i = 0; i < NW; i++) {
        const u32 t = lds_waves[i];
        before += i < wave ? t : 0u;
        tot += t;
    }
    total = tot;
    return before + x - v;
}

#define LS2_PAIRS (LS_CAP / 2 / LS_THREADS)
#define LS2_NW (LS_THREADS / 64)
#ifndef LS2_OCC
#define LS2_OCC 6
#endif
#define LS2_OVL 64

struct LsRegs { u32x4 q[LS2_PAIRS]; };
// ... 112 lines not shown
            for (u32 jj = k2 >> 1; jj > 0; jj >>= 1) {
                for (u32 t = tid; t < np / 2; t += LS_THREADS) {
                    const u32 i0 = ((t & ~(jj - 1)) << 1) | (t & (jj - 1));
                    const u32 i1 = i0 | jj;
                    const bool up = (i0 & k2) == 0;
                    const u64 a = S[i0], c2 = S[i1];
                    if ((a > c2) == up) { S[i0] = c2; S[i1] = a; }
                }
                __syncthreads();
            }
        }
#pragma unroll
        for (int q = 0; q < 2 * (int)LS2_PAIRS; q++) {
            const u32 p = tid + q * LS_THREADS;
            kk[q] = S[p < m ? p : 0];
            rk[q] = p;
        }
    }
    const bufrsrc ws = make_rsrc(keys + s, m * 8);
#pragma unroll
    for (int q = 0; q < 2 * (int)LS2_PAIRS; q++) {
        const u32 p = tid + q * LS_THREADS;
        buf_store_u64<KR_LS_ST_AUX>(kk[q], ws, p < m ? rk[q] * 8 : BUF_OOB);
    }
}

__global__ __launch_bounds__(LS_THREADS, LS2_OCC) void k_localsort2(u64* keys, const u32* __restrict__ off,
                                                                    const uint4* __restrict__ desc, u32 nchunks, int b,
                                                                    u32* __restrict__ ovf_count,
                                                                    uint4* __restrict__ ovf_list) {
    __shared__ __attribute__((aligned(16))) u64 S[LS_CAP];
    __shared__ __attribute__((aligned(16))) u32 cnt[2][LS_NB / 2 + 4];
    __shared__ u32 waves[LS2_NW];
    __shared__ u32 flag[2];
    __shared__ uint4 ovl[LS2_OVL];
    __shared__ u32 novl;
    const u32 tid = threadIdx.x;
    const u32 G = gridDim.x;
    const int rb = 64 - b;
    auto chunk = [&](u32 jj) {
        uint4 dd = desc[jj < nchunks ? jj : nchunks - 1];
        const u32 keep = jj < nchunks ? ~0u : 0u;
        dd.x &= keep; dd.y &= keep; dd.z &= keep; dd.w &= keep;
        return dd;
    };
    for (u32 i = tid; i < LS_NB / 2; i += LS_THREADS) cnt[0][i] = 0;
    if (tid == 0) { flag[0] = 0; flag[1] = 0; novl = 0; }
    u32 j = blockIdx.x;
    uint4 d0 = chunk(j);
    uint4 d1 = chunk(j + G);
    LsRegs A, B;
    ls2_issue(A, keys, d0);
    {
        const bufrsrc none = make_rsrc(keys, 0);
#pragma unroll
        for (int q = 0; q < 2 * (int)LS2_PAIRS; q++) buf_store_u64(0, none, 64u * q);
    }
    __syncthreads();
    for (; j < nchunks; j += 2 * G) {
        const uint4 d2 = chunk(j + 2 * G);
        ls2_issue(B, keys, d1);
        ls2_process(A, keys, off, d0, rb, S, cnt[0], cnt[1], waves, &flag[0], &flag[1], ovl, &novl);
        const uint4 d3 = chunk(j + 3 * G);
        ls2_issue(A, keys, d2);
        ls2_process(B, keys, off, d1, rb, S, cnt[1], cnt[0], waves, &flag[1], &flag[0], ovl, &novl);
        d0 = d2;
        d1 = d3;
    }
    __syncthreads();
    if (tid == 0 && novl) {
        const u32 n = novl;
        if (n > LS2_OVL) {
            atomicAdd(ovf_count, OVF_MAX + 1u);
        } else {
            const u32 idx = atomicAdd(ovf_count, n);
            for (u32 i = 0; i < n; i++)
                if (idx + i < OVF_MAX) ovf_list[idx + i] = ovl[i];
        }
    }
}

struct P1Regs { u32x4 c; u32x2 b; };

__device__ __forceinline__ void p1_issue(P1Regs& r, bufrsrc cs, bufrsrc bs, u64 wt) {
    const u32 w = (u32)wt + opaque_tid() / P1_TPW;
    r.c = __builtin_amdgcn_raw_buffer_load_b128(cs, w * 8, 0, 0);
    r.b = __builtin_amdgcn_raw_buffer_load_b64(bs, w * 4, 0, 0);
    __builtin_amdgcn_sched_barrier(0);
}

#define P0_DIGIT_BITS(g) ((int)(g).slice)

__device__ __forceinline__ void p1_fast_keys(u64 c0, u64 c1, u32 b0, u32 b1, const Geom& g, u64 (&key)[P1_KPT], u32& vm) {
    static_assert(P1_PPT <= 16, "a thread's windows must start inside one dword of the shifted strings");
    const u32 q = opaque_tid() % P1_TPW;
    const int cs = 2 * P1_PPT * (int)q;
    const u64 f01 = cs ? (c0 << cs) | (c1 >> (64 - cs)) : c0;
    const u32 f0 = (u32)(f01 >> 32), f1 = (u32)f01, f2 = (u32)((c1 << cs) >> 32);
    u32 sf[5], rv[5];
    word_revstring(c0, c1, g.k, sf, rv);
    (void)sf;
    const u64 q0 = ((u64)rv[0] << 32) | rv[1], q1 = ((u64)rv[2] << 32) | rv[3];
    const int ro = 64 - 2 * P1_PPT * ((int)q + 1);
    const u64 y01 = ro ? (q0 << ro) | (q1 >> (64 - ro)) : q0;
    const u32 y0 = (u32)(y01 >> 32), y1 = (u32)y01, y2 = (u32)((q1 << ro) >> 32);
    const u64 B = (((u64)b0 << 32) | b1) << (P1_PPT * q);
    const u32 bh = (u32)(B >> 32), bl = (u32)B;
    const u32 mLh = (u32)(g.mL >> 32), mLl = (u32)g.mL, mRl = (u32)g.mR, mDl = (u32)g.mD;
    const u32 sR = (u32)g.sR & 31u, sD = (u32)g.sD & 31u, vsh = 32u - (u32)g.k;
#pragma unroll
    for (int jj = 0; jj < P1_PPT; jj++) {
        const u32 bm = __funnelshift_l(bl, bh, jj);
        const u32 fh = __funnelshift_l(f1, f0, 2 * jj), fl = __funnelshift_l(f2, f1, 2 * jj);
        const u32 rh = __funnelshift_l(y1, y0, 2 * (P1_PPT - 1 - jj)), rl = __funnelshift_l(y2, y1, 2 * (P1_PPT - 1 - jj));
        key[2 * jj] = ((u64)(fh & mLh) << 32) | ((fl & mLl) | ((fl << sR) & mRl) | ((fl >> sD) & mDl));
        key[2 * jj + 1] = ((u64)(rh & mLh) << 32) | ((rl & mLl) | ((rl << sR) & mRl) | ((rl >> sD) & mDl));
        vm |= (bm >> vsh) == 0u ? 3u << (2 * jj) : 0u;
    }
}

template <int WIDE, int BIG, int FAST = 0>
__device__ __forceinline__ void p1_tile(const P1Regs& R, u64 wt, u64 w1, const Geom& g, bufrsrc ds, u64* dst,
                                        u64 sink, u64* stage, u64* cur, u32* cnt, u32* cnt_next, u64* delta,
                                        u32* waves) {
    const u32 tid = opaque_tid();
    const int dsh = BIG ? 64 - P0_DIGIT_BITS(g) : 56;
    const u64 w = wt + tid / P1_TPW;
    const int j0 = (tid % P1_TPW) * P1_PPT;
    u64 key[P1_KPT];
    u32 rp[P1_KPT / 2];
    u32 vm = 0;
#pragma unroll
    for (int q = 0; q < P1_KPT; q++) { key[q] = 0; if ((q & 1) == 0) rp[q >> 1] = 0; }
    if (w < w1) {
        const u32 b0 = R.b.x, b1 = R.b.y;
        if (b0 != 0xFFFFFFFFu) {
            const u64 c0 = pair_lo(R.c), c1 = pair_hi(R.c);
            if (FAST) {
                p1_fast_keys(c0, c1, b0, b1, g, key, vm);
            } else if (WIDE == 2) {
#pragma unroll
                for (int jj = 0; jj < P1_PPT; jj++) {
                    u64 k1;
                    if (window_key_single(c0, c1, b0, b1, j0 + jj, g, k1)) {
                        key[2 * jj] = k1;
                        vm |= 1u << (2 * jj);
                    }
                }
            } else {
#pragma unroll
                for (int jj = 0; jj < P1_PPT; jj++) {
                    u64 kf, kr;
                    if (window_keys(c0, c1, b0, b1, j0 + jj, g, kf, kr)) {
                        key[2 * jj] = kf;
                        key[2 * jj + 1] = kr;
                        vm |= 3u << (2 * jj);
                    }
                }
            }
        }
    }
#pragma unroll
    for (int q = 0; q < P1_KPT; q++)
        if ((vm >> q) & 1) rp[q >> 1] |= atomicAdd(&cnt[(u32)(key[q] >> dsh)], 1u) << (16 * (q & 1));
    __syncthreads();
    const u32 c = tid < 256 ? cnt[tid] : 0;
    u32 total;
    const u32 ex = block_excl_scan1<P1_T / 64>(c, waves, total);
    if (tid < 256) {
        cnt[tid] = ex;
        delta[tid] = cur[tid] - ex;
        cur[tid] += c;
        cnt_next[tid] = 0;
    }
    __syncthreads();
#pragma unroll
    for (int q = 0; q < P1_KPT; q++)
        if ((vm >> q) & 1) stage[cnt[(u32)(key[q] >> dsh)] + ((rp[q >> 1] >> (16 * (q & 1))) & 0xFFFFu)] = key[q];
    __syncthreads();
#pragma unroll
    for (int q = 0; q < P1_KPT; q++) {
        const u32 p = q * P1_T + tid;
        const u64 k2 = stage[p];
        const u64 o = p + delta[(u32)(k2 >> dsh)];
        if (BIG) dst[p < total ? o : sink] = k2;
        else buf_store_u64<KR_P1_ST_AUX>(k2, ds, p < total ? (u32)o * 8 : BUF_OOB);
    }
}

template <int WIDE, int BIG, int FAST = 0>
__global__ __launch_bounds__(P1_T, P1_OCC) void k_scatter1p(const u64* __restrict__ codes, const u32* __restrict__ bad,
                                                            u64 nwords, const u32* __restrict__ base1,
                                                            const u64* __restrict__ base64,
                                                            const u32* __restrict__ rowoff, u64* dst, u64 dst_keys,
                                                            Geom g) {
    __shared__ __attribute__((aligned(16))) u64 stage[P1_STAGE];
    __shared__ u64 cur[256];
    __shared__ u32 cnt[2][256];
    __shared__ u64 delta[256];
    __shared__ u32 waves[P1_T / 64];
    const u32 tid = threadIdx.x;
    if (tid < 256) {
        if (BIG) {
            const u32 per = 256u >> P0_DIGIT_BITS(g);
            u64 at = 0;
            if (tid * per < 256u) {
                at = base64[tid * per];
                for (u32 j = 0; j < per; j++) at += rowoff[P8(blockIdx.x, tid * per + j)];
            }
            cur[tid] = at;
        } else {
            cur[tid] = (u64)base1[tid] + rowoff[P8(blockIdx.x, tid)];
        }
        cnt[0][tid] = 0;
    }
    const u64 wpw = (nwords + NWG - 1) / NWG;
    const u64 w0 = (u64)blockIdx.x * wpw;
    const u64 w1 = w0 + wpw < nwords ? w0 + wpw : nwords;
    const bufrsrc cs = make_rsrc(codes, (u32)(nwords + PAD_WORDS) * 8);
    const bufrsrc bs = make_rsrc(bad, (u32)(nwords + PAD_WORDS) * 4);
    const bufrsrc ds = make_rsrc(dst, BIG ? 0u : (u32)dst_keys * 8);
    const u64 sink = dst_keys + 1;
    P1Regs A, B;
    p1_issue(A, cs, bs, w0);
    {
        const bufrsrc none = make_rsrc(dst, 0);
#pragma unroll
        for (int q = 0; q < P1_KPT; q++) buf_store_u64(0, none, 64u * q);
    }
    __syncthreads();
    for (u64 wt = w0; wt < w1; wt += 2 * P1_WORDS) {
        p1_issue(B, cs, bs, wt + P1_WORDS);
        p1_tile<WIDE, BIG, FAST>(A, wt, w1, g, ds, dst, sink, stage, cur, cnt[0], cnt[1], delta, waves);
        p1_issue(A, cs, bs, wt + 2 * P1_WORDS);
        p1_tile<WIDE, BIG, FAST>(B, wt + P1_WORDS, w1, g, ds, dst, sink, stage, cur, cnt[1], cnt[0], delta, waves);
    }
}

struct P1kRegs { u32x4 q[P1_KPT / 2]; };

__device__ __forceinline__ void p1k_issue(P1kRegs& r, const u64* src, u64 t0, u64 k1) {
    const u32 tid = opaque_tid();
    const u32 n = t0 < k1 ? (u32)min((u64)P1K_TILE, k1 - t0) : 0u;
    const bufrsrc rs = make_rsrc(src + (t0 < k1 ? t0 : 0), ((n + 1) & ~1u) * 8);
#pragma unroll
    for (int i = 0; i < P1_KPT / 2; i++)
        r.q[i] = __builtin_amdgcn_raw_buffer_load_b128(rs, (tid + i * P1_T) * 16, 0, 0);
    __builtin_amdgcn_sched_barrier(0);
}
#define P1K_KEY(r, e) ((((e) & 1) ? pair_hi((r).q[(e) >> 1]) : pair_lo((r).q[(e) >> 1])) << sbits)
#define P1K_POS(e) (2u * (tid + ((e) >> 1) * P1_T) + ((e) & 1))

__device__ __forceinline__ void p1k_tile(const P1kRegs& R, u64 t0, u64 k1, int sbits, bufrsrc ds, u64* stage, u32* cur,
                                         u32* cnt, u32* cnt_next, u32* delta, u32* waves) {
    const u32 tid = opaque_tid();
    const u32 nt = t0 < k1 ? (u32)min((u64)P1K_TILE, k1 - t0) : 0u;
    u32 rp[P1_KPT / 2];
#pragma unroll
    for (int q = 0; q < P1_KPT; q++) {
        if ((q & 1) == 0) rp[q >> 1] = 0;
        if (P1K_POS(q) < nt) rp[q >> 1] |= atomicAdd(&cnt[(u32)(P1K_KEY(R, q) >> 56)], 1u) << (16 * (q & 1));
    }
    __syncthreads();
    const u32 c = tid < 256 ? cnt[tid] : 0;
    u32 total;
    const u32 ex = block_excl_scan1<P1_T / 64>(c, waves, total);
    if (tid < 256) {
        cnt[tid] = ex;
        delta[tid] = cur[tid] - ex;
        cur[tid] += c;
        cnt_next[tid] = 0;
    }
    __syncthreads();
#pragma unroll
    for (int q = 0; q < P1_KPT; q++)
        if (P1K_POS(q) < nt)
            stage[cnt[(u32)(P1K_KEY(R, q) >> 56)] + ((rp[q >> 1] >> (16 * (q & 1))) & 0xFFFFu)] = P1K_KEY(R, q);
    __syncthreads();
#pragma unroll
    for (int q = 0; q < P1_KPT; q++) {
        const u32 p = q * P1_T + tid;
        const u64 k2 = stage[p];
        const u32 o = p + delta[(u32)(k2 >> 56)];
        buf_store_u64(k2, ds, p < nt ? o * 8 : BUF_OOB);
    }
}

__global__ __launch_bounds__(P1_T, P1_OCC) void k_scatter1kp(const u64* __restrict__ src, u64 n, int sbits,
                                                             const u32* __restrict__ base1,
                                                             const u32* __restrict__ rowoff, u64* dst, u32 dst_keys) {
    __shared__ __attribute__((aligned(16))) u64 stage[P1_STAGE];
    __shared__ u32 cur[256];
    __shared__ u32 cnt[2][256];
    __shared__ u32 delta[256];
    __shared__ u32 waves[P1_T / 64];
    const u32 tid = threadIdx.x;
    if (tid < 256) {
        cur[tid] = base1[tid] + rowoff[P8(blockIdx.x, tid)];
        cnt[0][tid] = 0;
    }
    const u64 per = ((n + NWG - 1) / NWG + P1K_TILE - 1) / P1K_TILE * P1K_TILE;
    const u64 k0 = (u64)blockIdx.x * per;
    const u64 k1 = k0 + per < n ? k0 + per : n;
    const bufrsrc ds = make_rsrc(dst, dst_keys * 8);
    P1kRegs A, B;
    p1k_issue(A, src, k0, k1);
    {
        const bufrsrc none = make_rsrc(dst, 0);
#pragma unroll
        for (int q = 0; q < P1_KPT; q++) buf_store_u64(0, none, 64u * q);
    }
    __syncthreads();
    for (u64 t0 = k0; t0 < k1; t0 += 2 * (u64)P1K_TILE) {
        p1k_issue(B, src, t0 + P1K_TILE, k1);
        p1k_tile(A, t0, k1, sbits, ds, stage, cur, cnt[0], cnt[1], delta, waves);
        p1k_issue(A, src, t0 + 2 * (u64)P1K_TILE, k1);
        p1k_tile(B, t0 + P1K_TILE, k1, sbits, ds, stage, cur, cnt[1], cnt[0], delta, waves);
    }
// ... 2 lines not shown
```

### krisp_amd/csrc/krisp_hip.hip

```cpp
#include <hip/hip_runtime.h>
#include <rccl/rccl.h>
#include <dlfcn.h>
#include <sys/stat.h>
#include <zlib.h>
#include <unistd.h>

#include <algorithm>
#include <atomic>
#include <chrono>
#include <cstdarg>
#include <cstdio>
#include <cstdlib>
#include <cstring>
#include <cmath>
#include <condition_variable>
#include <cerrno>
#include <map>
#include <memory>
#include <mutex>
#include <string>
#include <thread>
#include <utility>
#include <vector>

#include "krisp_hip.h"

#include "k_keys.inc"
#include "k_sort.inc"
#include "k_sort2.inc"
#include "k_intersect.inc"
#include "k_intersect3.inc"
#include "k_intersect3t.inc"
#include "k_join2.inc"
#include "k_text.inc"
#include "k_inflate.inc"
#include "k_gunzip.inc"
#include "k_wide.inc"
#include "k_scan.inc"
#include "k_locate.inc"
#include "k_near.inc"
#include "k_guide_hits.inc"
#include "k_guide_bulges.inc"

#include "k_products.inc"
#include "k_primers.inc"
#include "k_assay.inc"
#include "k_design.inc"
#include "k_coarse.inc"
#include "k_guides.inc"
#include "h_core.inc"
#include "h_intersect.inc"
#include "h_wide.inc"
#include "h_scan.inc"
#include "h_locate.inc"
#include "h_near.inc"
#include "h_guide_hits.inc"
#include "h_guide_bulges.inc"
#include "h_products.inc"
#include "h_primers.inc"
#include "h_assay.inc"
#include "h_design.inc"
#include "h_guides.inc"
#include "h_pgzip.inc"
#include "h_ingest.inc"
#include "h_gunzip.inc"
#include "h_comm.inc"
#include "h_text.inc"
#include "h_misc.inc"

}
```

Before: 122.5 billion.

## Partition only forward-strand k-mers in coarse path and probe reverse complements

Adds a one-strand mode for the coarse partition path. Only forward-strand windows are histogrammed and scattered, using a new digit function and a forward-only key builder that handles twice the positions per thread. At intersect time the candidate table is built per strand class, so reverse-complement matches are found by probing with rev-comp patterns. This roughly halves the k-mers written and sorted, at the cost of extra count, table and fill kernels plus more complex probe lookups.

```diff
diff --git a/include/krisp_hip.h b/include/krisp_hip.h
--- a/include/krisp_hip.h
+++ b/include/krisp_hip.h
@@ -228,6 +228,7 @@
        KR_OPT_COARSE_REST = 11,
        KR_OPT_COARSE_POOL = 12,
        KR_OPT_JOIN2 = 13,
+       KR_OPT_COARSE_ONE_STRAND = 14,
        KR_OPT_WIDE_ORDERED = 6 };
 int     kr_set_option(kr_ctx*, int option, int64_t value);
 
@@ -252,6 +253,7 @@
 int     kr_debug_scan(kr_ctx*, int64_t* out8);
 int     kr_debug_place(kr_ctx*, double* out8);
 int     kr_debug_coarse_pool(kr_ctx*, double* out8);
+int     kr_debug_coarse_strand(kr_ctx*, int64_t* out8);
 int     kr_debug_comm(kr_ctx*, int64_t* out8);
 int     kr_debug_comm_probe(kr_ctx*, size_t bytes, int reps, double* out3);
 int64_t kr_debug_cands_selfexchange(kr_ctx*, int apply_filter);
diff --git a/krisp_amd/_native.py b/krisp_amd/_native.py
--- a/krisp_amd/_native.py
+++ b/krisp_amd/_native.py
@@ -44,6 +44,7 @@
 OPT_COARSE_REST = 11
 OPT_COARSE_POOL = 12
 OPT_JOIN2 = 13
+OPT_COARSE_ONE_STRAND = 14
 ERR_KEY, ERR_HOST = -5, -6
 STRANDS_BOTH, STRANDS_FORWARD, STRANDS_CANONICAL = 0, 1, 2
 STAGES = ["pack", "hist8", "reduce8", "scatter1", "hist2", "scan2", "scatter2", "chunks", "localsort",
@@ -173,6 +174,7 @@
     ("kr_debug_comm", _c.c_int, [_P, _P]),
     ("kr_debug_place", _c.c_int, [_P, _P]),
     ("kr_debug_coarse_pool", _c.c_int, [_P, _P]),
+    ("kr_debug_coarse_strand", _c.c_int, [_P, _P]),
     ("kr_debug_comm_probe", _c.c_int, [_P, _c.c_size_t, _c.c_int, _P]),
     ("kr_debug_cands_selfexchange", _c.c_int64, [_P, _c.c_int]),
     ("kr_debug_info", _c.c_int, [_P, _P]),
@@ -894,6 +896,12 @@
         return dict(candidates=int(o[0]), taken=int(o[1]), fastest_ms=[round(float(x), 4) for x in o[2:6]],
                     median_ms=round(float(o[6]), 4), slowest_ms=round(float(o[7]), 4))
 
+    def debug_coarse_strand(self):
+        o = np.zeros(8, dtype=np.int64)
+        self._check(self.lib.kr_debug_coarse_strand(self.ctx, _ptr(o)), "kr_debug_coarse_strand")
+        return dict(partitions=int(o[0]), calls=int(o[1]), rounds_forward=int(o[2]), rounds_reverse=int(o[3]),
+                    last_forward=int(o[4]), last_reverse=int(o[5]), on=int(o[6]))
+
     def debug_coarse_pool(self):
         o = np.zeros(8, dtype=np.float64)
         self._check(self.lib.kr_debug_coarse_pool(self.ctx, _ptr(o)), "kr_debug_coarse_pool")
diff --git a/krisp_amd/csrc/co_strand.inc b/krisp_amd/csrc/co_strand.inc
--- /dev/null
+++ b/krisp_amd/csrc/co_strand.inc
@@ -0,0 +1,65 @@
+#include <stdint.h>
+
+struct CoStrand {
+    int L, R, k;
+    uint64_t mL, mR, mD;
+    int sR, sD;
+    uint64_t pmask, mask_rc;
+    int dhi, dlo;
+    uint32_t dlow;
+};
+
+__host__ __device__ inline uint64_t cs_topbits(int n) { return n <= 0 ? 0ull : (n >= 64 ? ~0ull : ~0ull << (64 - n)); }
+
+__host__ __device__ inline CoStrand cs_make(int L, int R) {
+    CoStrand S;
+    S.L = L; S.R = R; S.k = L + 1 + R;
+    S.mL = cs_topbits(2 * L);
+    S.mR = cs_topbits(2 * (L + R)) & ~S.mL;
+    S.mD = cs_topbits(2 * S.k) & ~cs_topbits(2 * (L + R));
+    S.sR = 2;
+    S.sD = 2 * R;
+    S.pmask = cs_topbits(2 * (L + R));
+    S.mask_rc = cs_topbits(2 * S.k) & ~(3ull << (62 - 2 * R));
+    const int rc = R < 4 ? R : 4;
+    S.dhi = 32 - 2 * rc;
+    S.dlo = 8 - 2 * rc;
+    S.dlow = (1u << S.dlo) - 1u;
+    return S;
+}
+
+__host__ __device__ inline uint32_t cs_digit(const CoStrand& S, uint64_t key) {
+    const uint32_t hi = (uint32_t)(key >> 32);
+    const uint32_t front = S.dhi >= 32 ? 0u : (hi >> S.dhi) << S.dlo;
+    return front | ((hi >> 22) & S.dlow);
+}
+__host__ __device__ inline uint32_t cs_class_fwd(const CoStrand& S, uint64_t prefix) { return cs_digit(S, prefix); }
+
+__host__ __device__ inline uint64_t cs_revcomp32(uint64_t x) {
+    x = ~x;
+    x = ((x >> 2) & 0x3333333333333333ull) | ((x & 0x3333333333333333ull) << 2);
+    x = ((x >> 4) & 0x0F0F0F0F0F0F0F0Full) | ((x & 0x0F0F0F0F0F0F0F0Full) << 4);
+    return __builtin_bswap64(x);
+}
+__host__ __device__ inline uint64_t cs_revcomp(uint64_t x, int len) { return cs_revcomp32(x) << (64 - 2 * len); }
+
+__host__ __device__ inline uint64_t cs_layout(const CoStrand& S, uint64_t w) {
+    return (w & S.mL) | ((w << S.sR) & S.mR) | ((w >> S.sD) & S.mD);
+}
+__host__ __device__ inline uint64_t cs_unlayout(const CoStrand& S, uint64_t key) {
+    return (key & S.mL) | ((key & S.mR) >> S.sR) | ((key & S.mD) << S.sD);
+}
+
+__host__ __device__ inline uint32_t cs_class_rev(const CoStrand& S, uint64_t prefix) {
+    return (uint32_t)(cs_revcomp(prefix, S.L + S.R) >> 56);
+}
+
+__host__ __device__ inline uint64_t cs_pattern_rev(const CoStrand& S, uint64_t prefix) {
+    const uint64_t s = cs_revcomp(prefix, S.L + S.R);
+    const uint64_t front = cs_topbits(2 * S.R);
+    return cs_layout(S, (s & front) | ((s & ~front) >> 2));
+}
+
+__host__ __device__ inline uint64_t cs_rev_key(const CoStrand& S, uint64_t key) {
+    return cs_layout(S, cs_revcomp(cs_unlayout(S, key), S.k));
+}
diff --git a/krisp_amd/csrc/h_core.inc b/krisp_amd/csrc/h_core.inc
--- a/krisp_amd/csrc/h_core.inc
+++ b/krisp_amd/csrc/h_core.inc
@@ -26,6 +26,7 @@
     bool uploaded = false, sorted = false, finalized = false;
     bool ordered = false;
     bool coarse = false;
+    bool one_strand = false;
     DevBuf ckeys;
     double ckeys_ms = 0;
     hipStream_t ckeys_busy = nullptr;
@@ -131,6 +132,9 @@
     DevBuf touchdesc, touchovf;
     int coarse_rest = 1;
     int64_t coarse_done = 0, coarse_promoted = 0;
+    int coarse_one = 1;
+    int64_t one_partitions = 0, one_calls = 0, one_rounds[2] = {0, 0}, one_last[2] = {0, 0};
+    DevBuf co_ent;
     int coarse_pool = 1;
     struct PoolBuf { DevBuf buf; double ms; hipEvent_t ev; bool wait; };
     std::vector<PoolBuf> cpool_free;
@@ -470,7 +474,7 @@
     G.sl.assign(c->nslices, Slice());
 }
 static void genome_unsorted(Genome& G) {
-    G.sorted = G.finalized = G.ordered = G.coarse = G.hits_valid = false;
+    G.sorted = G.finalized = G.ordered = G.coarse = G.one_strand = G.hits_valid = false;
     G.count = -1;
 }
 
@@ -603,6 +607,8 @@
         c->coarse_rest = e17 ? atoi(e17) != 0 : 1;
         const char* e21 = getenv("KR_COARSE_POOL");
         c->coarse_pool = e21 ? atoi(e21) != 0 : 1;
+        const char* e26 = getenv("KR_COARSE_ONE_STRAND");
+        c->coarse_one = e26 ? atoi(e26) != 0 : 1;
         const char* e22 = getenv("KR_PLACE_MIN_BYTES");
         if (e22) c->place_min_bytes = (size_t)std::max(0ll, atoll(e22));
         const char* e18 = getenv("KR_COARSE_TCAP");
@@ -674,7 +680,7 @@
                      &c->chunkpos, &c->flags, &c->blockcnt, &c->blockpos, &c->other, &c->records, &c->nrec, &c->fbdesc, &c->fbsegs,
                      &c->coltab, &c->collo, &c->colcnt, &c->colpos, &c->coltsum, &c->coltpos, &c->colfirst, &c->colfm, &c->isovf,
                      &c->bgz_in, &c->bgz_tab, &c->bgz_stat, &c->tx_scan, &c->tx_text, &c->tx_tile, &c->tx_tilepos, &c->tx_lines, &c->tx_ls, &c->tx_ll, &c->tx_op, &c->tx_outpos, &c->tx_state,
-                     &c->tx_tsum, &c->tx_tpos, &c->candP, &c->touchdesc, &c->touchovf, &c->co_state, &c->co_tab};
+                     &c->tx_tsum, &c->tx_tpos, &c->candP, &c->touchdesc, &c->touchovf, &c->co_state, &c->co_tab, &c->co_ent};
     for (DevBuf* b : all) release(c, *b);
     {
         kr_ctx::Bufs sb;
@@ -832,6 +838,10 @@
         if (value != 0 && value != 1) return fail(c, KR_ERR_PARAM, "KR_OPT_COARSE_POOL: 0 or 1");
         c->coarse_pool = (int)value;
         return KR_OK;
+    case KR_OPT_COARSE_ONE_STRAND:
+        if (value != 0 && value != 1) return fail(c, KR_ERR_PARAM, "KR_OPT_COARSE_ONE_STRAND: 0 or 1");
+        c->coarse_one = (int)value;
+        return KR_OK;
     case KR_OPT_JOIN2:
         if (value != 0 && value != 1) return fail(c, KR_ERR_PARAM, "KR_OPT_JOIN2: 0 or 1");
         c->join2 = (int)value;
@@ -1148,12 +1158,20 @@
                        (u64*)ln.codes.p, (u32*)ln.bad.p, nwp, c->g.omit, c->g.allow);
 }
 
+static bool p1_fast_on() {
+    static const bool on = [] { const char* e = getenv("KR_P1_FAST"); return e ? atoi(e) != 0 : true; }();
+    return on;
+}
+static bool p1_fast_form(const Geom& g) {
+    return p1_fast_on() && g.wmode == 0 && g.strands == 0 && g.rot == 0 && g.npc == 0 && (u32)((g.mR | g.mD) >> 32) == 0u;
+}
 static void launch_scatter1(const Geom& g, hipStream_t st, const u64* codes, const u32* bad, u64 nwords,
-                            const u32* base1, const u64* base64, const u32* rowoff, u64* dst, u64 dst_keys) {
+                            const u32* base1, const u64* base64, const u32* rowoff, u64* dst, u64 dst_keys, bool one = false) {
     const bool big = base64 != nullptr;
-    static const bool fast_on = [] { const char* e = getenv("KR_P1_FAST"); return e ? atoi(e) != 0 : true; }();
-    const bool fast = fast_on && g.wmode == 0 && g.strands == 0 && g.rot == 0 && g.npc == 0 && (u32)((g.mR | g.mD) >> 32) == 0u;
-    if (g.wmode && g.wmode != 1 && g.wcmode == 4) {
+    const bool fast = p1_fast_form(g);
+    if (one) {
+        hipLaunchKernelGGL((k_scatter1p<0, 0, 1, 1>), dim3(NWG), dim3(P1_T), 0, st, codes, bad, nwords, base1, base64, rowoff, dst, dst_keys, g);
+    } else if (g.wmode && g.wmode != 1 && g.wcmode == 4) {
         hipLaunchKernelGGL(k_scatter1l, dim3(NWG), dim3(P1_T), 0, st, base1, base64, rowoff, dst, g);
     } else if (g.wmode) {
         const auto kw = g.wmode == 1 ? k_scatter1w<1> : g.wcmode == 2 ? k_scatter1w<3> : k_scatter1w<2>;
@@ -1170,8 +1188,8 @@
     hipLaunchKernelGGL(k_scatter2<2 * P2_T>, dim3(ntmax), dim3(2 * P2_T), 0, st, src, dst, tiledesc, tilehist, cursor, b, shl, region_n);
 }
 
-static void launch_hist8(kr_ctx* c, Genome& G, Lane& ln, hipStream_t st, const Geom& g) {
-    const auto kh = g.wmode == 1 ? k_hist8w<1> : g.wmode ? (g.wcmode == 2 ? k_hist8w<3> : k_hist8w<2>) : g.strands ? k_hist8<2> : k_hist8<0>;
+static void launch_hist8(kr_ctx* c, Genome& G, Lane& ln, hipStream_t st, const Geom& g, bool one = false) {
+    const auto kh = one ? k_hist8<3> : g.wmode == 1 ? k_hist8w<1> : g.wmode ? (g.wcmode == 2 ? k_hist8w<3> : k_hist8w<2>) : g.strands ? k_hist8<2> : k_hist8<0>;
     hipLaunchKernelGGL(kh, dim3(NWG), dim3(P1_T), 0, st, (const u64*)ln.codes.p, (const u32*)ln.bad.p, G.nwords,
                        (u32*)ln.partial8.p, g);
 }
@@ -1354,6 +1372,7 @@
 struct SortPlan {
     bool reuse_count;
     bool coarse;
+    bool one;
     bool lazy;
     bool sliced, route2, fine16;
     bool cached_keys;
@@ -1363,10 +1382,15 @@
     int nsl, helper;
 };
 
+static bool one_strand_form(const kr_ctx* c) {
+    return c->coarse_one && c->g.D == 1 && p1_fast_form(c->g) && c->g.L >= 5 && c->g.R < c->g.L && c->g.sbits == 0;
+}
+
 static SortPlan sort_plan(const kr_ctx* c, const Genome& G, const Lane& ln, bool reuse_count, bool coarse) {
     SortPlan p{};
     p.reuse_count = reuse_count;
     p.coarse = coarse;
+    p.one = coarse && !reuse_count && one_strand_form(c);
     p.cached_keys = reuse_count && c->g.wmode == 2 && c->g.wcache;
     p.cached_mode = c->g.wlcnt ? 4 : 2;
     p.sliced = c->nslices > 1;
@@ -1528,7 +1552,7 @@
         hipLaunchKernelGGL(k_hist8k, dim3(NWG), dim3(P1_T), 0, ss, src, (u64)S.nmax, g.sbits, (u32*)ln.partial8.p);
     } else if (!p.reuse_count) {
         StageScope sc(c, KR_ST_HIST8, ss);
-        launch_hist8(c, G, ln, ss, g);
+        launch_hist8(c, G, ln, ss, g, p.one);
     }
     {
         StageScope sc(c, KR_ST_REDUCE8, ss);
@@ -1545,13 +1569,13 @@
                            (const u32*)ls.base1.p, (const u32*)ln.partial8.p, pass1_dst, (u32)S.nmax);
     else
         launch_scatter1(g, ss, (const u64*)ln.codes.p, (const u32*)ln.bad.p, G.nwords, (const u32*)ls.base1.p,
-                        (const u64*)nullptr, (const u32*)ln.partial8.p, pass1_dst, S.nmax);
-}
-
-static void coarse_exit(kr_ctx* c, Lane& ls, Slice& S) {
+                        (const u64*)nullptr, (const u32*)ln.partial8.p, pass1_dst, S.nmax, p.one);
+}
+
+static void coarse_exit(kr_ctx* c, Lane& ls, Slice& S, bool one) {
     StageScope sc(c, KR_ST_REDUCE8, ls.stream);
     hipLaunchKernelGGL(k_coarse_keep, dim3(1), dim3(320), 0, ls.stream, (const u32*)ls.base1.p, (u32*)S.off.p, 1u << c->g.b,
-                       (u32*)S.ovf.p);
+                       (u32*)S.ovf.p, one ? 2u : 1u);
 }
 
 static int pass2(kr_ctx* c, Genome& G, const SortPlan& p, Lane& ln, Lane& ls, Slice& S) {
@@ -1651,7 +1675,7 @@
         if (p.route2) pass1_route2(c, p, ln, ls, S, s, src, pass1_dst);
         else pass1_counted(c, G, p, ln, ls, S, s, src, pass1_dst);
         if (coarse) {
-            coarse_exit(c, ls, S);
+            coarse_exit(c, ls, S, p.one);
             continue;
         }
         if ((rc = pass2(c, G, p, ln, ls, S))) return rc;
@@ -1660,6 +1684,8 @@
     G.ordered = !p.lazy && !coarse;
     G.sorted = !coarse;
     G.coarse = coarse;
+    G.one_strand = p.one;
+    if (p.one) c->one_partitions++;
     return KR_OK;
 }
 
diff --git a/krisp_amd/csrc/h_intersect.inc b/krisp_amd/csrc/h_intersect.inc
--- a/krisp_amd/csrc/h_intersect.inc
+++ b/krisp_amd/csrc/h_intersect.inc
@@ -66,6 +66,10 @@
         }
     }
     if (cg.empty()) return KR_COARSE_PASS;
+    size_t n_one = 0;
+    for (Genome* G : cg) n_one += G->one_strand;
+    if (n_one != 0 && n_one != cg.size()) return KR_COARSE_PASS;
+    const bool one = n_one != 0;
     const bool ok = apply_filter && fmode(c, apply_filter) == 1 && c->g.D == 1 && n <= CO_MAXG && has_in && has_out &&
                     c->nslices == 1 && !c->wide.on && !c->custom_layout;
     if (!ok) return KR_COARSE_PASS;
@@ -84,6 +88,8 @@
     if ((rc = ensure(c, c->co_state, (size_t)nC * 4))) return rc;
     if ((rc = ensure(c, c->co_tab, (size_t)(2 * 260 + 256 * CO_ROW) * 4))) return rc;
     if ((rc = cands_compact_room(c, nC))) return rc;
+    const size_t ent_bytes = (size_t)2 * nC * sizeof(CoEnt);
+    if (one && (rc = ensure(c, c->co_ent, ent_bytes + (size_t)(3 * CS_CLS + 8) * 4))) return rc;
     for (Genome* G : cg) {
         if (G->hitcap < hitcap || !G->hits.p) {
             if ((rc = ensure(c, G->hits, (size_t)hitcap * 8 + 16))) return rc;
@@ -93,8 +99,10 @@
     }
     if (c->co_occ == 0) {
         int per = 0;
-        const hipError_t e = hipOccupancyMaxActiveBlocksPerMultiprocessor(&per, k_coarse_probe, CO_T, 0);
+        const hipError_t e = hipOccupancyMaxActiveBlocksPerMultiprocessor(&per, k_coarse_probe<0>, CO_T, 0);
         c->co_occ = (e == hipSuccess && per >= 1) ? per : 1;
+        if (hipOccupancyMaxActiveBlocksPerMultiprocessor(&per, k_coarse_probe<1>, CO_T, 0) == hipSuccess && per >= 1)
+            c->co_occ = std::min(c->co_occ, per);
     }
     const u32 grid = c->co_grid ? c->co_grid : (u32)(c->co_occ * c->ncu);
     if ((rc = join_lanes(c))) return rc;
@@ -118,9 +126,24 @@
     }
     {
         StageScope sc(c, KR_ST_INTERSECT, st);
-        hipLaunchKernelGGL(k_coarse_tables, dim3(1), dim3(256), 0, st, (const kr_cand*)c->candB.p, nC, ca, c->co_tcap, cb, ust, rows);
-        hipLaunchKernelGGL(k_coarse_probe, dim3(grid), dim3(CO_T), 0, st, ca, (const u32*)cb, (const u32*)ust, (const u32*)rows,
-                           (const kr_cand*)c->candB.p, (u32*)c->co_state.p, c->co_tcap, g.pmask, g.LRrel);
+        if (one) {
+            const CoStrand S = cs_make(g.L, g.R);
+            CoEnt* ents = (CoEnt*)c->co_ent.p;
+            u32 *cnt = (u32*)((char*)c->co_ent.p + ent_bytes), *cls = cnt + CS_CLS, *cursor = cls + CS_CLS + 4;
+            const u32 cgrid = std::min<u32>((nC + CS_T - 1) / CS_T, (u32)c->ncu);
+            HIPCHK(c, hipMemsetAsync(cnt, 0, CS_CLS * 4, st));
+            hipLaunchKernelGGL(k_strand_count, dim3(cgrid), dim3(CS_T), 0, st, (const kr_cand*)c->candB.p, nC, S, cnt);
+            hipLaunchKernelGGL(k_strand_tables, dim3(1), dim3(CS_CLS), 0, st, (const u32*)cnt, ca, c->co_tcap, cls, cursor, ust, rows,
+                               c->mbox + 56);
+            hipLaunchKernelGGL(k_strand_fill, dim3(cgrid), dim3(CS_T), 0, st, (const kr_cand*)c->candB.p, nC, S, cursor, ents);
+            hipLaunchKernelGGL(k_coarse_probe<1>, dim3(grid), dim3(CO_T), 0, st, ca, (const u32*)cls, (const u32*)ust, (const u32*)rows,
+                               (const kr_cand*)c->candB.p, (u32*)c->co_state.p, c->co_tcap, g.pmask, g.LRrel, (const CoEnt*)ents, S);
+        } else {
+            hipLaunchKernelGGL(k_coarse_tables, dim3(1), dim3(256), 0, st, (const kr_cand*)c->candB.p, nC, ca, c->co_tcap, cb, ust, rows);
+            hipLaunchKernelGGL(k_coarse_probe<0>, dim3(grid), dim3(CO_T), 0, st, ca, (const u32*)cb, (const u32*)ust, (const u32*)rows,
+                               (const kr_cand*)c->candB.p, (u32*)c->co_state.p, c->co_tcap, g.pmask, g.LRrel, (const CoEnt*)nullptr,
+                               CoStrand{});
+        }
     }
     for (Genome* G : cg)
         if (G->ckeys.p) G->ckeys_busy = st;
@@ -134,6 +157,13 @@
     HIPCHK(c, hipStreamSynchronize(st));
     HIPCHK(c, hipGetLastError());
     for (Genome* G : cg) G->ckeys_busy = nullptr;
+    if (one) {
+        c->one_calls++;
+        for (int q = 0; q < 2; q++) {
+            c->one_last[q] = ((volatile u32*)c->mbox)[56 + q];
+            c->one_rounds[q] += c->one_last[q];
+        }
+    }
     for (size_t j = 0; j < cg.size(); j++)
         if (((volatile u32*)c->mbox)[32 + j] > hitcap) {
             c->ncand = -1;
diff --git a/krisp_amd/csrc/h_misc.inc b/krisp_amd/csrc/h_misc.inc
--- a/krisp_amd/csrc/h_misc.inc
+++ b/krisp_amd/csrc/h_misc.inc
@@ -270,6 +270,19 @@
     return KR_OK;
 }
 
+int kr_debug_coarse_strand(kr_ctx* c, int64_t* o) {
+    if (!c || !o) return KR_ERR_PARAM;
+    o[0] = c->one_partitions;
+    o[1] = c->one_calls;
+    o[2] = c->one_rounds[0];
+    o[3] = c->one_rounds[1];
+    o[4] = c->one_last[0];
+    o[5] = c->one_last[1];
+    o[6] = c->coarse_one;
+    o[7] = 0;
+    return KR_OK;
+}
+
 int kr_debug_isect(kr_ctx* c, int64_t* o) {
     if (!c || !o) return KR_ERR_PARAM;
     o[0] = c->isect_ovf_items;
diff --git a/krisp_amd/csrc/k_coarse.inc b/krisp_amd/csrc/k_coarse.inc
--- a/krisp_amd/csrc/k_coarse.inc
+++ b/krisp_amd/csrc/k_coarse.inc
@@ -61,17 +61,125 @@
     if (t == 0) ust[256] = total;
 }
 
+#define CS_CLS 512
+#define CS_T 1024
+struct CoEnt { u64 pat; u32 ci, pad; };
+
+__device__ __forceinline__ u32 co_run_add(u32* h, u32 c, bool active) {
+    const u32 lane = threadIdx.x & 63u;
+    if (!active) c = 0xFFFFFFFFu;
+    const u32 prev = (u32)__shfl_up((int)c, 1);
+    const bool head = lane == 0 || prev != c;
+    const u64 hb = __builtin_amdgcn_ballot_w64(head);
+    const u32 leader = 63u - (u32)__clzll((long long)(hb & ((2ull << lane) - 1ull)));
+    const u64 above = (hb >> lane) >> 1;
+    const u32 len = above ? (u32)__builtin_ctzll(above) + 1u : 64u - lane;
+    u32 r0 = 0;
+    if (head && active) r0 = atomicAdd(&h[c], len);
+    return (u32)__shfl((int)r0, (int)leader) + (lane - leader);
+}
+
+__global__ __launch_bounds__(CS_T) void k_strand_count(const kr_cand* __restrict__ cands, u32 n, CoStrand S, u32* __restrict__ cnt) {
+    __shared__ u32 h[CS_CLS];
+    if (threadIdx.x < CS_CLS) h[threadIdx.x] = 0;
+    __syncthreads();
+    for (u32 i0 = blockIdx.x * CS_T; i0 < n; i0 += gridDim.x * CS_T) {
+        const u32 i = i0 + threadIdx.x;
+        const bool on = i < n;
+        const u64 P = cands[on ? i : n - 1].prefix;
+        (void)co_run_add(h, 2 * cs_class_fwd(S, P), on);
+        if (on) atomicAdd(&h[2 * cs_class_rev(S, P) + 1], 1u);
+    }
+    __syncthreads();
+    for (u32 t = threadIdx.x; t < CS_CLS; t += CS_T)
+        if (h[t]) atomicAdd(&cnt[t], h[t]);
+}
+
+__device__ __forceinline__ u32 co_rounds(u32 nc, u32 tcap) { return nc / tcap + (nc % tcap ? 1u : 0u); }
+__global__ __launch_bounds__(CS_CLS) void k_strand_tables(const u32* __restrict__ cnt, CoarseArgs A, u32 tcap, u32* __restrict__ cls,
+                                                          u32* __restrict__ cursor, u32* __restrict__ ust, u32* rows,
+                                                          u32* __restrict__ host_rounds) {
+    __shared__ u32 waves[17];
+    const u32 t = threadIdx.x;
+    u32 total;
+    const u32 ex = block_excl_scan(cnt[t], waves, total);
+    cls[t] = ex;
+    cursor[t] = ex;
+    if (t == 0) cls[CS_CLS] = total;
+    if (t < 4 * A.n) A.hits[t >> 2][t & 3u] = 0;
+    u32 units = 0, rf = 0, rr = 0;
+    if (t < 256) {
+        u32* row = rows + t * CO_ROW;
+        for (u32 j = 0; j < A.n; j++) {
+            row[2 * j] = A.off[j][t];
+            row[2 * j + 1] = A.off[j][t + 1];
+        }
+        rf = co_rounds(cnt[2 * t], tcap);
+        rr = co_rounds(cnt[2 * t + 1], tcap);
+        units = co_byte_units((rf + rr) * tcap, tcap, row, A.n);
+        if (co_row_chunks(row, A.n) == 0) rf = rr = 0;
+    }
+    const u32 ux = block_excl_scan(units, waves, total);
+    if (t < 256) ust[t] = ux;
+    if (t == 0) ust[256] = total;
+    (void)block_excl_scan(rf, waves, total);
+    if (t == 0) host_rounds[0] = total;
+    (void)block_excl_scan(rr, waves, total);
+    if (t == 0) host_rounds[1] = total;
+}
+
+__global__ __launch_bounds__(CS_T) void k_strand_fill(const kr_cand* __restrict__ cands, u32 n, CoStrand S, u32* __restrict__ cursor,
+                                                     CoEnt* __restrict__ ents) {
+    __shared__ u32 h[CS_CLS], base[CS_CLS];
+    if (threadIdx.x < CS_CLS) h[threadIdx.x] = 0;
+    __syncthreads();
+    for (u32 i0 = blockIdx.x * CS_T; i0 < n; i0 += gridDim.x * CS_T) {
+        const u32 i = i0 + threadIdx.x;
+        const bool on = i < n;
+        const u64 P = cands[on ? i : n - 1].prefix;
+        (void)co_run_add(h, 2 * cs_class_fwd(S, P), on);
+        if (on) atomicAdd(&h[2 * cs_class_rev(S, P) + 1], 1u);
+    }
+    __syncthreads();
+    for (u32 t = threadIdx.x; t < CS_CLS; t += CS_T) {
+        base[t] = h[t] ? atomicAdd(&cursor[t], h[t]) : 0u;
+        h[t] = 0;
+    }
+    __syncthreads();
+    for (u32 i0 = blockIdx.x * CS_T; i0 < n; i0 += gridDim.x * CS_T) {
+        const u32 i = i0 + threadIdx.x;
+        const bool on = i < n;
+        const u64 P = cands[on ? i : n - 1].prefix;
+        const u32 cf = 2 * cs_class_fwd(S, P), cr = 2 * cs_class_rev(S, P) + 1;
+        const u32 rank = co_run_add(h, cf, on);
+        if (!on) continue;
+        CoEnt e;
+        e.ci = i;
+        e.pad = 0;
+        e.pat = P;
+        ents[base[cf] + rank] = e;
+        e.pat = cs_pattern_rev(S, P);
+        ents[base[cr] + atomicAdd(&h[cr], 1u)] = e;
+    }
+}
+
+template <int OS>
 __device__ __forceinline__ void co_lookup(u64 key, u64 pmask, int LR, const u32* slots, u32 c0, const kr_cand* __restrict__ cands,
                                           u32* __restrict__ state, u32 orbits, u32 side_shift, u64* s_hit, u32* s_nhit,
-                                          u32* __restrict__ hits, u64* __restrict__ hitkeys, u32 hitcap) {
+                                          u32* __restrict__ hits, u64* __restrict__ hitkeys, u32 hitcap,
+                                          const CoEnt* __restrict__ ents, bool rev, const CoStrand& S) {
     const u64 pre = key & pmask;
     const u32 h = co_hash(pre);
     const u32 tag = h & 0x7FFFFu;
     u32 s = h >> (32 - CO_SLOT_LOG);
     for (u32 w = slots[s]; w != CO_EMPTY; w = slots[s]) {
         if ((w & 0x7FFFFu) == tag) {
-            const u32 ci = c0 + (w >> 19);
-            if (cands[ci].prefix == pre) {
+            u32 ci = c0 + (w >> 19);
+            if ((OS ? ents[ci].pat : cands[ci].prefix) == pre) {
+                if (OS) {
+                    ci = ents[ci].ci;
+                    if (rev) key = cs_rev_key(S, key);
+                }
                 const u32 at0 = atomicAdd(s_nhit, 1u);
                 if (at0 < CO_HB) s_hit[at0] = key;
                 else {
@@ -98,9 +206,11 @@
 
 #define CO_RFL(x) ((u32)__builtin_amdgcn_readfirstlane((int)(x)))
 
+template <int OS>
 __global__ __launch_bounds__(CO_T, 8) void k_coarse_probe(CoarseArgs A, const u32* __restrict__ cb, const u32* __restrict__ ust,
                                                        const u32* __restrict__ rows, const kr_cand* __restrict__ cands,
-                                                       u32* __restrict__ state, u32 tcap, u64 pmask, int LR) {
+                                                       u32* __restrict__ state, u32 tcap, u64 pmask0, int LR,
+                                                       const CoEnt* __restrict__ ents, CoStrand S) {
     __shared__ u32 slots[CO_SLOTS];
     __shared__ u32 bitmap[1u << (CO_BM_LOG - 5)];
     __shared__ u32 s_ust[257];
@@ -123,6 +233,8 @@
     u64* __restrict__ hitkeys = nullptr;
     u32 hitcap = 0, orbits = 0, side_shift = 0;
     bool cold = true;
+    u64 pmask = pmask0;
+    bool rev = false;
 
     auto adopt = [&](const CoUnit& un) {
         const u32 g = un.genome, r = un.round;
@@ -141,11 +253,22 @@
             for (u32 i = threadIdx.x; i < CO_SLOTS; i += CO_T) slots[i] = CO_EMPTY;
             for (u32 i = threadIdx.x; i < (1u << (CO_BM_LOG - 5)); i += CO_T) bitmap[i] = 0;
             __syncthreads();
-            const u32 cb0 = cb[t], cb1 = cb[t + 1];
-            c0 = cb0 + r * tcap;
+            u32 cb0 = cb[OS ? 2 * t : t], cb1 = cb[OS ? 2 * t + 1 : t + 1], rr = r;
+            if (OS) {
+                const u32 rf = CO_RFL(co_rounds(cb1 - cb0, tcap));
+                rev = r >= rf;
+                if (rev) {
+                    rr = r - rf;
+                    cb0 = cb1;
+                    cb1 = cb[2 * t + 2];
+                }
+                const u64 m = rev ? S.mask_rc : pmask0;
+                pmask = ((u64)CO_RFL((u32)(m >> 32)) << 32) | CO_RFL((u32)m);
+            }
+            c0 = cb0 + rr * tcap;
             const u32 c1 = cb1 - c0 > tcap ? c0 + tcap : cb1;
             for (u32 i = c0 + threadIdx.x; i < c1; i += CO_T) {
-                const u32 h = co_hash(cands[i].prefix);
+                const u32 h = co_hash(OS ? ents[i].pat : cands[i].prefix);
                 const u32 word = ((i - c0) << 19) | (h & 0x7FFFFu);
                 u32 s = h >> (32 - CO_SLOT_LOG);
                 while (atomicCAS(&slots[s], CO_EMPTY, word) != CO_EMPTY) s = (s + 1) & (CO_SLOTS - 1);
@@ -215,7 +338,8 @@
         if (s_qn <= CO_QCAP) {
             const u32 qn = s_qn;
             for (u32 i = threadIdx.x; i < qn; i += CO_T)
-                co_lookup(s_q[i], pmask, LR, slots, c0, cands, state, orbits, side_shift, s_hit, &s_nhit, hits, hitkeys, hitcap);
+                co_lookup<OS>(s_q[i], pmask, LR, slots, c0, cands, state, orbits, side_shift, s_hit, &s_nhit, hits, hitkeys, hitcap,
+                              ents, rev, S);
         } else {
             const u32 a0 = k0 & ~1u;
             for (u32 p = a0 + 2 * threadIdx.x; p < k1; p += 2 * CO_T) {
@@ -225,7 +349,8 @@
                     const u64 key = e ? ((u64)w.w << 32 | w.z) : ((u64)w.y << 32 | w.x);
                     const u32 h = co_hash(key & pmask);
                     if (p + e >= k0 && p + e < k1 && ((bitmap[h >> (37 - CO_BM_LOG)] >> ((h >> (32 - CO_BM_LOG)) & 31u)) & 1u))
-                        co_lookup(key, pmask, LR, slots, c0, cands, state, orbits, side_shift, s_hit, &s_nhit, hits, hitkeys, hitcap);
+                        co_lookup<OS>(key, pmask, LR, slots, c0, cands, state, orbits, side_shift, s_hit, &s_nhit, hits, hitkeys, hitcap,
+                                      ents, rev, S);
                 }
             }
         }
@@ -327,9 +452,9 @@
     }
 }
 
-__global__ void k_coarse_keep(const u32* __restrict__ base1, u32* __restrict__ off, u32 nb, u32* __restrict__ ovf) {
+__global__ void k_coarse_keep(const u32* __restrict__ base1, u32* __restrict__ off, u32 nb, u32* __restrict__ ovf, u32 per_key) {
     const u32 t = threadIdx.x;
     if (t <= 256) off[t] = base1[t];
-    else if (t == 257) off[nb] = base1[256];
+    else if (t == 257) off[nb] = per_key * base1[256];
     else if (t == 258) ovf[0] = 0;
 }
diff --git a/krisp_amd/csrc/k_sort.inc b/krisp_amd/csrc/k_sort.inc
--- a/krisp_amd/csrc/k_sort.inc
+++ b/krisp_amd/csrc/k_sort.inc
@@ -115,6 +115,17 @@
     (hist8_window<J>(sf, sr, invalid, g, lhist), ...);
 }
 
+template <int J>
+__device__ __forceinline__ void hist8_window_fwd(const u32 (&sf)[5], u32 invalid, const CoStrand& S, u32* lhist) {
+    if ((invalid >> (31 - J)) & 1u) return;
+    atomicAdd(&lhist[cs_digit(S, (u64)bits128<2 * J>(sf) << 32)], 1u);
+}
+template <int... J>
+__device__ __forceinline__ void hist8_word_fwd(std::integer_sequence<int, J...>, const u32 (&sf)[5], u32 invalid,
+                                               const CoStrand& S, u32* lhist) {
+    (hist8_window_fwd<J>(sf, invalid, S, lhist), ...);
+}
+
 template <int WIDE>
 __global__ __launch_bounds__(P1_T) void k_hist8(const u64* __restrict__ codes, const u32* __restrict__ bad,
                                                u64 nwords, u32* __restrict__ partial8, Geom g) {
@@ -129,6 +140,12 @@
         u32 b0 = bad[w], b1 = bad[w + 1];
         if (b0 == 0xFFFFFFFFu) continue;
         u64 c0 = codes[w], c1 = codes[w + 1];
+        if (WIDE == 3) {
+            const CoStrand S = cs_make(g.L, g.R);
+            const u32 sf[5] = {(u32)(c0 >> 32), (u32)c0, (u32)(c1 >> 32), (u32)c1, 0u};
+            hist8_word_fwd(std::make_integer_sequence<int, 32>{}, sf, word_invalid(b0, b1, g.k), S, lhist);
+            continue;
+        }
         if (WIDE == 2) {
 #pragma unroll 4
             for (int j = 0; j < 32; j++) {
diff --git a/krisp_amd/csrc/k_sort2.inc b/krisp_amd/csrc/k_sort2.inc
--- a/krisp_amd/csrc/k_sort2.inc
+++ b/krisp_amd/csrc/k_sort2.inc
@@ -218,8 +218,9 @@
 
 struct P1Regs { u32x4 c; u32x2 b; };
 
+template <int TPW = P1_TPW>
 __device__ __forceinline__ void p1_issue(P1Regs& r, bufrsrc cs, bufrsrc bs, u64 wt) {
-    const u32 w = (u32)wt + opaque_tid() / P1_TPW;
+    const u32 w = (u32)wt + opaque_tid() / TPW;
     r.c = __builtin_amdgcn_raw_buffer_load_b128(cs, w * 8, 0, 0);
     r.b = __builtin_amdgcn_raw_buffer_load_b64(bs, w * 4, 0, 0);
     __builtin_amdgcn_sched_barrier(0);
@@ -255,14 +256,37 @@
     }
 }
 
-template <int WIDE, int BIG, int FAST = 0>
+#define P1_ONE_TPW (P1_TPW / 2)
+#define P1_ONE_PPT (2 * P1_PPT)
+__device__ __forceinline__ void p1_fast_keys_fwd(u64 c0, u64 c1, u32 b0, u32 b1, const Geom& g, u64 (&key)[P1_KPT], u32& vm) {
+    static_assert(P1_ONE_PPT <= 16 && P1_ONE_PPT == P1_KPT, "a thread's windows must start inside one dword of the shifted string");
+    const u32 q = opaque_tid() % P1_ONE_TPW;
+    const int cs = 2 * P1_ONE_PPT * (int)q;
+    const u64 f01 = cs ? (c0 << cs) | (c1 >> (64 - cs)) : c0;
+    const u32 f0 = (u32)(f01 >> 32), f1 = (u32)f01, f2 = (u32)((c1 << cs) >> 32);
+    const u64 B = (((u64)b0 << 32) | b1) << (P1_ONE_PPT * q);
+    const u32 bh = (u32)(B >> 32), bl = (u32)B;
+    const u32 mLh = (u32)(g.mL >> 32), mLl = (u32)g.mL, mRl = (u32)g.mR, mDl = (u32)g.mD;
+    const u32 sR = (u32)g.sR & 31u, sD = (u32)g.sD & 31u, vsh = 32u - (u32)g.k;
+#pragma unroll
+    for (int jj = 0; jj < P1_ONE_PPT; jj++) {
+        const u32 bm = __funnelshift_l(bl, bh, jj);
+        const u32 fh = __funnelshift_l(f1, f0, 2 * jj), fl = __funnelshift_l(f2, f1, 2 * jj);
+        key[jj] = ((u64)(fh & mLh) << 32) | ((fl & mLl) | ((fl << sR) & mRl) | ((fl >> sD) & mDl));
+        vm |= (bm >> vsh) == 0u ? 1u << jj : 0u;
+    }
+}
+
+template <int WIDE, int BIG, int FAST = 0, int ONE = 0>
 __device__ __forceinline__ void p1_tile(const P1Regs& R, u64 wt, u64 w1, const Geom& g, bufrsrc ds, u64* dst,
                                         u64 sink, u64* stage, u64* cur, u32* cnt, u32* cnt_next, u64* delta,
                                         u32* waves) {
     const u32 tid = opaque_tid();
     const int dsh = BIG ? 64 - P0_DIGIT_BITS(g) : 56;
-    const u64 w = wt + tid / P1_TPW;
+    const u64 w = wt + tid / (ONE ? P1_ONE_TPW : P1_TPW);
     const int j0 = (tid % P1_TPW) * P1_PPT;
+    const CoStrand S = cs_make(ONE ? g.L : 5, ONE ? g.R : 0);
+    auto digit = [&](u64 k) { return ONE ? cs_digit(S, k) : (u32)(k >> dsh); };
     u64 key[P1_KPT];
     u32 rp[P1_KPT / 2];
     u32 vm = 0;
@@ -272,7 +296,9 @@
         const u32 b0 = R.b.x, b1 = R.b.y;
         if (b0 != 0xFFFFFFFFu) {
             const u64 c0 = pair_lo(R.c), c1 = pair_hi(R.c);
-            if (FAST) {
+            if (ONE) {
+                p1_fast_keys_fwd(c0, c1, b0, b1, g, key, vm);
+            } else if (FAST) {
                 p1_fast_keys(c0, c1, b0, b1, g, key, vm);
             } else if (WIDE == 2) {
 #pragma unroll
@@ -298,7 +324,7 @@
     }
 #pragma unroll
     for (int q = 0; q < P1_KPT; q++)
-        if ((vm >> q) & 1) rp[q >> 1] |= atomicAdd(&cnt[(u32)(key[q] >> dsh)], 1u) << (16 * (q & 1));
+        if ((vm >> q) & 1) rp[q >> 1] |= atomicAdd(&cnt[digit(key[q])], 1u) << (16 * (q & 1));
     __syncthreads();
     const u32 c = tid < 256 ? cnt[tid] : 0;
     u32 total;
@@ -312,19 +338,19 @@
     __syncthreads();
 #pragma unroll
     for (int q = 0; q < P1_KPT; q++)
-        if ((vm >> q) & 1) stage[cnt[(u32)(key[q] >> dsh)] + ((rp[q >> 1] >> (16 * (q & 1))) & 0xFFFFu)] = key[q];
+        if ((vm >> q) & 1) stage[cnt[digit(key[q])] + ((rp[q >> 1] >> (16 * (q & 1))) & 0xFFFFu)] = key[q];
     __syncthreads();
 #pragma unroll
     for (int q = 0; q < P1_KPT; q++) {
         const u32 p = q * P1_T + tid;
         const u64 k2 = stage[p];
-        const u64 o = p + delta[(u32)(k2 >> dsh)];
+        const u64 o = p + delta[digit(k2)];
         if (BIG) dst[p < total ? o : sink] = k2;
         else buf_store_u64<KR_P1_ST_AUX>(k2, ds, p < total ? (u32)o * 8 : BUF_OOB);
     }
 }
 
-template <int WIDE, int BIG, int FAST = 0>
+template <int WIDE, int BIG, int FAST = 0, int ONE = 0>
 __global__ __launch_bounds__(P1_T, P1_OCC) void k_scatter1p(const u64* __restrict__ codes, const u32* __restrict__ bad,
                                                             u64 nwords, const u32* __restrict__ base1,
                                                             const u64* __restrict__ base64,
@@ -357,19 +383,21 @@
     const bufrsrc bs = make_rsrc(bad, (u32)(nwords + PAD_WORDS) * 4);
     const bufrsrc ds = make_rsrc(dst, BIG ? 0u : (u32)dst_keys * 8);
     const u64 sink = dst_keys + 1;
+    constexpr int TPW = ONE ? P1_ONE_TPW : P1_TPW;
+    constexpr u64 WORDS = P1_T / TPW;
     P1Regs A, B;
-    p1_issue(A, cs, bs, w0);
+    p1_issue<TPW>(A, cs, bs, w0);
     {
         const bufrsrc none = make_rsrc(dst, 0);
 #pragma unroll
         for (int q = 0; q < P1_KPT; q++) buf_store_u64(0, none, 64u * q);
     }
     __syncthreads();
-    for (u64 wt = w0; wt < w1; wt += 2 * P1_WORDS) {
-        p1_issue(B, cs, bs, wt + P1_WORDS);
-        p1_tile<WIDE, BIG, FAST>(A, wt, w1, g, ds, dst, sink, stage, cur, cnt[0], cnt[1], delta, waves);
-        p1_issue(A, cs, bs, wt + 2 * P1_WORDS);
-        p1_tile<WIDE, BIG, FAST>(B, wt + P1_WORDS, w1, g, ds, dst, sink, stage, cur, cnt[1], cnt[0], delta, waves);
+    for (u64 wt = w0; wt < w1; wt += 2 * WORDS) {
+        p1_issue<TPW>(B, cs, bs, wt + WORDS);
+        p1_tile<WIDE, BIG, FAST, ONE>(A, wt, w1, g, ds, dst, sink, stage, cur, cnt[0], cnt[1], delta, waves);
+        p1_issue<TPW>(A, cs, bs, wt + 2 * WORDS);
+        p1_tile<WIDE, BIG, FAST, ONE>(B, wt + WORDS, w1, g, ds, dst, sink, stage, cur, cnt[1], cnt[0], delta, waves);
     }
 }
 
diff --git a/krisp_amd/csrc/krisp_hip.hip b/krisp_amd/csrc/krisp_hip.hip
--- a/krisp_amd/csrc/krisp_hip.hip
+++ b/krisp_amd/csrc/krisp_hip.hip
@@ -26,6 +26,7 @@
 #include "krisp_hip.h"
 
 #include "k_keys.inc"
+#include "co_strand.inc"
 #include "k_sort.inc"
 #include "k_sort2.inc"
 #include "k_intersect.inc"
```

New measurement: 128.7 billion (median of 6 runs). +5.1%, better.
